# Algolzw/image-restoration-sde

Hardware: AMD Instinct MI355X
Metric: restored images/sec at 256x256, 100-step IR-SDE reverse sampler (higher is better)
Workload: dtype f32; 1 GPU; IR-SDE deraining ConditionalUNet nf=64 depth=4, reverse_sde, batch=16/GPU 256x256, T=100 (BASELINE.json configs[1]); compute_dtype=fp32, global_batch=16

## Files before the change

image_restoration_sde_amd/_lib.py:

```python
import ctypes
import os
import subprocess
import threading

_HERE = os.path.dirname(os.path.abspath(__file__))
LIB_PATH = os.environ.get("IRSDE_LIB_PATH") or os.path.join(_HERE, "libirsde_hip.so")
CSRC = os.path.join(_HERE, "csrc")

MODE = {"sde": 0, "ode": 1, "posterior": 2, "dsde_sde": 3, "dsde_ode": 4}
COEF_STRIDE = 12
FLAG_KEEP_ACTIVATIONS = 1
FLAG_NAIVE_CONV = 2
FLAG_NO_WINOGRAD = 4
FLAG_NO_WINOGRAD_F43 = 8
FLAG_UNCOND_FULLATTN = 16
FLAG_BF16 = 32
FLAG_NAF_INTRO_SKIP = 64
FLAG_BF16_ACT = 128
FLAG_NO_FUSED_LN = 256
FLAG_NAF_LENS = 512
FLAG_FP16 = 1024
FLAG_NO_WINOGRAD_FUSED = 2048
FLAG_NO_FUSED_ATTN = 4096
FLAG_NO_NAF_CHAIN = 8192
FLAG_SPLIT_BF16X2 = 16384
FLAG_SPLIT_F16X2 = 32768
FLAG_NAF_STEREO = 65536
FLAG_NAF_UNCOND = 131072
FLAG_UNET_STEREO = 262144
FLAG_F16_ACT = 524288
FLAG_NO_WINO_POLY = 1048576
FLAG_SCAM_STREAM = 2097152
FLAG_NO_SPLIT3 = 4194304
SAMPLE_GRAPH = 1
SAMPLE_PROFILE = 2

SYMBOLS = [
    "irsde_last_error", "irsde_version", "irsde_create", "irsde_create_nafnet", "irsde_destroy", "irsde_num_weights",
    "irsde_weight_name", "irsde_weight_shape", "irsde_load_weight", "irsde_finalize_weights",
    "irsde_set_schedule", "irsde_unet_forward", "irsde_sample", "irsde_sde_step", "irsde_philox_normal",
    "irsde_get_profile", "irsde_debug_tap", "irsde_work_model", "irsde_debug_conv", "irsde_debug_conv_choice", "irsde_debug_conv_halo_choice", "irsde_debug_conv_features", "irsde_plan_describe", "irsde_bench_conv", "irsde_op_profile", "irsde_debug_split_gemm", "irsde_bench_naf_chain", "irsde_debug_force_subbatches", "irsde_debug_force_chain_groups", "irsde_debug_force_wino_poly", "irsde_debug_force_split3", "irsde_debug_force_split3_attn", "irsde_debug_force_split3_blocks", "irsde_debug_force_split3_1x1", "irsde_debug_split3_1x1", "irsde_debug_split3_1x1_choice", "irsde_debug_scam", "irsde_debug_scam_full",
    "irsde_debug_scam_stream", "irsde_debug_scam_full_stream", "irsde_debug_force_scam_stream",
    "irsde_debug_naf_gate_sca", "irsde_debug_tlsc", "irsde_debug_ln_film", "irsde_debug_naf_lnconv", "irsde_debug_naf_chain", "irsde_debug_naf_chain_split_order",
    "irsde_debug_full_attention16",
    "irsde_eval_metrics", "irsde_tensor2img", "irsde_upscale_bicubic", "irsde_mask_to", "irsde_imresize",
    "irsde_create_lpips", "irsde_lpips", "irsde_debug_lpips_tap",
    "irsde_set_lens_info", "irsde_nafnet_set_local_pool", "irsde_create_latent_unet", "irsde_latent_shapes", "irsde_latent_encode", "irsde_latent_decode", "irsde_latent_hidden",
]


class IrsdeLibraryError(RuntimeError):
    pass


class IrsdeError(RuntimeError):
    pass


class Config(ctypes.Structure):
    _fields_ = [("in_nc", ctypes.c_int32), ("out_nc", ctypes.c_int32), ("nf", ctypes.c_int32),
                ("depth", ctypes.c_int32), ("device", ctypes.c_int32), ("flags", ctypes.c_int32)]


class NafConfig(ctypes.Structure):
    _fields_ = [("img_channel", ctypes.c_int32), ("width", ctypes.c_int32), ("middle_blk_num", ctypes.c_int32),
                ("n_enc", ctypes.c_int32), ("enc_blk_nums", ctypes.c_int32 * 8), ("n_dec", ctypes.c_int32),
                ("dec_blk_nums", ctypes.c_int32 * 8), ("device", ctypes.c_int32), ("flags", ctypes.c_int32)]


class LatentConfig(ctypes.Structure):
    _fields_ = [("in_ch", ctypes.c_int32), ("out_ch", ctypes.c_int32), ("ch", ctypes.c_int32), ("n_mult", ctypes.c_int32),
                ("ch_mult", ctypes.c_int32 * 8), ("embed_dim", ctypes.c_int32), ("device", ctypes.c_int32),
                ("flags", ctypes.c_int32)]


_lib = None
_lock = threading.Lock()


PROBES_LIB_PATH = os.path.join(_HERE, "libirsde_hip_probes.so")


def build_library(force=False, verbose=False, probes=True):
    if force:
        subprocess.run(["make", "-C", CSRC, "clean"], check=True, capture_output=not verbose)
    for extra in ([], ["PROBES=1"]) if probes else ([],):
        r = subprocess.run(["make", "-j8", "-C", CSRC] + extra, capture_output=True, text=True)
        if r.returncode != 0:
            raise IrsdeLibraryError("building libirsde_hip%s.so failed:\n" % ("_probes" if extra else "") + r.stdout + r.stderr)
        if verbose:
            print(r.stdout)
    return LIB_PATH


def _declare(lib):
    c = ctypes
    P = c.c_void_p
    lib.irsde_last_error.restype = c.c_char_p
    lib.irsde_last_error.argtypes = []
    lib.irsde_version.restype = c.c_int
    lib.irsde_create.argtypes = [c.POINTER(Config), c.POINTER(P)]
    lib.irsde_create_nafnet.argtypes = [c.POINTER(NafConfig), c.POINTER(P)]
    lib.irsde_destroy.argtypes = [P]
    lib.irsde_destroy.restype = None
    lib.irsde_num_weights.argtypes = [P]
    lib.irsde_weight_name.argtypes = [P, c.c_int]
    lib.irsde_weight_name.restype = c.c_char_p
    lib.irsde_weight_shape.argtypes = [P, c.c_int, c.POINTER(c.c_int64), c.POINTER(c.c_int)]
    lib.irsde_load_weight.argtypes = [P, c.c_char_p, P, c.POINTER(c.c_int64), c.c_int]
    lib.irsde_finalize_weights.argtypes = [P]
    lib.irsde_set_schedule.argtypes = [P, c.c_int, P]
    lib.irsde_unet_forward.argtypes = [P, P, P, c.POINTER(c.c_int64), c.c_int, c.c_int, c.c_int, c.c_int, P, P]
    lib.irsde_sample.argtypes = [P, c.c_int, P, P, P, c.c_uint64, c.c_uint64, c.c_int, c.c_int, c.c_int,
                                 c.c_int, c.c_int, P, P, c.c_int]
    lib.irsde_sde_step.argtypes = [c.c_int, c.c_int, P, P, P, P, P, c.c_uint64, c.c_uint64, c.c_int, c.c_int,
                                   c.c_int, c.c_int, P]
    lib.irsde_philox_normal.argtypes = [P, c.c_int, c.c_int, c.c_int, c.c_uint64, c.c_uint64, P]
    lib.irsde_get_profile.argtypes = [P, c.POINTER(c.c_double)]
    lib.irsde_debug_tap.argtypes = [P, c.c_char_p, P, c.POINTER(c.c_int64)]
    lib.irsde_work_model.argtypes = [P, c.c_int, c.c_int, c.c_int, c.POINTER(c.c_double)]
    lib.irsde_debug_conv.argtypes = [P, c.c_int, P, c.c_int, c.c_int, c.c_int, c.c_int, c.c_int, P, c.c_int, c.c_int,
                                     c.c_int, c.c_int, c.c_int, P, P, c.c_int, c.c_int, P, P, c.c_int, c.c_int, P]
    lib.irsde_debug_conv_choice.argtypes = [c.c_int] * 13 + [c.c_uint] + [c.c_int] * 4 + [c.POINTER(c.c_int), c.c_char_p, c.c_int]
    lib.irsde_debug_conv_halo_choice.argtypes = [c.c_int] * 13 + [c.c_uint] + [c.c_int] * 5 + [c.c_char_p, c.c_int]
    lib.irsde_debug_conv_features.argtypes = ([P, c.c_int, P, c.c_int] + [c.c_int] * 4 + [P] + [c.c_int] * 7 + [P] * 3 + [P, c.c_int, P, P, P, c.c_int] + [c.c_int] * 6 +
                                              [c.POINTER(c.c_int), P, c.c_char_p, c.c_int, P])
    lib.irsde_plan_describe.argtypes = [P, c.c_int, c.c_int, c.c_int, c.c_char_p, c.c_int]
    lib.irsde_op_profile.argtypes = [P, c.c_char_p, c.c_int]
    lib.irsde_bench_conv.argtypes = [c.c_int] * 11 + [c.POINTER(c.c_double)]
    lib.irsde_bench_naf_chain.argtypes = [c.c_int] * 4 + [c.POINTER(c.c_double)]
    lib.irsde_debug_force_subbatches.argtypes = [c.c_int]
    lib.irsde_debug_force_chain_groups.argtypes = [c.c_int]
    lib.irsde_debug_force_wino_poly.argtypes = [c.c_int]
    lib.irsde_debug_force_split3.argtypes = [c.c_int]
    lib.irsde_debug_force_split3_attn.argtypes = [c.c_int]
    lib.irsde_debug_force_split3_1x1.argtypes = [c.c_int]
    lib.irsde_debug_split3_1x1.argtypes = [P, c.c_int, c.c_int, P, c.c_int, c.c_int, P, P, P, c.c_int, c.c_int, c.c_int, c.c_int, P]
    lib.irsde_debug_split3_1x1_choice.argtypes = [c.c_int] * 13 + [c.c_uint] + [c.c_int] * 6 + [c.c_char_p, c.c_int]
    lib.irsde_debug_force_split3_blocks.argtypes = [c.c_int]
    lib.irsde_debug_scam.argtypes = [P, c.c_int, c.c_int, c.c_int, c.c_int] + [P] * 12 + [P, P]
    lib.irsde_debug_scam_full.argtypes = [P, c.c_int, c.c_int, c.c_int, c.c_int] + [P] * 12 + [P, P]
    lib.irsde_debug_scam_stream.argtypes = [P, c.c_int, c.c_int, c.c_int, c.c_int] + [P] * 12 + [c.c_int, P, P]
    lib.irsde_debug_scam_full_stream.argtypes = [P, c.c_int, c.c_int, c.c_int, c.c_int] + [P] * 12 + [c.c_int, P, P]
    lib.irsde_debug_force_scam_stream.argtypes = [c.c_int]
    lib.irsde_debug_naf_gate_sca.argtypes = [P, c.c_int, c.c_int, c.c_int, c.c_int] + [P] * 8
    lib.irsde_debug_tlsc.argtypes = [P] + [c.c_int] * 6 + [P] * 4
    lib.irsde_debug_ln_film.argtypes = [P, c.c_int64, c.c_int, c.c_int64, P, P, P, c.c_int, P, P]
    lib.irsde_debug_naf_lnconv.argtypes = [c.c_int, P, c.c_int64, c.c_int, c.c_int, c.c_int64, P, P, P, c.c_int, P, P, P, c.c_int, P, P, P, P, P]
    lib.irsde_debug_naf_chain.argtypes = [P, P, c.c_int, c.c_int] + [P] * 16 + [P, c.c_int, c.c_int, P, c.c_int, c.c_int, c.c_int, P]
    lib.irsde_debug_naf_chain_split_order.argtypes = [c.c_int, c.c_int, c.POINTER(c.c_int), c.c_int64]
    lib.irsde_debug_full_attention16.argtypes = [P, c.c_int, c.c_int, P, P]
    lib.irsde_debug_split_gemm.argtypes = [P, P, P, c.c_int, c.c_int, c.c_int, c.c_int, c.c_int, P]
    lib.irsde_eval_metrics.argtypes = [P, P, c.c_int, c.c_int, c.c_int, c.c_int, c.c_int, c.POINTER(c.c_double), P]
    lib.irsde_tensor2img.argtypes = [P, P, c.c_int, c.c_int, c.c_int, c.c_int, P]
    lib.irsde_upscale_bicubic.argtypes = [P, P, c.c_int, c.c_int, c.c_int, c.c_int, c.c_int, P]
    lib.irsde_mask_to.argtypes = [P, P, c.c_int, c.c_int, c.c_int, c.c_int, P, c.c_int, c.c_int, c.c_int, c.c_int, P]
    lib.irsde_imresize.argtypes = [P, P] + [c.c_int] * 6 + [P, P, c.c_int, P, P, c.c_int, P]
    lib.irsde_create_lpips.argtypes = [c.POINTER(P)]
    lib.irsde_lpips.argtypes = [P, P, P, c.c_int, c.c_int, c.c_int, c.c_int, c.POINTER(c.c_double), c.POINTER(c.c_double), P]
    lib.irsde_debug_lpips_tap.argtypes = [P, P, c.c_int, c.c_int, c.c_int, c.c_int, c.c_int, P, c.POINTER(c.c_int64), P]
    lib.irsde_set_lens_info.argtypes =[P, c.POINTER(c.c_float), c.c_int]
    lib.irsde_nafnet_set_local_pool.argtypes = [P, c.c_int, c.c_int, c.c_int, c.c_int]
    lib.irsde_create_latent_unet.argtypes = [c.POINTER(LatentConfig), c.POINTER(P)]
    lib.irsde_latent_shapes.argtypes = [P, c.c_int, c.c_int, c.POINTER(c.c_int64), c.POINTER(c.c_int64), c.POINTER(c.c_int)]
    lib.irsde_latent_encode.argtypes = [P, P, c.c_int, c.c_int, c.c_int, P, c.POINTER(P), P]
    lib.irsde_latent_decode.argtypes = [P, P, c.POINTER(P), c.c_int, c.c_int, c.c_int, P, P]
    lib.irsde_latent_hidden.argtypes = [P, c.c_int, c.c_int, c.c_int, c.c_int, P, P]
    for name in SYMBOLS:
        getattr(lib, name)
    return lib


def lib():
    global _lib
    with _lock:
        if _lib is None:
            if not os.path.exists(LIB_PATH):
                raise IrsdeLibraryError(
                    "libirsde_hip.so not found at %s — build it with `python -c 'import __graft_entry__ as g; "
                    "g.build()'` or `make -C %s`. There is no CPU/PyTorch fallback for this path." % (LIB_PATH, CSRC))
            try:
                _lib = _declare(ctypes.CDLL(LIB_PATH))
            except OSError as ex:
                raise IrsdeLibraryError("failed to load %s: %s" % (LIB_PATH, ex)) from ex
        return _lib


_probes = None


def probes_lib():
    global _probes
    with _lock:
        if _probes is None:
            if not os.path.exists(PROBES_LIB_PATH):
                raise IrsdeLibraryError("libirsde_hip_probes.so not found at %s — build it with `make -C %s PROBES=1`" % (PROBES_LIB_PATH, CSRC))
            try:
                _probes = _declare(ctypes.CDLL(PROBES_LIB_PATH))
            except OSError as ex:
                raise IrsdeLibraryError("failed to load %s: %s" % (PROBES_LIB_PATH, ex)) from ex
        return _probes


def check(rc, L=None):
    if rc != 0:
        msg = (L or lib()).irsde_last_error()
        raise IrsdeError("libirsde_hip error %d: %s" % (rc, msg.decode() if msg else "?"))


def stream_ptr(torch_stream=None):
    import torch
    s = torch_stream if torch_stream is not None else torch.cuda.current_stream()
    return ctypes.c_void_p(s.cuda_stream)
```

image_restoration_sde_amd/csrc/common.h:

```cpp
#pragma once
#include <hip/hip_runtime.h>
#include <cstdint>
#include <cstdio>
#include <cstdlib>
#include <functional>
#include <stdexcept>
#include <string>
#include <vector>
#include "split3_layout.h"

namespace irsde {

struct HipError : std::runtime_error {
    using std::runtime_error::runtime_error;
};
struct HipOutOfMemory : HipError {
    using HipError::HipError;
};

inline int tuning_env_int(const char* name, int dflt) {
    static const bool on = [] { const char* t = getenv("IRSDE_TUNING"); return t && atoi(t) == 1; }();
    if (!on) return dflt;
    const char* v = getenv(name);
    return v ? atoi(v) : dflt;
}

#define IRSDE_HIP_CHECK(expr)                                                                  \
    do {                                                                                       \
        hipError_t _e = (expr);                                                                \
        if (_e != hipSuccess) {                                                                \
            throw ::irsde::HipError(std::string(#expr) + " failed: " + hipGetErrorString(_e) + \
                                    " (" __FILE__ ":" + std::to_string(__LINE__) + ")");       \
        }                                                                                      \
    } while (0)

struct ConvParams {
    const float* in0 = nullptr;
    const float* in1 = nullptr;
    int C0 = 0, C1 = 0;
    int pix0 = 0, pix1 = 0;
    int Hin = 0, Win = 0;
    int in_shift = 0;
    const float* w = nullptr;
    const unsigned short* w_bf = nullptr;
    int f16 = 0;
    const unsigned short* w_pair = nullptr;
    float pair_scale = 1.f;
    int Cout = 0;
    int KH = 1, KW = 1, stride = 1, pad_y = 0, pad_x = 0;
    int B = 0, Ho = 0, Wo = 0;
    float* out = nullptr;
    int out_stride = 0;
    const float* bias = nullptr;
    const float* film = nullptr;
    int film_bstride = 0;
    int silu = 0;
    const float* res = nullptr;
    int res_stride = 0;
    int splits = 1;
    float* partial = nullptr;
    const float* zeros = nullptr;
    const float* ch_scale = nullptr;
    const float* in_scale = nullptr;
    int gate = 0;
    const float* gate_film = nullptr;
    int gate_film_bstride = 0;
    int shuffle = 0;
    int nz = 1;
    long long z_in = 0, z_w = 0, z_out = 0;
    int no_direct_epi = 0;
    int in_bf16 = 0, out_bf16 = 0;
    int in_f16 = 0, out_f16 = 0;
    const float* ln_g = nullptr;
    float ln_eps = 1e-5f;
};

struct WinoParams {
    const float* in0 = nullptr;
    const float* in1 = nullptr;
    int C0 = 0, C1 = 0, Hin = 0, Win = 0, in_shift = 0;
    int B = 0, TH = 0, TW = 0, T = 0;
    int tile = 2;
    float* V = nullptr;
    unsigned short* Vs = nullptr;
    int nplanes = 0;
    int v_f16 = 0;
    float v_scale = 1.f;
    int v_pairs = 0;
    int v_triples = 0;
    const float* M = nullptr;
    int Cout = 0;
    float* out = nullptr;
    int out_stride = 0;
    const float* bias = nullptr;
    const float* film = nullptr;
    int film_bstride = 0;
    int silu = 0;
    const float* res = nullptr;
    int res_stride = 0;
};
void launch_wino_input(const WinoParams& p, hipStream_t s);
struct WinoPolyParams {
    int up = 0;
    const float* in = nullptr;
    int C = 0, Hin = 0, Win = 0;
    int B = 0, TH = 0, TW = 0, T = 0;
    float* V = nullptr;
    unsigned short* Vs = nullptr;
    int thread_writer = 0;
    const float* M = nullptr;
    int Cout = 0, Ho = 0, Wo = 0;
    float* out = nullptr;
    int out_stride = 0;
    const float* bias = nullptr;
};
void launch_wino_poly_input(const WinoPolyParams& p, hipStream_t s);
void launch_wino_poly_output(const WinoPolyParams& p, hipStream_t s);
void wino_poly_transform_weights(const float* w_packed, int Cout, int Cin, float* U, int up);
struct SplitGemmArgs {
    const unsigned short* a = nullptr;
    const unsigned short* b = nullptr;
    float* out = nullptr;
    long long plA = 0, plB = 0, pA = 0, pB = 0, pO = 0;
    int M = 0, N = 0, K = 0, lda = 0, ldc = 0;
    float out_scale = 1.f;
    int n_inner = 1;
    int nblk_n = 0;
};
void gemm_split_global_init();
void launch_gemm_split_pairs(const SplitGemmArgs& a, int ncomp, hipStream_t s, int abl = 0, bool f16 = false);
void launch_split_pairs(const float* in, unsigned short* out, size_t rows, int K, hipStream_t s, bool f16 = false,
                        float scale = 1.0f);
struct Split3Launch {
    enum Abl { FULL = 0, NO_LOADS = 1, NO_MFMA = 3, NO_STORES = 4 };
    enum Tri { RULE, ON, OFF };
    Abl abl = FULL;
    Tri walk = RULE;
    Tri drain = RULE;
};
void launch_gemm_split_triples(const SplitGemmArgs& a, int ncomp, hipStream_t s, const Split3Launch& o = {});
void set_force_split3_blocks(int n);
bool gemm_split_triples_fits(long long M, long long N, long long K, long long ldc);
void launch_split_triples(const float* in, unsigned short* out, int ncomp, size_t rows, int K, hipStream_t s);
struct Split3aArgs {
    const float* in0 = nullptr;
    const float* in1 = nullptr;
    int C0 = 0, C1 = 0;
    int pix0 = 0, pix1 = 0;
    const unsigned short* w3 = nullptr;
    const float* bias = nullptr;
    float* out = nullptr;
    int M = 0, N = 0, out_stride = 0;
    int nblk_n = 0;
};
bool gemm_split3a_fits(const Split3aArgs& a, const char** why_not = nullptr);
int gemm_split3a_blocks(long long M, int N, int cus, bool walk = true);
constexpr size_t kSplit3aLds = (size_t)2 * (256 * 128 + 128 * 192);
void launch_gemm_split3a(const Split3aArgs& a, hipStream_t s, const Split3Launch& o = {});
struct Split3x1Choice {
    bool adopt = false;
    const char* why_not = "";
    int grid = 0, lds = 0;
};
Split3x1Choice split3_1x1_choose(const ConvParams& p, bool exact_f32, int master, int knob, int cus);
Split3aArgs split3_1x1_args(const ConvParams& p, const unsigned short* w3);
void launch_split_planes(const float* in, unsigned short* out, size_t n, size_t plane, int nplanes, hipStream_t s, bool f16 = false,
                         float scale = 1.0f);
void launch_wino_output(const WinoParams& p, hipStream_t s);
void wino_transform_weights(const float* w_packed, int Cout, int Cin, float* U, int tile);
bool wino_fused_eligible(const ConvParams& p);
void wino_fused_pack_weights(const float* U, int Cout, int Cin, float* Uf);
void launch_wino_fused(const ConvParams& p, const float* Uf, hipStream_t s, unsigned long long* dbg = nullptr, int dflags = 0);
int wino_fused_num_blocks(const ConvParams& p);
bool wino_fused64_eligible(const ConvParams& p);
void wino_fused64_pack_weights(const float* U, int Cout, int Cin, float* Uf);
void launch_wino_fused64(const ConvParams& p, const float* Uf, hipStream_t s, int variant = 0);
void wino_fused64_set_debug(unsigned long long* buf);
constexpr float kWinoFused64PairVScale = 0.0625f;
void launch_wino_fused64_split_weights(const float* Uf, unsigned short* out, size_t nfloats, float scale, hipStream_t s);
int wino_fused64_num_blocks(const ConvParams& p);
bool wino_fused64_xcd_nb(const ConvParams& p);
void wino_fused_global_init();
int device_cu_count();
bool wino_fused64t_eligible(const ConvParams& p);
long long wino_fused64t_num_items(const ConvParams& p);
void launch_wino_fused64t(const ConvParams& p, const float* Uf, hipStream_t s, int variant = 0);
void wino_fused64t_set_debug(unsigned long long* buf);
void wino_fused_t_global_init();
void naf_chain_global_init();
void naf_chain_set_debug(unsigned long long* buf);
bool naf_chain_shape_ok(int H, int W, int c);
size_t naf_chain_weight_halves(int nblocks);
size_t naf_chain_vec_floats(int nblocks);
void launch_naf_chain(const float* x, float* out, const unsigned short* w, const float* vecs, int nblocks, int B, const float* film, int film_bstride,
                      int film_off, const float* cam, int cam_bstride, int cam_off, hipStream_t s, int variant = 0);
std::vector<int> naf_chain_split_order(int nblocks, int G);
void naf_chain_build_split_weights(const unsigned short* w1, unsigned short* dst, int nblocks, int G, hipStream_t s);
size_t naf_chain_split_scratch_bytes(int B);
int naf_chain_split_groups(int B, int G);
void launch_naf_chain_split(const float* x, float* out, const unsigned short* wG, const float* vecs, int nblocks, int B, const float* film, int film_bstride,
                            int film_off, const float* cam, int cam_bstride, int cam_off, int G, void* scratch, hipStream_t s);
const unsigned* naf_chain_split_error_flag(const void* scratch, int B);
void naf_chain_split_reset(void* scratch, int B);
void naf_chain_set_sabotage(int on);
void attention_global_init();

double conv_flops(const ConvParams& p);
struct ConvTune {
    enum Tile { TILE_AUTO, TILE_128, TILE_256x128, TILE_256, TILE_128_ONE_PER_CU };
    enum Halo { HALO_AUTO, HALO_OFF, HALO_FORCE_512, HALO_FORCE_256 };
    enum ZLoop { ZLOOP_AUTO, ZLOOP_OFF, ZLOOP_ALL, ZLOOP_PAIRS, ZLOOP_FORCE_1X1 };
    enum Order { ORDER_AUTO, ORDER_N_FAST, ORDER_N_SLOW };
    bool rules_off = false;
    Tile tile = TILE_AUTO;
    bool no_buffer_desc = false;
    bool no_direct_epi = false;
    Halo halo = HALO_AUTO;
    ZLoop zloop = ZLOOP_AUTO;
    Order halo_order = ORDER_AUTO;
};
struct ConvKnobs {
    int small_bn = 2, small_bn_f32 = 0;
    int pair_tile256 = 1, pair_inscale256 = 0;
    int no_bufa = 0;
    int zloop = -1, zloop_1x1 = -1;
    int zloop_maxnk = 32, zloop_minblk = 1024, zloop_deep = 1, zloop_ragged64 = 2048;
};
const ConvKnobs& conv_knobs_from_env();
struct HaloChoice {
    int pixels = 0;
    int BN = 0;
    int op = 0, act = 0;
    int tiles_x = 0, tiles_y = 0, nblk_n = 0;
    int n_slow = 0;
    unsigned grid = 0;
    int lds = 0;
    int instance = -1;
};
constexpr int kHaloInstances = 9;
struct ConvChoice {
    enum Family { PAIR, NARROW3, ZLOOP_BATCH, ZLOOP_1X1, HALO, IGEMM };
    enum Operand { OP_F32, OP_F32_BUF, OP_BF16, OP_F16 };
    enum Storage { ACT_F32, ACT_BF16, ACT_F16 };
    Family family = IGEMM;
    int BM = 0, BN = 0;
    Operand op = OP_F32;
    Storage act = ACT_F32;
    bool inscale = false;
    int zbatch = 0, zrows = 0;
    unsigned gx = 0, gy = 1, gz = 1;
    HaloChoice halo;
    int threads = 0, lds = 0;
    int row = -1;
    std::string name() const;
    long long blocks() const { return (long long)gx * gy * gz; }
};
int conv_base_bn(int Cout);
void conv_validate(const ConvParams& p);
ConvChoice conv_choose(const ConvParams& p, const ConvTune& t, const ConvKnobs& k, int cu_count);
int conv_instance_count();
void launch_conv(const ConvParams& p, hipStream_t s, const ConvTune& t = {}, const ConvKnobs* knobs = nullptr, ConvChoice* chosen = nullptr);
void conv_global_init();
void conv_halo_global_init();
bool conv_halo_eligible(const ConvParams& p);
HaloChoice conv_halo_choose(const ConvParams& p, const ConvTune& t, int halo2, int nslow);
bool conv_halo2_wanted(const ConvParams& p);
HaloChoice launch_conv_halo(const ConvParams& p, hipStream_t s, const ConvTune& t = {});
void launch_fill_random(float* p, size_t n, unsigned seed, float scale, hipStream_t s);
__device__ __forceinline__ float silu_hw(const float v) {
    return v * __builtin_amdgcn_rcpf(1.0f + __builtin_amdgcn_exp2f(v * -1.44269504088896341f));
}

void launch_f32_to_bf16(const float* in, unsigned short* out, size_t n, hipStream_t s);
void launch_f32_to_f16(const float* in, unsigned short* out, size_t n, hipStream_t s);
void launch_bf16_to_f32(const unsigned short* in, float* out, size_t n, hipStream_t s);
void launch_f16_to_f32(const unsigned short* in, float* out, size_t n, hipStream_t s);
void launch_conv_naive(const ConvParams& p, hipStream_t s);

void launch_layernorm(const float* x, const float* g, const float* res, float* out, int64_t M, int C,
                      float eps, hipStream_t s, bool bf16 = false);
void launch_layernorm_film(const float* x, const float* g, const float* scale, const float* shift, int film_bstride,
                           int64_t pixels_per_image, float* out, int64_t M, int C, float eps, hipStream_t s,
                           bool f16 = false);
int dwgate_tiles(int H, int W, int c);
bool naf_lnconv_ok(int c, int Cout, long long M);
void launch_naf_pwconv(const float* x, const float* in_scale, int64_t pixels_per_image, const unsigned short* w16, const float* bias, const float* ch_scale,
                       const float* res, float* out, int64_t M, int c, int Cout, hipStream_t s, bool f16 = false);
void naf_lnconv_global_init();
void launch_naf_lnconv(const float* x, const float* g, const float* fscale, const float* fshift, int film_bstride, int64_t pixels_per_image,
                       const unsigned short* w16, const float* bias, float* out, int64_t M, int c, int Cout, int gate, const float* gate_film,
                       int gate_film_bstride, hipStream_t s, bool f16 = false);
void launch_dwconv_gate(const float* u, const float* w, const float* bias, float* out, float* partial, int B, int H, int W,
                        int c, hipStream_t s, bool f16 = false);
void launch_sca(const float* partial, int ntiles, const float* W, const float* bias, float* mean, float* s_out, int B,
                int c, int HW, hipStream_t s);
void launch_sca_mean(const float* partial, int ntiles, float* mean, int B, int c, int HW, hipStream_t s);
void tlsc_check_shape(int B, int h, int w, int c, int k1, int k2);
void launch_tlsc_pool(const float* gated, float* rowsum, float* pooled, int B, int h, int w, int c, int k1, int k2, hipStream_t s);
void launch_tlsc_scale(float* gated, const float* scale, int B, int h, int w, int c, int k1, int k2, hipStream_t s);
void launch_row_gate(const float* in, float* out, int rows, int h, hipStream_t s);

struct AttnWorkspace {
    float* pmax = nullptr;
    float* pctx = nullptr;
    float* psum = nullptr;
    float* ctx = nullptr;
    int nch = 0;
};
int attn_num_chunks(int N, int B);
void launch_linear_attention(const float* qkv, float* out, int B, int N, const AttnWorkspace& ws, hipStream_t s,
                             bool bf16 = false);

enum class AttnMode : int {
    F32 = 0,
    PairF16 = 1,
    Bf16 = 2,
    Fp16 = 3,
    Bf16x3 = 4,
};
struct AttnProj {
    AttnMode mode = AttnMode::F32;
    bool act_bf16 = false;
    const unsigned short *kv = nullptr, *q = nullptr, *out = nullptr;
    float kv_inv = 1.f, q_inv = 1.f, out_inv = 1.f;
};
bool attn_fused_has_instance(int C, AttnMode mode, bool act_bf16);
void launch_attention_kv_context(const float* xn, const float* wkv, int B, int N, int C, const AttnWorkspace& ws, hipStream_t s,
                                 const float* ln_g = nullptr, float ln_eps = 1e-5f, const AttnProj& proj = {});
__host__ __device__ inline size_t attn_frag3_index(size_t row, int k, int K) {
    return ((((row >> 5) * (size_t)(K >> 4) + (size_t)(k >> 4)) * 2 + (size_t)((k >> 3) & 1)) * 32 + (row & 31)) * 8 + (size_t)(k & 7);
}
void launch_split_frag3(const float* in, unsigned short* out, size_t rows, int K, hipStream_t s);
void launch_attention_q_out(const float* q, float* out, int B, int N, const AttnWorkspace& ws, hipStream_t s);
void launch_attention_q_out_fused(const float* xn, const float* x, const float* wq, const float* wout, const float* bias,
                                  const float* g2, float* y, int B, int N, int C, float eps, const AttnWorkspace& ws, hipStream_t s,
                                  const float* ln_g = nullptr, const AttnProj& proj = {});

void scam_check_shape(int H, int W, int c, bool any_width = false);
void launch_scam_prologue(const float* x, const float* g_l, const float* g_r, float* xs2, int B, int H, int W, int c, hipStream_t s);
void launch_scam_core(const float* qv, float* F, int B, int H, int W, int c, hipStream_t s);
void launch_scam_epilogue(const float* x, const float* F, const float* beta, const float* gamma, float* out, int B, int H, int W, int c, hipStream_t s);
void scam_pack_proj(const float* w1, const float* b1, const float* w2, const float* b2, int c, std::vector<float>& w, std::vector<float>& bias);
constexpr int kScamFullMaxW = 1024;
constexpr int kScamFullMaxC = 2048;
void scam_full_check_shape(int H, int W, int c, bool any_width = false);
void launch_scam_full_prologue(const float* x, const float* g_l, const float* g_r, float* x2, int B, int H, int W, int c, hipStream_t s);
void launch_scam_full_core(const float* qv, float* F, int B, int H, int W, int c, hipStream_t s);
void launch_scam_full_epilogue(float* x, const float* F, const float* beta, const float* gamma, int B, int H, int W, int c, hipStream_t s);
constexpr int kScamMaxWs = 512;
constexpr int kScamStreamMaxBlockW = 512;
bool scam_stream_block_ok(int block_w);
void launch_scam_stream_core(const float* qv, float* F, int B, int Hs, int Ws, int c, int block_w, hipStream_t s);
void launch_stereo_prep(const float* xt, const float* cond, float* x0, int B, int ic, int P, int H, int W, int Hp, int Wp, hipStream_t s);
void launch_stereo_pack_pred(const float* in, float* out, int B, int ic, int Hp, int Wp, int in_stride, int out_stride, hipStream_t s);
void launch_stereo_unet_prep(const float* xt, const float* cond, float* x0, int B, int ic, int P, int H, int W, int Hp, int Wp, hipStream_t s);
void launch_stereo_unet_pack_pred(const float* in, const float* xt, float* out, int B, int ic, int H, int W, int Hp, int Wp, int in_stride, int out_stride,
                                  hipStream_t s);

void launch_full_attention(const float* qkv, float* out, int B, int N, hipStream_t s);
void launch_full_attention16(const unsigned short* qkv, unsigned short* out, int B, int N, hipStream_t s);

void launch_prep_input(const float* xt, const float* cond, float* x0, int B, int in_nc, int H, int W, int Hp, int Wp,
                       hipStream_t s, int reflect = 1);

enum Act { ACT_NONE = 0, ACT_SILU = 1, ACT_GELU = 2 };
void launch_sinusoid(const float* tvals, const float* freqs, float* out, int rows, int half, hipStream_t s);
void launch_row_linear(const float* in, int in_stride, const float* W, const float* b, float* out, int out_stride,
                       int rows, int in_dim, int out_dim, int act_in, int act_out, hipStream_t s);

struct StepState {
    int t;
    int t_next;
    int pad0, pad1;
    float coef[12];
};
void launch_step_begin(StepState* st, const float* film_table, int film_row, float* film_cur,
                       const float* coef_table, hipStream_t s);
void launch_set_step(StepState* st, int t_next, hipStream_t s);

struct SampleCtl {
    int mode;
    int pad;
    const float* noise;
    long long noise_tstride;
    unsigned long long seed;
    unsigned long long image_offset;
};
void launch_set_ctl(SampleCtl* ctl, int mode, const float* noise, long long noise_tstride, unsigned long long seed,
                    unsigned long long image_offset, hipStream_t s);

void launch_unpack_pred(const float* pred, float* out, int B, int C, int H, int W, int Hp, int Wp, int stride, hipStream_t s);
void launch_add(const float* a, const float* b, float* out, size_t n, hipStream_t s);
void launch_nchw_to_nhwc_pad(const float* in, float* out, int B, int C, int H, int W, int Hp, int Wp, int Cp, int reflect,
                             hipStream_t s);
void launch_nhwc_to_nchw(const float* in, float* out, int B, int C, int H, int W, hipStream_t s, bool bf16 = false, bool f16 = false);

struct UpdateParams {
    float* x;
    const float* mu;
    const float* pred;
    int64_t sb, sc, sy, sx;
    const float* noise;
    int64_t noise_tstride;
    const StepState* st;
    const SampleCtl* ctl;
    int t_imm;
    float coef_imm[12];
    int mode;
    int B, C, H, W;
    uint64_t seed;
    uint64_t image_offset;
    int batch0;
};
void launch_sde_update(const UpdateParams& p, hipStream_t s);
void launch_philox_normal(float* out, int B, int CHW, int t, uint64_t seed, uint64_t image_offset, hipStream_t s);

void eval_metrics(const float* out, const float* gt, int B, int C, int H, int W, int crop, double* sums_host, hipStream_t s);
void tensor2img_u8(const float* in, unsigned char* out, int B, int C, int H, int W, hipStream_t s);

struct LpipsLayer { int k, stride, pad, cin, cout; };
constexpr LpipsLayer kLpipsLayers[5] = {{11, 4, 2, 3, 64}, {5, 1, 2, 64, 192}, {3, 1, 1, 192, 384}, {3, 1, 1, 384, 256}, {3, 1, 1, 256, 256}};
inline int lpips_cin_padded(int l) { return (kLpipsLayers[l].cin + 3) & ~3; }
struct LpipsWeights {
    const float* w[5];
    const float* bias[5];
    const float* lin[5];
};
struct LpipsGeom {
    int h[5], w[5];
    int ph[2], pw[2];
};
LpipsGeom lpips_geometry(int H, int W);
int lpips_dist_blocks(int hw);
size_t lpips_workspace_floats(int N, int H, int W);
void lpips_features(const LpipsWeights& wt, const float* in0, const float* in1, int B, int H, int W, int normalize, float* ws, float* taps[5], hipStream_t s,
                    const std::function<void(const char*)>& mark);
void lpips_distances(const LpipsWeights& wt, float* const taps[5], int B, int H, int W, double* partial, hipStream_t s,
                     const std::function<void(const char*)>& mark);

void upscale_bicubic(const float* in, float* out, int B, int C, int H, int W, int scale, hipStream_t s);
void mask_to(const float* x, const unsigned char* masks, int Bm, int Hm, int Wm, int Cm, float* out, int B, int C, int H, int W, hipStream_t s);
void imresize(const float* in, float* out, int B, int C, int H, int W, int Ho, int Wo, const float* wH, const int* sH, int KH, const float* wW,
              const int* sW, int KW, hipStream_t s);

}
```

image_restoration_sde_amd/csrc/engine_debug.hip:

```cpp
#include "engine.h"
#include "../../include/irsde_hip_debug.h"

using namespace irsde;

namespace irsde {
namespace {

struct Scratch {
    hipStream_t s;
    std::vector<void*> bufs;
    explicit Scratch(hipStream_t s_) : s(s_) {}
    ~Scratch() {
        (void)hipStreamSynchronize(s);
        for (void* p : bufs) (void)hipFree(p);
    }
    Scratch(const Scratch&) = delete;
    Scratch& operator=(const Scratch&) = delete;
    template <class T> T* alloc(size_t n) {
        void* p = nullptr;
        IRSDE_HIP_CHECK(hipMalloc(&p, n * sizeof(T)));
        bufs.push_back(p);
        return static_cast<T*>(p);
    }
    float* upload(const float* host, size_t n) {
        float* d = alloc<float>(n);
        IRSDE_HIP_CHECK(hipMemcpy(d, host, n * sizeof(float), hipMemcpyHostToDevice));
        return d;
    }
    float* upload(const std::vector<float>& v) { return upload(v.data(), v.size()); }
};
struct OwnedStream {
    hipStream_t s = nullptr;
    explicit OwnedStream(unsigned flags) { IRSDE_HIP_CHECK(hipStreamCreateWithFlags(&s, flags)); }
    ~OwnedStream() { (void)hipStreamDestroy(s); }
    OwnedStream(const OwnedStream&) = delete;
    OwnedStream& operator=(const OwnedStream&) = delete;
};
struct EventPair {
    hipEvent_t e0 = nullptr, e1 = nullptr;
    EventPair() {
        IRSDE_HIP_CHECK(hipEventCreate(&e0));
        IRSDE_HIP_CHECK(hipEventCreate(&e1));
    }
    ~EventPair() {
        if (e0) (void)hipEventDestroy(e0);
        if (e1) (void)hipEventDestroy(e1);
    }
    EventPair(const EventPair&) = delete;
    EventPair& operator=(const EventPair&) = delete;
};
template <class Run>
double time_launches(hipStream_t s, int iters, Run&& run) {
    EventPair ev;
    IRSDE_HIP_CHECK(hipEventRecord(ev.e0, s));
    for (int i = 0; i < iters; ++i) run();
    IRSDE_HIP_CHECK(hipEventRecord(ev.e1, s));
    IRSDE_HIP_CHECK(hipStreamSynchronize(s));
    float ms = 0.f;
    IRSDE_HIP_CHECK(hipEventElapsedTime(&ms, ev.e0, ev.e1));
    return ms / iters;
}


ConvTune conv_tune_from_code(int code) {
    ConvTune t;
    t.rules_off = code != 0;
    switch (code) {
        case 3: t.tile = ConvTune::TILE_256x128; break;
        case 50: t.tile = ConvTune::TILE_256; break;
        case 5: t.tile = ConvTune::TILE_128_ONE_PER_CU; break;
        case 6: t.no_buffer_desc = true; break;
        case 7: t.no_direct_epi = true; break;
        case 60: t.tile = ConvTune::TILE_256; t.halo = ConvTune::HALO_OFF; break;
        case 61: t.tile = ConvTune::TILE_128; t.halo = ConvTune::HALO_OFF; break;
        case 64: t.halo = ConvTune::HALO_FORCE_512; break;
        case 65: t.halo = ConvTune::HALO_FORCE_256; break;
        case 68: t.halo = ConvTune::HALO_FORCE_512; t.halo_order = ConvTune::ORDER_N_SLOW; break;
        case 69: t.halo = ConvTune::HALO_FORCE_256; t.halo_order = ConvTune::ORDER_N_SLOW; break;
        case 70: t.zloop = ConvTune::ZLOOP_OFF; break;
        case 71: t.zloop = ConvTune::ZLOOP_ALL; break;
        case 72: t.zloop = ConvTune::ZLOOP_PAIRS; break;
        case 73: t.zloop = ConvTune::ZLOOP_FORCE_1X1; break;
        default: break;
    }
    return t;
}

Split3Launch split3_launch_twin(int twin, int abl = 0) {
    Split3Launch o;
    o.abl = static_cast<Split3Launch::Abl>(abl);
    o.walk = twin == 0 ? Split3Launch::RULE : twin == 1 ? Split3Launch::OFF : Split3Launch::ON;
    o.drain = twin == 0 ? Split3Launch::RULE : twin == 1 ? Split3Launch::OFF : Split3Launch::ON;
    return o;
}

enum class Operand { F32, BF16, F16 };

enum class ConvPath {
    Direct,
    Valu,
    WinoF2,
    WinoF4,
    Poly,
    PolyTriples,
    F4Triples,
    F4Pairs,
    DirectPair,
    Fused32,
    Fused64,
    Fused64Pair,
    Fused64T,
    Split3a,
};
struct DebugConvRow {
    int code;
    ConvPath path;
    Operand op;
    bool act_bf16;
    int tune;
    int variant;
    bool up;
    bool thread_writer;
};
constexpr DebugConvRow direct(int code, Operand op, bool act_bf16, int tune) { return {code, ConvPath::Direct, op, act_bf16, tune, 0, false, false}; }
constexpr DebugConvRow on_path(int code, ConvPath path, Operand op = Operand::F32) { return {code, path, op, false, 0, 0, false, false}; }
constexpr DebugConvRow wino(int code, ConvPath path, int tune) { return {code, path, Operand::F32, false, tune, 0, false, false}; }
constexpr DebugConvRow poly(int code, ConvPath path, bool up, bool thread_writer = false) { return {code, path, Operand::F32, false, 0, 0, up, thread_writer}; }
constexpr DebugConvRow fused(int code, ConvPath path, int variant) { return {code, path, Operand::F32, false, 0, variant, false, false}; }
constexpr DebugConvRow kDebugConv[] = {
    direct(0, Operand::F32, false, 0),
    on_path(1, ConvPath::Valu),
    wino(2, ConvPath::WinoF2, 0), wino(12, ConvPath::WinoF2, 71), wino(22, ConvPath::WinoF2, 72),
    wino(3, ConvPath::WinoF4, 0), wino(13, ConvPath::WinoF4, 71), wino(23, ConvPath::WinoF4, 72),
    poly(24, ConvPath::Poly, false), poly(25, ConvPath::Poly, true),
    poly(26, ConvPath::PolyTriples, false), poly(27, ConvPath::PolyTriples, true), poly(28, ConvPath::PolyTriples, true, true),
    on_path(48, ConvPath::F4Triples), on_path(49, ConvPath::Split3a),
    on_path(44, ConvPath::F4Pairs, Operand::F16), on_path(45, ConvPath::F4Pairs, Operand::BF16),
    on_path(46, ConvPath::DirectPair, Operand::F16), on_path(47, ConvPath::DirectPair, Operand::BF16),
    on_path(33, ConvPath::Fused32),
    fused(34, ConvPath::Fused64, 0), fused(36, ConvPath::Fused64, 64), fused(55, ConvPath::Fused64, 20),
    fused(35, ConvPath::Fused64Pair, 4), fused(37, ConvPath::Fused64Pair, 4 + 64), fused(56, ConvPath::Fused64Pair, 24),
    fused(62, ConvPath::Fused64T, 0), fused(63, ConvPath::Fused64T, 64),
    direct(4, Operand::BF16, false, 0), direct(160, Operand::BF16, false, 60), direct(161, Operand::BF16, false, 61), direct(162, Operand::BF16, false, 64),
    direct(163, Operand::BF16, false, 65),
    direct(5, Operand::F16, false, 0), direct(165, Operand::F16, false, 61), direct(166, Operand::F16, false, 64), direct(167, Operand::F16, false, 65),
    direct(204, Operand::BF16, true, 0), direct(260, Operand::BF16, true, 60), direct(261, Operand::BF16, true, 61), direct(262, Operand::BF16, true, 64),
    direct(263, Operand::BF16, true, 65),
    direct(100, Operand::F32, false, 0), direct(103, Operand::F32, false, 3), direct(105, Operand::F32, false, 5), direct(106, Operand::F32, false, 6),
    direct(107, Operand::F32, false, 7), direct(150, Operand::F32, false, 50), direct(170, Operand::F32, false, 70), direct(171, Operand::F32, false, 71),
    direct(172, Operand::F32, false, 72), direct(173, Operand::F32, false, 73),
};

enum class BenchKind {
    Conv,
    Fused32,
    Fused32Stamps,
    Wino3,
    Wino3Gemm,
    Fused64,
    Fused64Stamps,
    Fused64T,
    Fused64TStamps,
    PairGemm,
    TripleGemm,
    Split3aGemm,
};
struct BenchRow {
    int lo, hi;
    BenchKind kind;
    int arg;
    Operand op;
    bool pair;
    bool act_bf16;
};
constexpr BenchRow bench(int lo, int hi, BenchKind kind, int arg, Operand op = Operand::F32, bool pair = false, bool act_bf16 = false) {
    return {lo, hi, kind, arg, op, pair, act_bf16};
}
constexpr BenchRow kBenchConv[] = {
    bench(0, 0, BenchKind::Conv, 0), bench(3, 3, BenchKind::Conv, 3), bench(5, 7, BenchKind::Conv, 5), bench(50, 50, BenchKind::Conv, 50),
    bench(70, 73, BenchKind::Conv, 70),
    bench(60, 61, BenchKind::Conv, 60, Operand::BF16),
    bench(62, 62, BenchKind::Conv, 0, Operand::BF16),
    bench(63, 63, BenchKind::Conv, 0, Operand::BF16, false, true),
    bench(64, 65, BenchKind::Conv, 64, Operand::BF16),
    bench(66, 67, BenchKind::Conv, 64, Operand::BF16, false, true),
    bench(480, 480, BenchKind::Conv, 0, Operand::F16, true), bench(481, 481, BenchKind::Conv, 0, Operand::BF16, true),
    bench(482, 482, BenchKind::Conv, 61, Operand::F16, true),
    bench(80, 80, BenchKind::Fused32, 0),
    bench(83, 82 + 255, BenchKind::Fused32, 1),
    bench(82, 82, BenchKind::Fused32Stamps, 0),
    bench(81, 81, BenchKind::Wino3, 0), bench(421, 421, BenchKind::Wino3Gemm, 0),
    bench(430, 432, BenchKind::Fused64, 20),
    bench(434, 434, BenchKind::Fused64, 24, Operand::F16),
    bench(435, 435, BenchKind::Fused64Stamps, 25), bench(2004, 2004, BenchKind::Fused64Stamps, 25),
    bench(2001, 2002, BenchKind::Fused64Stamps, 28),
    bench(460, 462, BenchKind::Fused64T, 0),
    bench(467, 469, BenchKind::Fused64T, 6),
    bench(465, 465, BenchKind::Fused64TStamps, 5),
    bench(4650, 4653, BenchKind::Fused64TStamps, 12),
    bench(472, 476, BenchKind::PairGemm, 0),
    bench(490, 504, BenchKind::TripleGemm, 0),
    bench(510, 524, BenchKind::Split3aGemm, 0),
};

template <class Row, size_t N, class Lo, class Hi>
constexpr bool codes_disjoint(const Row (&rows)[N], Lo lo, Hi hi) {
    for (size_t i = 0; i < N; ++i)
        for (size_t j = 0; j < N; ++j)
            if (i != j && lo(rows[i]) <= hi(rows[j]) && lo(rows[j]) <= hi(rows[i])) return false;
    return true;
}
constexpr int row_code(const DebugConvRow& r) { return r.code; }
constexpr int row_lo(const BenchRow& r) { return r.lo; }
constexpr int row_hi(const BenchRow& r) { return r.hi; }
static_assert(codes_disjoint(kDebugConv, row_code, row_code), "irsde_debug_conv: a selector code has two rows");
static_assert(codes_disjoint(kBenchConv, row_lo, row_hi), "irsde_bench_conv: a variant has two rows");

const DebugConvRow& debug_conv_lookup(int code) {
    for (const DebugConvRow& r : kDebugConv)
        if (r.code == code) return r;
    throw HipError("debug_conv: unknown selector code " + std::to_string(code));
}
struct BenchSel {
    const BenchRow& row;
    int arg;
};
BenchSel bench_conv_lookup(int code) {
    for (const BenchRow& r : kBenchConv)
        if (code >= r.lo && code <= r.hi) return {r, r.arg + (code - r.lo)};
    throw HipError("bench_conv: unknown variant " + std::to_string(code));
}

SplitGemmArgs split_gemm_args(const unsigned short* a, const unsigned short* b, float* C, int M, int N, int K, size_t pA, size_t pB) {
    SplitGemmArgs g;
    g.a = a; g.b = b; g.out = C;
    g.pA = (long long)pA; g.pB = (long long)pB; g.pO = (long long)M * N;
    g.M = M; g.N = N; g.K = K; g.lda = K; g.ldc = N;
    return g;
}
SplitGemmArgs split_triples(Scratch& mem, const float* A, const float* Bm, float* C, int M, int N, int K, int ncomp, hipStream_t s) {
    const size_t ea = split3_comp_elems((size_t)M, (size_t)K), eb = split3_comp_elems((size_t)N, (size_t)K);
    unsigned short *ta = mem.alloc<unsigned short>(ea * ncomp), *tb = mem.alloc<unsigned short>(eb * ncomp);
    launch_split_triples(A, ta, ncomp, (size_t)M, K, s);
    launch_split_triples(Bm, tb, ncomp, (size_t)N, K, s);
    return split_gemm_args(ta, tb, C, M, N, K, ea, eb);
}
SplitGemmArgs split_pairs(Scratch& mem, const float* A, const float* Bm, float* C, int M, int N, int K, int ncomp, hipStream_t s, bool f16 = false, float sa = 1.f,
                          float sb = 1.f) {
    unsigned short *pa = mem.alloc<unsigned short>((size_t)2 * ncomp * M * K), *pb = mem.alloc<unsigned short>((size_t)2 * ncomp * N * K);
    launch_split_pairs(A, pa, (size_t)ncomp * M, K, s, f16, sa);
    launch_split_pairs(Bm, pb, (size_t)ncomp * N, K, s, f16, sb);
    SplitGemmArgs g = split_gemm_args(pa, pb, C, M, N, K, (size_t)M * K, (size_t)N * K);
    g.out_scale = 1.0f / (sa * sb);
    return g;
}

void write_choice_line(const ConvChoice& c, char* out, int out_len) {
    snprintf(out, (size_t)out_len, "name=%s family=%d tile=%dx%d op=%d act=%d inscale=%d zbatch=%d zrows=%d grid=%ux%ux%u threads=%d lds=%d row=%d of %d",
             c.name().c_str(), (int)c.family, c.BM, c.BN, (int)c.op, (int)c.act, (int)c.inscale, c.zbatch, c.zrows, c.gx, c.gy, c.gz, c.threads, c.lds, c.row,
             conv_instance_count());
}

void write_halo_line(const HaloChoice& h, char* out, int out_len) {
    snprintf(out, (size_t)out_len, "kernel=halo%d bn=%d op=%d act=%d tiles=%dx%d nblk_n=%d nslow=%d grid=%u lds=%d instance=%d of %d", h.pixels, h.BN, h.op, h.act,
             h.tiles_x, h.tiles_y, h.nblk_n, h.n_slow, h.grid, h.lds, h.instance, kHaloInstances);
}

ConvParams choice_hook_params(int B, int Hin, int Win, int C0, int C1, int Cout, int K, int stride, int pad, int in_shift, int operand, int storage, int pair,
                              unsigned features, int splits, int nz) {
    static const float dummy[4] = {};
    float* const some = const_cast<float*>(dummy);
    auto bit = [&](int i) { return (features >> i & 1u) ? some : nullptr; };
    ConvParams p;
    p.in0 = some; p.C0 = C0; p.pix0 = C0; p.in1 = C1 ? some : nullptr; p.C1 = C1; p.pix1 = C1;
    p.Hin = Hin; p.Win = Win; p.in_shift = in_shift;
    p.w = some; p.Cout = Cout; p.KH = K; p.KW = K; p.stride = stride; p.pad_y = pad; p.pad_x = pad;
    p.B = B;
    p.Ho = ((Hin << in_shift) + 2 * pad - K) / stride + 1;
    p.Wo = ((Win << in_shift) + 2 * pad - K) / stride + 1;
    p.out = some; p.out_stride = Cout; p.res_stride = Cout; p.zeros = some;
    p.bias = bit(0); p.film = bit(1); p.silu = bit(2) != nullptr; p.res = bit(3); p.in_scale = bit(4); p.ch_scale = bit(5);
    p.gate = bit(6) != nullptr; p.shuffle = bit(7) != nullptr; p.ln_g = bit(8);
    if (pair) p.w_pair = reinterpret_cast<const unsigned short*>(some);
    else if (operand) p.w_bf = reinterpret_cast<const unsigned short*>(some);
    p.f16 = operand == 2;
    p.in_bf16 = p.out_bf16 = storage == 1;
    p.in_f16 = p.out_f16 = storage == 2;
    p.nz = nz;
    if (splits > 1) { p.splits = splits; p.partial = some; }
    return p;
}

struct ScamHookArgs {
    const float* x;
    float* out;
    const float *norm_l_g, *norm_r_g, *l_proj1_w, *l_proj1_b, *r_proj1_w, *r_proj1_b, *l_proj2_w, *l_proj2_b, *r_proj2_w, *r_proj2_b, *beta, *gamma;
};
struct ScamHookDev {
    float *gl, *gr, *beta, *gamma;
    float *in2, *qv, *F;
    size_t vsz;
};
template <class ShapeCheck, class Prologue, class Tail>
void scam_hook(const ScamHookArgs& a, int B, int Hs, int Ws, int C, void* stream, ShapeCheck check_shape, Prologue prologue, Tail tail) {
    if (!a.x || !a.out || !a.norm_l_g || !a.norm_r_g || !a.l_proj1_w || !a.l_proj1_b || !a.r_proj1_w || !a.r_proj1_b || !a.l_proj2_w || !a.l_proj2_b ||
        !a.r_proj2_w || !a.r_proj2_b || !a.beta || !a.gamma)
        throw HipError("null argument");
    check_shape();
    hipStream_t s = reinterpret_cast<hipStream_t>(stream);
    conv_global_init();
    std::vector<float> wl, bl, wr, br;
    scam_pack_proj(a.l_proj1_w, a.l_proj1_b, a.l_proj2_w, a.l_proj2_b, C, wl, bl);
    scam_pack_proj(a.r_proj1_w, a.r_proj1_b, a.r_proj2_w, a.r_proj2_b, C, wr, br);
    Scratch mem(s);
    auto up = [&](const float* h, size_t n) {
        float* d = mem.alloc<float>(std::max<size_t>(n, 16));
        if (h) IRSDE_HIP_CHECK(hipMemcpy(d, h, n * 4, hipMemcpyHostToDevice));
        return d;
    };
    ScamHookDev d;
    d.gl = up(a.norm_l_g, C); d.gr = up(a.norm_r_g, C); d.beta = up(a.beta, C); d.gamma = up(a.gamma, C);
    float *dwl = up(wl.data(), wl.size()), *dbl = up(bl.data(), bl.size()), *dwr = up(wr.data(), wr.size()), *dbr = up(br.data(), br.size());
    d.vsz = (size_t)B * Hs * Ws * 2 * C;
    d.in2 = up(nullptr, 2 * d.vsz); d.qv = up(nullptr, 2 * d.vsz); d.F = up(nullptr, d.vsz);
    float* dz = up(nullptr, 256);
    IRSDE_HIP_CHECK(hipMemset(dz, 0, 1024));
    prologue(d, s);
    for (int v = 0; v < 2; ++v) {
        ConvParams p;
        p.in0 = d.in2 + v * d.vsz; p.C0 = 2 * C; p.pix0 = 2 * C;
        p.Hin = Hs; p.Win = Ws;
        p.w = v ? dwr : dwl; p.Cout = 2 * C; p.KH = p.KW = 1; p.stride = 1;
        p.B = B; p.Ho = Hs; p.Wo = Ws;
        p.out = d.qv + v * d.vsz; p.out_stride = 2 * C;
        p.bias = v ? dbr : dbl;
        p.zeros = dz;
        launch_conv(p, s);
    }
    tail(d, s);
    IRSDE_HIP_CHECK(hipStreamSynchronize(s));
}

}
}

extern "C" {

int irsde_debug_scam(const float* x, int B, int H, int W, int C, const float* norm_l_g, const float* norm_r_g, const float* l_proj1_w,
                     const float* l_proj1_b, const float* r_proj1_w, const float* r_proj1_b, const float* l_proj2_w, const float* l_proj2_b,
                     const float* r_proj2_w, const float* r_proj2_b, const float* beta, const float* gamma, float* out, void* stream) {
    return guard([&] {
        scam_hook(
            {x, out, norm_l_g, norm_r_g, l_proj1_w, l_proj1_b, r_proj1_w, r_proj1_b, l_proj2_w, l_proj2_b, r_proj2_w, r_proj2_b, beta, gamma}, B, H / 4, W / 4, C, stream,
            [&] {
                if (B < 1) throw HipError("debug_scam: bad shape");
                scam_check_shape(H, W, C);
            },
            [&](const ScamHookDev& d, hipStream_t s) { launch_scam_prologue(x, d.gl, d.gr, d.in2, B, H, W, C, s); },
            [&](const ScamHookDev& d, hipStream_t s) {
                launch_scam_core(d.qv, d.F, B, H, W, C, s);
                launch_scam_epilogue(x, d.F, d.beta, d.gamma, out, B, H, W, C, s);
            });
    });
}

int irsde_debug_scam_full(const float* x, int B, int H, int W, int C, const float* norm_l_g, const float* norm_r_g, const float* l_proj1_w,
                          const float* l_proj1_b, const float* r_proj1_w, const float* r_proj1_b, const float* l_proj2_w, const float* l_proj2_b,
                          const float* r_proj2_w, const float* r_proj2_b, const float* beta, const float* gamma, float* out, void* stream) {
    return guard([&] {
        scam_hook(
            {x, out, norm_l_g, norm_r_g, l_proj1_w, l_proj1_b, r_proj1_w, r_proj1_b, l_proj2_w, l_proj2_b, r_proj2_w, r_proj2_b, beta, gamma}, B, H, W, C, stream,
            [&] {
                if (B < 1 || (long long)B * H > 65535) throw HipError("debug_scam_full: bad shape");
                scam_full_check_shape(H, W, C);
            },
            [&](const ScamHookDev& d, hipStream_t s) { launch_scam_full_prologue(x, d.gl, d.gr, d.in2, B, H, W, C, s); },
            [&](const ScamHookDev& d, hipStream_t s) {
                launch_scam_full_core(d.qv, d.F, B, H, W, C, s);
                if (out != x) IRSDE_HIP_CHECK(hipMemcpyAsync(out, x, d.vsz * sizeof(float), hipMemcpyDeviceToDevice, s));
                launch_scam_full_epilogue(out, d.F, d.beta, d.gamma, B, H, W, C, s);
            });
    });
}

int irsde_debug_scam_stream(const float* x, int B, int H, int W, int C, const float* norm_l_g, const float* norm_r_g, const float* l_proj1_w,
                            const float* l_proj1_b, const float* r_proj1_w, const float* r_proj1_b, const float* l_proj2_w, const float* l_proj2_b,
                            const float* r_proj2_w, const float* r_proj2_b, const float* beta, const float* gamma, int block_w, float* out, void* stream) {
    return guard([&] {
        scam_hook(
            {x, out, norm_l_g, norm_r_g, l_proj1_w, l_proj1_b, r_proj1_w, r_proj1_b, l_proj2_w, l_proj2_b, r_proj2_w, r_proj2_b, beta, gamma}, B, H / 4, W / 4, C, stream,
            [&] {
                if (B < 1 || (long long)B * (H / 4) > 65535) throw HipError("debug_scam_stream: bad shape");
                if (block_w != 0 && !scam_stream_block_ok(block_w)) throw HipError("debug_scam_stream: block_w must be 0 or a multiple of 16 in [16, 512]");
                scam_check_shape(H, W, C, true);
            },
            [&](const ScamHookDev& d, hipStream_t s) { launch_scam_prologue(x, d.gl, d.gr, d.in2, B, H, W, C, s); },
            [&](const ScamHookDev& d, hipStream_t s) {
                launch_scam_stream_core(d.qv, d.F, B, H / 4, W / 4, C, block_w, s);
                launch_scam_epilogue(x, d.F, d.beta, d.gamma, out, B, H, W, C, s);
            });
    });
}

int irsde_debug_scam_full_stream(const float* x, int B, int H, int W, int C, const float* norm_l_g, const float* norm_r_g, const float* l_proj1_w,
                                 const float* l_proj1_b, const float* r_proj1_w, const float* r_proj1_b, const float* l_proj2_w, const float* l_proj2_b,
                                 const float* r_proj2_w, const float* r_proj2_b, const float* beta, const float* gamma, int block_w, float* out,
                                 void* stream) {
    return guard([&] {
        scam_hook(
            {x, out, norm_l_g, norm_r_g, l_proj1_w, l_proj1_b, r_proj1_w, r_proj1_b, l_proj2_w, l_proj2_b, r_proj2_w, r_proj2_b, beta, gamma}, B, H, W, C, stream,
            [&] {
                if (B < 1 || (long long)B * H > 65535) throw HipError("debug_scam_full_stream: bad shape");
                if (block_w != 0 && !scam_stream_block_ok(block_w)) throw HipError("debug_scam_full_stream: block_w must be 0 or a multiple of 16 in [16, 512]");
                scam_full_check_shape(H, W, C, true);
            },
            [&](const ScamHookDev& d, hipStream_t s) { launch_scam_full_prologue(x, d.gl, d.gr, d.in2, B, H, W, C, s); },
            [&](const ScamHookDev& d, hipStream_t s) {
                launch_scam_stream_core(d.qv, d.F, B, H, W, C, block_w, s);
                if (out != x) IRSDE_HIP_CHECK(hipMemcpyAsync(out, x, d.vsz * sizeof(float), hipMemcpyDeviceToDevice, s));
                launch_scam_full_epilogue(out, d.F, d.beta, d.gamma, B, H, W, C, s);
            });
    });
}

int irsde_debug_force_scam_stream(int block_w) {
    if (block_w != 0 && !scam_stream_block_ok(block_w)) return guard([&] { throw HipError("debug_force_scam_stream: block_w must be 0 or a multiple of 16 in [16, 512]"); });
    set_force_scam_stream(block_w);
    return IRSDE_OK;
}

int irsde_debug_naf_gate_sca(const float* u, int B, int H, int W, int c, const float* conv2_w, const float* conv2_b, const float* sca_w, const float* sca_b,
                             float* gated_out, float* mean_out, float* s_out, void* stream) {
    return guard([&] {
        if (!u || !conv2_w || !conv2_b || !sca_w || !sca_b || !gated_out || !s_out) throw HipError("null argument");
        if (B < 1 || B > 65535 || H < 1 || W < 1 || c < 4 || c % 4 || (long long)H * W >= (1ll << 31)) throw HipError("debug_naf_gate_sca: bad shape");
        hipStream_t s = reinterpret_cast<hipStream_t>(stream);
        conv_global_init();
        Scratch mem(s);
        float *dw = mem.upload(pack_dwconv_taps(conv2_w, 2 * c)), *db = mem.upload(conv2_b, (size_t)2 * c);
        float *dsw = mem.upload(sca_w, (size_t)c * c), *dsb = mem.upload(sca_b, c);
        const int nt = dwgate_tiles(H, W, c);
        float *partial = mem.alloc<float>((size_t)B * nt * c), *mean = mem.alloc<float>((size_t)B * c);
        launch_dwconv_gate(u, dw, db, gated_out, partial, B, H, W, c, s);
        launch_sca(partial, nt, dsw, dsb, mean, s_out, B, c, H * W, s);
        if (mean_out) launch_sca_mean(partial, nt, mean_out, B, c, H * W, s);
        IRSDE_HIP_CHECK(hipStreamSynchronize(s));
    });
}

int irsde_debug_tlsc(const float* g, int B, int h, int w, int c, int k1, int k2, float* pooled_out, const float* scale_map, float* scaled_out, void* stream) {
    return guard([&] {
        if (!g || !pooled_out || !scale_map || !scaled_out) throw HipError("null argument");
        tlsc_check_shape(B, h, w, c, k1, k2);
        hipStream_t s = reinterpret_cast<hipStream_t>(stream);
        conv_global_init();
        Scratch mem(s);
        float* rowsum = mem.alloc<float>((size_t)B * h * (w - k2 + 1) * c);
        launch_tlsc_pool(g, rowsum, pooled_out, B, h, w, c, k1, k2, s);
        IRSDE_HIP_CHECK(hipMemcpyAsync(scaled_out, g, (size_t)B * h * w * c * sizeof(float), hipMemcpyDeviceToDevice, s));
        launch_tlsc_scale(scaled_out, scale_map, B, h, w, c, k1, k2, s);
        IRSDE_HIP_CHECK(hipStreamSynchronize(s));
    });
}

int irsde_debug_ln_film(const float* x, long long M, int C, long long ppi, const float* g, const float* fscale, const float* fshift, int film_bstride,
                        float* out, void* stream) {
    return guard([&] {
        if (!x || !g || !fscale || !fshift || !out) throw HipError("null argument");
        if (M < 1 || ppi < 1 || C < 4 || C % 4 || C > 2048 || film_bstride < 0 || film_bstride % 4) throw HipError("debug_ln_film: bad shape");
        hipStream_t s = reinterpret_cast<hipStream_t>(stream);
        conv_global_init();
        Scratch mem(s);
        float* dg = mem.upload(g, C);
        launch_layernorm_film(x, dg, fscale, fshift, film_bstride, ppi, out, M, C, 1e-5f, s);
        IRSDE_HIP_CHECK(hipStreamSynchronize(s));
    });
}

int irsde_debug_full_attention16(const void* qkv_bf16, int B, int N, void* out_bf16, void* stream) {
    return guard([&] {
        if (!qkv_bf16 || !out_bf16) throw HipError("null argument");
        hipStream_t s = reinterpret_cast<hipStream_t>(stream);
        launch_full_attention16(static_cast<const unsigned short*>(qkv_bf16), static_cast<unsigned short*>(out_bf16), B, N, s);
        IRSDE_HIP_CHECK(hipStreamSynchronize(s));
    });
}

int irsde_debug_naf_lnconv(int mode, const float* x, long long M, int c, int Cout, long long ppi, const float* g, const float* fscale, const float* fshift,
                           int film_bstride, const float* w, const float* bias, const float* gate_film, int gate_film_bstride, const float* in_scale,
                           const float* ch_scale, const float* res, float* out, void* stream) {
    return guard([&] {
        if (mode < 0 || mode > 3) throw HipError("debug_naf_lnconv: mode must be 0 .. 3");
        if (!x || !w || !bias || !out) throw HipError("null argument");
        if (!naf_lnconv_ok(c, Cout, M) || ppi < 1) throw HipError("debug_naf_lnconv: bad shape");
        const bool ln = mode <= 1;
        if (ln && (!g || !fscale || !fshift || film_bstride < 0 || film_bstride % 4)) throw HipError("debug_naf_lnconv: modes 0 / 1 need g and the FiLM rows");
        if (mode == 1 && gate_film && gate_film_bstride < 0) throw HipError("debug_naf_lnconv: bad lens FiLM stride");
        if (!ln && (!ch_scale || !res || (mode == 2 && !in_scale))) throw HipError("debug_naf_lnconv: modes 2 / 3 need ch_scale and res, mode 2 in_scale");
        hipStream_t s = reinterpret_cast<hipStream_t>(stream);
        conv_global_init();
        std::vector<float> pw, pb;
        pack_conv_rows(w, bias, Cout, c, 1, 1, mode == 1 ? naf_gate_perm(Cout / 2) : std::vector<int>(), pw, pb);
        Scratch mem(s);
        float *dwf = mem.upload(pw), *dbias = mem.upload(pb);
        unsigned short* w16 = mem.alloc<unsigned short>(pw.size());
        launch_f32_to_f16(dwf, w16, pw.size(), s);
        if (ln) {
            float* dg = mem.upload(g, c);
            launch_naf_lnconv(x, dg, fscale, fshift, film_bstride, ppi, w16, dbias, out, M, c, Cout, mode, mode == 1 ? gate_film : nullptr,
                              mode == 1 && gate_film ? gate_film_bstride : 0, s);
        } else {
            float* dcs = mem.upload(ch_scale, Cout);
            launch_naf_pwconv(x, mode == 2 ? in_scale : nullptr, ppi, w16, dbias, dcs, res, out, M, c, Cout, s);
        }
        IRSDE_HIP_CHECK(hipStreamSynchronize(s));
    });
}

int irsde_debug_naf_chain(const float* x, float* out, int B, int nblocks, const float* norm1_g, const float* conv1_w, const float* conv1_b, const float* conv2_w,
                          const float* conv2_b, const float* sca_w, const float* sca_b, const float* conv3_w, const float* conv3_b, const float* beta,
                          const float* norm2_g, const float* conv4_w, const float* conv4_b, const float* conv5_w, const float* conv5_b, const float* gamma,
                          const float* film, int film_bstride, int film_off, const float* cam, int cam_bstride, int cam_off, int groups, void* stream) {
    return guard([&] {
        if (!x || !out || !norm1_g || !conv1_w || !conv1_b || !conv2_w || !conv2_b || !sca_w || !sca_b || !conv3_w || !conv3_b || !beta || !norm2_g || !conv4_w ||
            !conv4_b || !conv5_w || !conv5_b || !gamma || !film)
            throw HipError("null argument");
        if (B < 1 || B > 65535 || nblocks < 1 || nblocks > 64) throw HipError("debug_naf_chain: bad B or nblocks");
        if (groups != 1 && groups != 2 && groups != 4) throw HipError("debug_naf_chain: groups must be 1, 2 or 4");
        if (film_bstride < 0 || film_bstride % 4 || film_off < 0 || film_off % 4) throw HipError("debug_naf_chain: bad FiLM stride / offset");
        if (cam && (cam_bstride < 0 || cam_bstride % 4 || cam_off < 0 || cam_off % 4)) throw HipError("debug_naf_chain: bad lens FiLM stride / offset");
        hipStream_t s = reinterpret_cast<hipStream_t>(stream);
        conv_global_init();
        if (groups > 1 && naf_chain_split_groups(B, groups) > device_cu_count())
            throw HipError("debug_naf_chain: more work-groups than compute units (they must be co-resident)");
        constexpr size_t C = 512;
        std::vector<NafChainHostW> blocks(nblocks);
        for (int i = 0; i < nblocks; ++i) {
            NafChainHostW& b = blocks[i];
            const size_t k = (size_t)i;
            b.norm1_g = norm1_g + k * C; b.conv1_w = conv1_w + k * 2 * C * C; b.conv1_b = conv1_b + k * 2 * C;
            b.conv2_w = conv2_w + k * 18 * C; b.conv2_b = conv2_b + k * 2 * C;
            b.sca_w = sca_w + k * C * C; b.sca_b = sca_b + k * C;
            b.conv3_w = conv3_w + k * C * C; b.conv3_b = conv3_b + k * C; b.beta = beta + k * C;
            b.norm2_g = norm2_g + k * C; b.conv4_w = conv4_w + k * 2 * C * C; b.conv4_b = conv4_b + k * 2 * C;
            b.conv5_w = conv5_w + k * C * C; b.conv5_b = conv5_b + k * C; b.gamma = gamma + k * C;
        }
        std::vector<unsigned short> w;
        std::vector<float> vecs;
        pack_naf_chain_host(blocks, w, vecs);
        Scratch mem(s);
        unsigned short* dw = mem.alloc<unsigned short>(w.size());
        IRSDE_HIP_CHECK(hipMemcpy(dw, w.data(), w.size() * 2, hipMemcpyHostToDevice));
        float* dvec = mem.upload(vecs);
        if (groups == 1) {
            launch_naf_chain(x, out, dw, dvec, nblocks, B, film, film_bstride, film_off, cam, cam ? cam_bstride : 0, cam ? cam_off : 0, s, 0);
            IRSDE_HIP_CHECK(hipStreamSynchronize(s));
            return;
        }
        unsigned short* dwg = mem.alloc<unsigned short>(w.size());
        naf_chain_build_split_weights(dw, dwg, nblocks, groups, s);
        const size_t sb = naf_chain_split_scratch_bytes(B);
        char* dscratch = mem.alloc<char>(sb);
        IRSDE_HIP_CHECK(hipMemset(dscratch, 0, sb));
        launch_naf_chain_split(x, out, dwg, dvec, nblocks, B, film, film_bstride, film_off, cam, cam ? cam_bstride : 0, cam ? cam_off : 0, groups, dscratch, s);
        IRSDE_HIP_CHECK(hipStreamSynchronize(s));
        std::vector<unsigned> state((size_t)4 * B + 1);
        IRSDE_HIP_CHECK(hipMemcpy(state.data(), naf_chain_split_error_flag(dscratch, B) - 4 * B, state.size() * 4, hipMemcpyDeviceToHost));
        if (state[(size_t)4 * B]) throw HipError("debug_naf_chain: the split kernel's groups were not co-resident (spin timeout)");
        for (size_t i = 0; i < (size_t)4 * B; ++i)
            if (state[i]) throw HipError("debug_naf_chain: the split kernel left a barrier counter non-zero");
    });
}

int irsde_debug_naf_chain_split_order(int nblocks, int groups, int* order_out, long long n) {
    return guard([&] {
        if (!order_out || nblocks < 1 || nblocks > 64) throw HipError("debug_naf_chain_split_order: bad argument");
        const std::vector<int> order = naf_chain_split_order(nblocks, groups);
        if ((long long)order.size() != n) throw HipError("debug_naf_chain_split_order: the order has " + std::to_string(order.size()) + " entries");
        std::copy(order.begin(), order.end(), order_out);
    });
}

int irsde_debug_conv(const float* in0, int C0, const float* in1, int C1, int B, int Hin, int Win, int in_shift,
                     const float* w_oihw, int Cout, int KH, int KW, int stride, int pad, const float* bias,
                     const float* film, int film_bstride, int silu, const float* res, float* out, int naive,
                     int splits, void* stream) {
    return guard([&] {
        if (!in0 || !w_oihw || !out) throw HipError("null argument");
        const DebugConvRow& r = debug_conv_lookup(naive);
        hipStream_t s = reinterpret_cast<hipStream_t>(stream);
        conv_global_init();
        const int Cin = C0 + C1;
        std::vector<float> pk((size_t)Cout * KH * KW * Cin);
        for (int o = 0; o < Cout; ++o)
            for (int i = 0; i < Cin; ++i)
                for (int ky = 0; ky < KH; ++ky)
                    for (int kx = 0; kx < KW; ++kx)
                        pk[(((size_t)o * KH + ky) * KW + kx) * Cin + i] = w_oihw[(((size_t)o * Cin + i) * KH + ky) * KW + kx];
        Scratch mem(s);
        float* dw = mem.upload(pk);
        float* db = bias ? mem.upload(bias, Cout) : nullptr;
        ConvParams p;
        p.in0 = in0; p.C0 = C0; p.pix0 = C0; p.in1 = in1; p.C1 = C1; p.pix1 = C1;
        p.Hin = Hin; p.Win = Win; p.in_shift = in_shift;
        p.w = dw; p.Cout = Cout; p.KH = KH; p.KW = KW; p.stride = stride; p.pad_y = pad; p.pad_x = pad;
        p.B = B;
        p.Ho = ((Hin << in_shift) + 2 * pad - KH) / stride + 1;
        p.Wo = ((Win << in_shift) + 2 * pad - KW) / stride + 1;
        p.out = out; p.out_stride = Cout; p.bias = db; p.film = film; p.film_bstride = film_bstride; p.silu = silu;
        p.res = res; p.res_stride = Cout;
        float* dz = mem.alloc<float>(256);
        IRSDE_HIP_CHECK(hipMemset(dz, 0, 1024));
        p.zeros = dz;
        if (splits > 1 && r.path != ConvPath::Valu && r.path != ConvPath::WinoF2 && r.path != ConvPath::WinoF4) {
            p.splits = splits;
            p.partial = mem.alloc<float>((size_t)splits * B * p.Ho * p.Wo * Cout);
        }
        auto wino_weights = [&](int tile) {
            std::vector<float> U((size_t)(tile + 2) * (tile + 2) * Cout * Cin);
            wino_transform_weights(pk.data(), Cout, Cin, U.data(), tile);
            return U;
        };
        auto wino_tiles = [&](int tile) { return (long long)B * (p.Ho / tile) * (p.Wo / tile); };
        auto alloc_M = [&](int ncomp, long long T) { return mem.alloc<float>((size_t)ncomp * T * Cout); };
        auto poly_plan = [&](const char* refusal, float*& dU) {
            if (!(r.up ? wino_poly_up_shape(p) : wino_poly_down_shape(p)) || !wino_poly_eligible(p) || splits > 1) throw HipError(refusal);
            std::vector<float> U((size_t)100 * Cout * Cin);
            wino_poly_transform_weights(pk.data(), Cout, Cin, U.data(), r.up);
            dU = mem.upload(U);
            return make_wino_poly(p, dU, nullptr, nullptr);
        };
        switch (r.path) {
        case ConvPath::PolyTriples: {
            float* dU = nullptr;
            WinoPolyPlan wp = poly_plan("debug_conv: selectors 26 / 27 / 28 run what 24 / 25 run (single source, channels a multiple of 32, bias only)", dU);
            if (!gemm_split_triples_fits(wp.T, Cout, wp.K, Cout)) throw HipError("debug_conv: shape not eligible for the three-piece GEMM");
            unsigned short* dUt = mem.alloc<unsigned short>((size_t)wp.ncomp * split3_comp_elems((size_t)Cout, (size_t)wp.K));
            unsigned short* dVt = mem.alloc<unsigned short>((size_t)wp.ncomp * split3_comp_elems((size_t)wp.T, (size_t)wp.K));
            float* dM = alloc_M(wp.ncomp, wp.T);
            launch_split_triples(dU, dUt, wp.ncomp, (size_t)Cout, wp.K, s);
            wp = make_wino_poly(p, dU, nullptr, dM);
            const SplitGemmArgs sg = make_wino_poly_triples(wp, Cout, dUt, dVt, dM);
            wp.in.thread_writer = r.thread_writer;
            launch_wino_poly_input(wp.in, s);
            launch_gemm_split_triples(sg, wp.ncomp, s);
            launch_wino_poly_output(wp.out, s);
            break;
        }
        case ConvPath::Poly: {
            float* dU = nullptr;
            WinoPolyPlan wp = poly_plan(r.up ? "debug_conv: selector 25 runs a 3x3 stride-1 pad-1 convolution with in_shift = 1 (single source, channels a multiple of 32, bias only)"
                                             : "debug_conv: selector 24 runs a 4x4 stride-2 pad-1 convolution (single source, channels a multiple of 32, bias only)", dU);
            float* dV = mem.alloc<float>((size_t)wp.ncomp * wp.T * wp.K);
            wp = make_wino_poly(p, dU, dV, alloc_M(wp.ncomp, wp.T));
            launch_wino_poly_input(wp.in, s);
            launch_conv(wp.gemm, s);
            launch_wino_poly_output(wp.out, s);
            break;
        }
        case ConvPath::F4Triples: {
            if (!wino_shape_ok(p, 4) || Cin % 32) throw HipError("debug_conv: shape not eligible for the three-piece GEMM");
            const std::vector<float> U = wino_weights(4);
            const long long T = wino_tiles(4);
            if (!gemm_split_triples_fits(T, Cout, Cin, Cout)) throw HipError("debug_conv: shape not eligible for the three-piece GEMM");
            float* dU = mem.upload(U);
            unsigned short* dUt = mem.alloc<unsigned short>((size_t)36 * split3_comp_elems((size_t)Cout, (size_t)Cin));
            unsigned short* dVt = mem.alloc<unsigned short>((size_t)36 * split3_comp_elems((size_t)T, (size_t)Cin));
            launch_split_triples(dU, dUt, 36, (size_t)Cout, Cin, s);
            const WinoSplitPlan sp = make_wino_triples(p, dUt, dVt, alloc_M(36, T));
            launch_wino_input(sp.in, s);
            launch_gemm_split_triples(sp.gemm, 36, s);
            launch_wino_output(sp.out, s);
            break;
        }
        case ConvPath::Split3a: {
            if (splits > 1) p.splits = splits;
            const Split3x1Choice c = split3_1x1_choose(p, true, 2, 2, device_cu_count());
            if (!c.adopt) throw HipError(std::string("debug_conv: selector 49 runs a plain 1x1 layer (bias only): ") + c.why_not);
            unsigned short* dwt = mem.alloc<unsigned short>(split3_comp_elems((size_t)Cout, (size_t)Cin));
            launch_split_triples(dw, dwt, 1, (size_t)Cout, Cin, s);
            launch_gemm_split3a(split3_1x1_args(p, dwt), s);
            break;
        }
        case ConvPath::F4Pairs: {
            const bool f16 = r.op == Operand::F16;
            if (!wino_shape_ok(p, 4) || Cin % 32) throw HipError("debug_conv: shape not eligible for the pair GEMM");
            std::vector<float> U = wino_weights(4);
            const float us = f16 ? pow2_scale_into_512(U.data(), U.size()) : 1.f;
            const long long T = wino_tiles(4);
            float* dU = mem.upload(U);
            unsigned short* dUp = mem.alloc<unsigned short>(2 * U.size());
            unsigned short* dVp = mem.alloc<unsigned short>((size_t)36 * T * Cin * 2);
            launch_split_pairs(dU, dUp, (size_t)36 * Cout, Cin, s, f16, us);
            const WinoSplitPlan sp = make_wino_pairs(p, dUp, dVp, alloc_M(36, T), f16, us);
            launch_wino_input(sp.in, s);
            launch_gemm_split_pairs(sp.gemm, 36, s, 0, f16);
            launch_wino_output(sp.out, s);
            break;
        }
        case ConvPath::Fused64Pair: {
            if (!wino_fused64_eligible(p)) throw HipError("debug_conv: shape not eligible for the fused Winograd kernel");
            std::vector<float> U = wino_weights(4), Uf(U.size());
            wino_fused64_pack_weights(U.data(), Cout, Cin, Uf.data());
            const float usc = pow2_scale_into_512(U.data(), U.size());
            float* dUf = mem.upload(Uf);
            unsigned short* dUp = mem.alloc<unsigned short>(2 * Uf.size());
            launch_wino_fused64_split_weights(dUf, dUp, Uf.size(), usc, s);
            p.pair_scale = 1.0f / (kWinoFused64PairVScale * usc);
            launch_wino_fused64(p, reinterpret_cast<const float*>(dUp), s, r.variant);
            break;
        }
        case ConvPath::Fused32:
        case ConvPath::Fused64:
        case ConvPath::Fused64T: {
            const bool f32k = r.path == ConvPath::Fused32;
            if (f32k ? !wino_fused_eligible(p) : !wino_fused64_eligible(p)) throw HipError("debug_conv: shape not eligible for the fused Winograd kernel");
            const std::vector<float> U = wino_weights(4);
            std::vector<float> Uf(U.size());
            if (f32k) wino_fused_pack_weights(U.data(), Cout, Cin, Uf.data());
            else wino_fused64_pack_weights(U.data(), Cout, Cin, Uf.data());
            float* dUf = mem.upload(Uf);
            if (r.path == ConvPath::Fused64T) {
                if (!wino_fused64t_eligible(p)) throw HipError("debug_conv: shape not eligible for the two-tile-group fused Winograd kernel");
                launch_wino_fused64t(p, dUf, s, r.variant);
            } else if (f32k) {
                launch_wino_fused(p, dUf, s);
            } else {
                launch_wino_fused64(p, dUf, s, r.variant);
            }
            break;
        }
        case ConvPath::WinoF2:
        case ConvPath::WinoF4: {
            const int tile = r.path == ConvPath::WinoF2 ? 2 : 4, ncomp = (tile + 2) * (tile + 2);
            if (!wino_shape_ok(p, tile)) throw HipError("debug_conv: shape not eligible for Winograd");
            const std::vector<float> U = wino_weights(tile);
            const long long T = wino_tiles(tile);
            float* dU = mem.upload(U);
            float* dV = mem.alloc<float>((size_t)ncomp * T * Cin);
            const WinoPlan wp = make_wino(p, dU, dV, alloc_M(ncomp, T), tile);
            launch_wino_input(wp.in, s);
            launch_conv(wp.gemm, s, conv_tune_from_code(r.tune));
            launch_wino_output(wp.out, s);
            break;
        }
        case ConvPath::DirectPair: {
            const bool f16 = r.op == Operand::F16;
            const float sc = f16 ? pow2_scale_into_512(pk.data(), pk.size()) : 1.f;
            unsigned short* dwp = mem.alloc<unsigned short>(2 * pk.size());
            launch_split_pairs(dw, dwp, (size_t)Cout, KH * KW * (C0 + C1), s, f16, sc);
            p.w_pair = dwp; p.pair_scale = 1.0f / sc; p.f16 = f16 ? 1 : 0;
            launch_conv(p, s);
            break;
        }
        case ConvPath::Valu:
            launch_conv_naive(p, s);
            break;
        case ConvPath::Direct: {
            unsigned short* ao = nullptr;
            if (r.op != Operand::F32) {
                unsigned short* d16 = mem.alloc<unsigned short>(pk.size());
                if (r.op == Operand::F16) launch_f32_to_f16(dw, d16, pk.size(), s);
                else launch_f32_to_bf16(dw, d16, pk.size(), s);
                p.w_bf = d16;
                p.f16 = r.op == Operand::F16 ? 1 : 0;
            }
            const size_t npix_in = (size_t)B * Hin * Win, nout = (size_t)B * p.Ho * p.Wo * Cout;
            if (r.act_bf16) {
                auto to_bf = [&](const float* src, size_t n) {
                    unsigned short* d = mem.alloc<unsigned short>(n + 32);
                    launch_f32_to_bf16(src, d, n, s);
                    return reinterpret_cast<const float*>(d);
                };
                p.in0 = to_bf(in0, npix_in * C0);
                if (in1) p.in1 = to_bf(in1, npix_in * C1);
                if (res) p.res = to_bf(res, nout);
                ao = mem.alloc<unsigned short>(nout + 32);
                p.out = reinterpret_cast<float*>(ao);
                p.in_bf16 = p.out_bf16 = 1;
            }
            launch_conv(p, s, conv_tune_from_code(r.tune));
            if (r.act_bf16) launch_bf16_to_f32(ao, out, nout, s);
            break;
        }
        }
        IRSDE_HIP_CHECK(hipStreamSynchronize(s));
    });
}

int irsde_debug_conv_choice(int B, int Hin, int Win, int C0, int C1, int Cout, int K, int stride, int pad, int in_shift, int operand, int storage, int pair,
                            unsigned features, int splits, int nz, int tune, int cu_count, const int* knobs, char* out, int out_len) {
    return guard([&] {
        if (!out || out_len < 1 || K < 1 || stride < 1 || cu_count < 1 || operand < 0 || operand > 2 || storage < 0 || storage > 2 || (pair && operand == 0))
            throw HipError("debug_conv_choice: bad argument");
        const ConvParams p = choice_hook_params(B, Hin, Win, C0, C1, Cout, K, stride, pad, in_shift, operand, storage, pair, features, splits, nz);
        ConvKnobs k;
        static_assert(sizeof(ConvKnobs) == 11 * sizeof(int), "the hook's knob array is ConvKnobs, field by field");
        if (knobs) memcpy(&k, knobs, sizeof k);
        conv_validate(p);
        const ConvChoice c = conv_choose(p, conv_tune_from_code(tune), k, cu_count);
        const bool tabled = c.family != ConvChoice::NARROW3 && c.family != ConvChoice::HALO;
        if (tabled && c.row < 0) throw HipError("launch_conv: no kernel instance " + c.name());
        write_choice_line(c, out, out_len);
    });
}

int irsde_debug_conv_halo_choice(int B, int Hin, int Win, int C0, int C1, int Cout, int K, int stride, int pad, int in_shift, int operand, int storage, int pair,
                                 unsigned features, int splits, int nz, int tune, int halo2, int nslow, char* out, int out_len) {
    return guard([&] {
        if (!out || out_len < 1 || K < 1 || stride < 1 || operand < 0 || operand > 2 || storage < 0 || storage > 2 || (pair && operand == 0))
            throw HipError("debug_conv_halo_choice: bad argument");
        const ConvParams p = choice_hook_params(B, Hin, Win, C0, C1, Cout, K, stride, pad, in_shift, operand, storage, pair, features, splits, nz);
        conv_validate(p);
        const ConvTune t = conv_tune_from_code(tune);
        const ConvChoice c = conv_choose(p, t, ConvKnobs{}, 256);
        if (c.family != ConvChoice::HALO) throw HipError("debug_conv_halo_choice: conv_choose does not send this layer to the halo family, but to " + c.name());
        write_halo_line(conv_halo_choose(p, t, halo2, nslow), out, out_len);
    });
}

int irsde_debug_conv_features(const float* in0, int C0, const float* in1, int C1, int B, int Hin, int Win, int in_shift, const float* w_oihw, int Cout, int K,
                              int stride, int pad, int operand, int storage, int pair, const float* bias, const float* ch_scale, const float* ln_g,
                              const float* film, int film_bstride, const float* res, const float* in_scale, const float* gate_film, int gate_film_bstride,
                              int silu, int gate, int shuffle, int nz, int splits, int tune, const int* knobs, float* out, char* choice, int choice_len,
                              void* stream) {
    return guard([&] {
        if (!in0 || !w_oihw || !out || !choice || choice_len < 1) throw HipError("null argument");
        if (B < 1 || Hin < 1 || Win < 1 || C0 < 1 || C1 < 0 || (C1 > 0) != (in1 != nullptr) || Cout < 1 || K < 1 || stride < 1 || pad < 0 || in_shift < 0 || in_shift > 1 ||
            operand < 0 || operand > 2 || storage < 0 || storage > 2 || (pair && operand == 0) || nz < 1 || splits < 1 || film_bstride < 0 || gate_film_bstride < 0)
            throw HipError("debug_conv_features: bad argument");
        if ((gate && shuffle) || (gate && (Cout % 4 || res)) || (shuffle && Cout % 4) || (gate_film && !gate) || ((gate || shuffle) && film))
            throw HipError("debug_conv_features: gate needs Cout % 4 == 0 and takes no residual, shuffle needs Cout % 4 == 0, gate_film goes with gate, film with neither");
        if (nz > 1 && (B != 1 || Hin != 1 || K != 1 || stride != 1 || pad || in_shift || C1 || storage))
            throw HipError("debug_conv_features: nz > 1 is a stack of 1x1 GEMMs: B = 1, Hin = 1, K = 1, one fp32 source");
        const int Ho = ((Hin << in_shift) + 2 * pad - K) / stride + 1, Wo = ((Win << in_shift) + 2 * pad - K) / stride + 1;
        if (Ho < 1 || Wo < 1) throw HipError("debug_conv_features: empty output");
        hipStream_t s = reinterpret_cast<hipStream_t>(stream);
        conv_global_init();
        const int Cin = C0 + C1;
        const std::vector<int> perm = gate ? naf_gate_perm(Cout / 2) : shuffle ? naf_shuffle_perm(Cout) : std::vector<int>();
        const size_t wz = (size_t)Cout * K * K * Cin;
        std::vector<float> pk(wz * nz), pb, one, oneb;
        for (int z = 0; z < nz; ++z) {
            pack_conv_rows(w_oihw + z * wz, z == 0 ? bias : nullptr, Cout, Cin, K, K, perm, one, z == 0 ? pb : oneb);
            std::copy(one.begin(), one.end(), pk.begin() + z * wz);
        }
        Scratch mem(s);
        float* dw = mem.upload(pk);
        ConvParams p;
        p.in0 = in0; p.C0 = C0; p.pix0 = C0; p.in1 = in1; p.C1 = C1; p.pix1 = C1;
        p.Hin = Hin; p.Win = Win; p.in_shift = in_shift;
        p.w = dw; p.Cout = Cout; p.KH = K; p.KW = K; p.stride = stride; p.pad_y = pad; p.pad_x = pad;
        p.B = B; p.Ho = Ho; p.Wo = Wo;
        const int ostride = gate ? Cout / 2 : shuffle ? Cout / 4 : Cout;
        const size_t npix_in = (size_t)B * Hin * Win * nz, M = (size_t)B * Ho * Wo, nout = M * nz * (gate ? Cout / 2 : Cout);
        p.out = out; p.out_stride = ostride; p.res = res; p.res_stride = ostride;
        if (bias) p.bias = mem.upload(pb);
        if (ch_scale) {
            std::vector<float> cs(Cout);
            for (int o = 0; o < Cout; ++o) cs[o] = ch_scale[perm.empty() ? o : perm[o]];
            p.ch_scale = mem.upload(cs);
        }
        if (ln_g) p.ln_g = mem.upload(ln_g, Cout);
        p.film = film; p.film_bstride = film_bstride; p.silu = silu; p.in_scale = in_scale;
        p.gate = gate ? 1 : 0; p.gate_film = gate_film; p.gate_film_bstride = gate_film ? gate_film_bstride : 0; p.shuffle = shuffle ? 1 : 0;
        p.nz = nz;
        if (nz > 1) { p.z_in = (long long)Win * C0; p.z_w = (long long)Cout * C0; p.z_out = (long long)Win * Cout; }
        float* dz = mem.alloc<float>(256);
        IRSDE_HIP_CHECK(hipMemset(dz, 0, 1024));
        p.zeros = dz;
        if (splits > 1) {
            p.splits = splits;
            p.partial = mem.alloc<float>((size_t)splits * M * Cout);
        }
        const bool f16 = operand == 2;
        unsigned short *w16 = nullptr, *a0 = nullptr, *a1 = nullptr, *ar = nullptr, *ao = nullptr;
        float wsc = 1.f;
        if (pair) {
            wsc = f16 ? pow2_scale_into_512(pk.data(), pk.size()) : 1.f;
            w16 = mem.alloc<unsigned short>(2 * pk.size());
            p.w_pair = w16; p.pair_scale = 1.0f / wsc;
        } else if (operand) {
            w16 = mem.alloc<unsigned short>(pk.size());
            p.w_bf = w16;
        }
        p.f16 = f16 ? 1 : 0;
        if (storage) {
            a0 = mem.alloc<unsigned short>(npix_in * C0);
            p.in0 = reinterpret_cast<const float*>(a0);
            if (in1) { a1 = mem.alloc<unsigned short>(npix_in * C1); p.in1 = reinterpret_cast<const float*>(a1); }
            if (res) { ar = mem.alloc<unsigned short>(nout); p.res = reinterpret_cast<const float*>(ar); }
            ao = mem.alloc<unsigned short>(nout);
            p.out = reinterpret_cast<float*>(ao);
            p.in_bf16 = p.out_bf16 = storage == 1;
            p.in_f16 = p.out_f16 = storage == 2;
        }
        ConvKnobs k;
        static_assert(sizeof(ConvKnobs) == 11 * sizeof(int), "the hook's knob array is ConvKnobs, field by field");
        if (knobs) memcpy(&k, knobs, sizeof k);
        conv_validate(p);
        auto narrow = [&](const float* src, unsigned short* dst, size_t n) {
            if (storage == 2) launch_f32_to_f16(src, dst, n, s);
            else launch_f32_to_bf16(src, dst, n, s);
        };
        if (pair) launch_split_pairs(dw, w16, (size_t)Cout * nz, K * K * Cin, s, f16, wsc);
        else if (operand == 2) launch_f32_to_f16(dw, w16, pk.size(), s);
        else if (operand == 1) launch_f32_to_bf16(dw, w16, pk.size(), s);
        if (storage) {
            narrow(in0, a0, npix_in * C0);
            if (in1) narrow(in1, a1, npix_in * C1);
            if (res) narrow(res, ar, nout);
            IRSDE_HIP_CHECK(hipMemsetAsync(ao, 0xFF, nout * 2, s));
        }
        ConvChoice c;
        launch_conv(p, s, conv_tune_from_code(tune), knobs ? &k : nullptr, &c);
        if (storage == 2) launch_f16_to_f32(ao, out, nout, s);
        else if (storage == 1) launch_bf16_to_f32(ao, out, nout, s);
        IRSDE_HIP_CHECK(hipStreamSynchronize(s));
        write_choice_line(c, choice, choice_len);
        if (c.family == ConvChoice::HALO) {
            const size_t n = strlen(choice);
            if (n + 2 < (size_t)choice_len) {
                choice[n] = ' ';
                write_halo_line(c.halo, choice + n + 1, choice_len - (int)n - 1);
            }
        }
    });
}

int irsde_debug_split_gemm(const float* A, const float* Bm, float* C, int M, int N, int K, int ncomp, int nplanes, void* stream) {
    return guard([&] {
        const int twin3 = nplanes == 43 ? 0 : nplanes == 45 ? 1 : nplanes == 47 ? 2 : -1;
        if (twin3 < 0 && nplanes != 42 && nplanes != 44) throw HipError("debug_split_gemm: nplanes must be 42, 43, 44, 45 or 47");
        hipStream_t s = reinterpret_cast<hipStream_t>(stream);
        conv_global_init();
        Scratch mem(s);
        if (twin3 >= 0) {
            if (!gemm_split_triples_fits(M, N, K, N)) throw HipError("debug_split_gemm: shape not eligible for the three-piece GEMM");
            launch_gemm_split_triples(split_triples(mem, A, Bm, C, M, N, K, ncomp, s), ncomp, s, split3_launch_twin(twin3));
        } else {
            const bool f16 = nplanes == 44;
            launch_gemm_split_pairs(split_pairs(mem, A, Bm, C, M, N, K, ncomp, s, f16, f16 ? 1.0f / 16.0f : 1.f, f16 ? 64.0f : 1.f), ncomp, s, 0, f16);
        }
        IRSDE_HIP_CHECK(hipStreamSynchronize(s));
    });
}

int irsde_debug_force_chain_groups(int g) {
    set_force_chain_groups(g == 1 || g == 2 || g == 4 ? g : 0);
    return IRSDE_OK;
}

int irsde_debug_force_split3(int mode) {
    set_force_split3(mode >= 0 && mode <= 2 ? mode : -1);
    return IRSDE_OK;
}

int irsde_debug_force_split3_attn(int mode) {
    set_force_split3_attn(mode >= 0 && mode <= 2 ? mode : -1);
    return IRSDE_OK;
}
int irsde_debug_force_split3_1x1(int mode) {
    set_force_split3_1x1(mode >= 0 && mode <= 2 ? mode : -1);
    return IRSDE_OK;
}

int irsde_debug_split3_1x1(const float* in0, int C0, int pix0, const float* in1, int C1, int pix1, const float* w, const float* bias, float* out, int M, int N,
                           int out_stride, int mode, void* stream) {
    return guard([&] {
        if (!in0 || !w || !out || (C1 && !in1) || mode < 0 || mode > 2) throw HipError("debug_split3_1x1: bad argument");
        hipStream_t s = reinterpret_cast<hipStream_t>(stream);
        conv_global_init();
        Split3aArgs a;
        a.in0 = in0; a.C0 = C0; a.pix0 = pix0; a.in1 = C1 ? in1 : nullptr; a.C1 = C1; a.pix1 = C1 ? pix1 : 0;
        a.bias = bias; a.out = out; a.M = M; a.N = N; a.out_stride = out_stride;
        const char* why = nullptr;
        if (!gemm_split3a_fits(a, &why)) throw HipError(std::string("debug_split3_1x1: ") + why);
        Scratch mem(s);
        unsigned short* wt = mem.alloc<unsigned short>(split3_comp_elems((size_t)N, (size_t)(C0 + C1)));
        launch_split_triples(w, wt, 1, (size_t)N, C0 + C1, s);
        a.w3 = wt;
        launch_gemm_split3a(a, s, split3_launch_twin(mode));
        IRSDE_HIP_CHECK(hipStreamSynchronize(s));
    });
}

int irsde_debug_split3_1x1_choice(int B, int Hin, int Win, int C0, int C1, int Cout, int K, int stride, int pad, int in_shift, int operand, int storage, int pair,
                                  unsigned features, int splits, int nz, int engine_flags, int master, int knob, int cu_count, char* out, int out_len) {
    return guard([&] {
        if (!out || out_len < 1 || K < 1 || stride < 1 || cu_count < 1 || operand < 0 || operand > 2 || storage < 0 || storage > 2 || (pair && operand == 0))
            throw HipError("debug_split3_1x1_choice: bad argument");
        const ConvParams p = choice_hook_params(B, Hin, Win, C0, C1, Cout, K, stride, pad, in_shift, operand, storage, pair, features, splits, nz);
        const Split3x1Choice c = split3_1x1_choose(p, !(engine_flags & kSplit3NotExactF32), master, knob, cu_count);
        snprintf(out, (size_t)out_len, "adopt=%d grid=%d lds=%d why_not=%s", c.adopt ? 1 : 0, c.grid, c.lds, c.why_not);
    });
}

int irsde_debug_force_split3_blocks(int n) {
    if (n >= 0 && n < 8) return guard([&] { throw HipError("debug_force_split3_blocks: n must be at least 8 (one block per XCD), or negative for the default"); });
    set_force_split3_blocks(n);
    return IRSDE_OK;
}

int irsde_debug_force_wino_poly(int mode) {
    set_force_wino_poly(mode >= 0 && mode <= 2 ? mode : -1);
    return IRSDE_OK;
}

int irsde_debug_force_subbatches(int n) {
    set_force_subbatches(n < 0 ? 0 : n);
    return IRSDE_OK;
}

int irsde_bench_naf_chain(int variant, int nblocks, int B, int iters, double* ms_out) {
    return guard([&] {
        if (!ms_out || nblocks < 1 || nblocks > 64 || B < 1 || iters < 1) throw HipError("bench_naf_chain: bad argument");
        const int G = variant == 22 ? 2 : (variant == 24 || variant == 25 || variant == 26) ? 4 : 1;
#ifdef IRSDE_PROBES
        if (variant != 0 && variant != 1 && variant != 11 && G == 1) throw HipError("bench_naf_chain: bad variant");
#else
        if (variant != 0 && variant != 1 && G == 1) throw HipError("bench_naf_chain: variant 11 is a measurement twin (make PROBES=1)");
#endif
        conv_global_init();
        OwnedStream stream(hipStreamDefault);
        hipStream_t s = stream.s;
        Scratch mem(s);
        const size_t nx = (size_t)B * 64 * 512, nw = naf_chain_weight_halves(nblocks), nv = naf_chain_vec_floats(nblocks);
        float *dx = mem.alloc<float>(nx), *dout = mem.alloc<float>(nx), *dvec = mem.alloc<float>(nv), *dfilm = mem.alloc<float>((size_t)nblocks * 2048);
        unsigned short* dw = mem.alloc<unsigned short>(nw);
        const size_t chunk = (size_t)64 << 20;
        float* dwf = mem.alloc<float>(chunk);
        launch_fill_random(dx, nx, 1, 1.0f, s);
        launch_fill_random(dvec, nv, 2, 0.1f, s);
        launch_fill_random(dfilm, (size_t)nblocks * 2048, 3, 0.1f, s);
        for (size_t o = 0; o < nw; o += chunk) {
            const size_t n = std::min(chunk, nw - o);
            launch_fill_random(dwf, n, 4 + (unsigned)(o / chunk), 0.04f, s);
            launch_f32_to_f16(dwf, dw + o, n, s);
        }
        unsigned short* dwg = nullptr;
        void* dscratch = nullptr;
        if (G > 1) {
            IRSDE_HIP_CHECK(hipStreamSynchronize(s));
            dwg = mem.alloc<unsigned short>(nw);
            naf_chain_build_split_weights(dw, dwg, nblocks, G, s);
            dscratch = mem.alloc<char>(naf_chain_split_scratch_bytes(B));
            IRSDE_HIP_CHECK(hipMemset(dscratch, 0, naf_chain_split_scratch_bytes(B)));
        }
        auto run = [&]() {
            if (G > 1) launch_naf_chain_split(dx, dout, dwg, dvec, nblocks, B, dfilm, 0, 0, nullptr, 0, 0, G, dscratch, s);
            else launch_naf_chain(dx, dout, dw, dvec, nblocks, B, dfilm, 0, 0, nullptr, 0, 0, s, variant == 11 ? 1 : variant);
        };
        if (variant == 26) {
#ifdef IRSDE_PROBES
            naf_chain_set_sabotage(1);
#else
            throw HipError("bench_naf_chain: variant 26 is a PROBES-build test");
#endif
        }
        struct SabotageOff { ~SabotageOff() { naf_chain_set_sabotage(0); } } sabotage_off;
        run();
        if (variant == 25) {
#ifdef IRSDE_PROBES
            const int ng = naf_chain_split_groups(B, 4);
            unsigned long long* dd = mem.alloc<unsigned long long>((size_t)ng * 8 * 16);
            IRSDE_HIP_CHECK(hipMemsetAsync(dd, 0, (size_t)ng * 8 * 16 * 8, s));
            naf_chain_set_debug(dd);
            run();
            IRSDE_HIP_CHECK(hipStreamSynchronize(s));
            naf_chain_set_debug(nullptr);
            std::vector<unsigned long long> hd((size_t)ng * 8 * 16);
            IRSDE_HIP_CHECK(hipMemcpy(hd.data(), dd, hd.size() * 8, hipMemcpyDeviceToHost));
            double acc[16] = {0};
            double nwv = 0;
            for (size_t w = 0; w < (size_t)ng * 8; ++w) {
                if (!hd[w * 16 + 15]) continue;
                for (int k = 0; k < 16; ++k) acc[k] += (double)hd[w * 16 + k];
                nwv += 1;
            }
            static const char* names[12] = {"norm1 (incl. residual-stream fetch)", "conv1 GEMM passes", "depthwise 3x3 + gate + pool", "gated fetch behind barrier (pool)", "sca.1 GEMM", "conv3 GEMM + residual", "norm2 (incl. residual-stream fetch)", "conv4 GEMM + gate", "conv5 GEMM + residual", "scale-vector / gated fetch (sca, conv4)", "group barriers (6 per block)", "publishing (gated slice, residual slice)"};
            printf("naf_chain stamps, 4 groups per image: %d blocks, B=%d; shader cycles per wave and block (mean over %.0f waves)\n", nblocks, B, nwv);
            for (int k = 0; k < 12; ++k) printf("  %-42s %9.0f\n", names[k], acc[k] / nwv / nblocks);
            printf("  %-42s %9.0f\n", "whole kernel / blocks", acc[15] / nwv / nblocks);
            fflush(stdout);
#else
            throw HipError("bench_naf_chain: variant 25 is a measurement twin (make PROBES=1)");
#endif
        }
        if (variant == 11) {
            unsigned long long* dd = mem.alloc<unsigned long long>((size_t)B * 8 * 16);
            IRSDE_HIP_CHECK(hipMemsetAsync(dd, 0, (size_t)B * 8 * 16 * 8, s));
            naf_chain_set_debug(dd);
            launch_naf_chain(dx, dout, dw, dvec, nblocks, B, dfilm, 0, 0, nullptr, 0, 0, s, 11);
            IRSDE_HIP_CHECK(hipStreamSynchronize(s));
            naf_chain_set_debug(nullptr);
            std::vector<unsigned long long> hd((size_t)B * 8 * 16);
            IRSDE_HIP_CHECK(hipMemcpy(hd.data(), dd, hd.size() * 8, hipMemcpyDeviceToHost));
            double acc[16] = {0};
            for (size_t i = 0; i < hd.size(); ++i) acc[i % 16] += (double)hd[i];
            const double nwv = (double)B * 8, nb = nblocks;
            static const char* names[10] = {"norm1", "conv1 GEMM passes", "depthwise 3x3 + gate + pool", "barrier (pool)", "sca.1 GEMM", "conv3 GEMM + residual", "norm2", "conv4 GEMM + gate", "conv5 GEMM + residual", "barriers (sca, conv4)"};
            printf("naf_chain stamps: %d blocks, B=%d; shader cycles per wave and block (mean over %d waves); MFMA floor per wave: conv1 / conv4 512 x 16, conv3 / conv5 256 x 16, sca 64 x 16\n", nblocks, B, B * 8);
            for (int k = 0; k < 10; ++k) printf("  %-30s %9.0f\n", names[k], acc[k] / nwv / nb);
            printf("  %-30s %9.0f\n", "whole kernel / blocks", acc[15] / nwv / nb);
            fflush(stdout);
        }
        *ms_out = time_launches(s, iters, run);
        if (G > 1) {
            unsigned flag = 0;
            IRSDE_HIP_CHECK(hipMemcpy(&flag, naf_chain_split_error_flag(dscratch, B), 4, hipMemcpyDeviceToHost));
            if (flag) throw HipError("bench_naf_chain: the split kernel's groups were not co-resident (spin timeout)");
        }
    });
}

int irsde_bench_conv(int variant, int B, int H, int W, int Cin, int Cout, int K, int stride, int up, int epi, int iters,
                     double* ms_out) {
    return guard([&] {
        if (!ms_out || iters < 1) throw HipError("bad argument");
        const BenchSel sel = bench_conv_lookup(variant);
        const BenchRow& r = sel.row;
        const BenchKind kind = r.kind;
        const int arg = sel.arg;
        conv_global_init();
        OwnedStream stream(hipStreamNonBlocking);
        hipStream_t s = stream.s;
        Scratch mem(s);
        ConvParams p;
        p.B = B; p.Hin = H; p.Win = W; p.in_shift = up; p.C0 = Cin; p.pix0 = Cin;
        p.Cout = Cout; p.KH = K; p.KW = K; p.stride = stride; p.pad_y = p.pad_x = (K == 4 ? 1 : K / 2);
        p.Ho = ((H << up) + 2 * p.pad_y - K) / stride + 1;
        p.Wo = ((W << up) + 2 * p.pad_x - K) / stride + 1;
        const size_t nin = (size_t)B * H * W * Cin, nw = (size_t)Cout * K * K * Cin, nout = (size_t)B * p.Ho * p.Wo * Cout;
        float *din = mem.alloc<float>(nin), *dw = mem.alloc<float>(nw), *dout = mem.alloc<float>(nout), *dres = mem.alloc<float>(nout);
        float* dfilm = mem.alloc<float>((size_t)2 * Cout + 256);
        float* dz = dfilm + 2 * Cout;
        IRSDE_HIP_CHECK(hipMemset(dz, 0, 1024));
        p.zeros = dz;
        launch_fill_random(din, nin, 1, 1.0f, s);
        launch_fill_random(dw, nw, 2, 1.0f / sqrtf((float)(K * K * Cin)), s);
        launch_fill_random(dres, nout, 3, 1.0f, s);
        launch_fill_random(dfilm, (size_t)2 * Cout, 4, 0.3f, s);
        p.in0 = din; p.w = dw; p.out = dout; p.out_stride = Cout;
        if (kind == BenchKind::Conv && r.op == Operand::BF16 && !r.pair) {
            unsigned short* dbf = mem.alloc<unsigned short>(nw);
            launch_f32_to_bf16(dw, dbf, nw, s);
            p.w_bf = dbf;
        }
        if (epi == 1) { p.film = dfilm; p.silu = 1; }
        if (epi == 2) { p.silu = 1; p.res = dres; p.res_stride = Cout; }
        if (r.act_bf16) {
            unsigned short* dabf = mem.alloc<unsigned short>(nin);
            launch_f32_to_bf16(din, dabf, nin, s);
            launch_f32_to_bf16(dout, reinterpret_cast<unsigned short*>(dres), nout / 2, s);
            p.in0 = reinterpret_cast<const float*>(dabf);
            p.in_bf16 = 1; p.out_bf16 = 1;
        }
        if (r.pair) {
            const bool f16 = r.op == Operand::F16;
            unsigned short* dwp = mem.alloc<unsigned short>(2 * nw);
            launch_split_pairs(dw, dwp, (size_t)Cout, K * K * Cin, s, f16, 64.0f);
            p.w_pair = dwp; p.pair_scale = 1.0f / 64.0f; p.f16 = f16 ? 1 : 0;
        }
        if (kind == BenchKind::Split3aGemm) {
            const Split3x1Choice c = split3_1x1_choose(p, true, 2, 2, device_cu_count());
            if (!c.adopt || up || epi) throw HipError(std::string("bench_conv: variants 510 - 524 run a plain 1x1 layer: ") + (c.adopt ? "no epilogue" : c.why_not));
            unsigned short* dwt = mem.alloc<unsigned short>(split3_comp_elems((size_t)Cout, (size_t)Cin));
            launch_split_triples(dw, dwt, 1, (size_t)Cout, Cin, s);
            const Split3aArgs a = split3_1x1_args(p, dwt);
            const Split3Launch twin = split3_launch_twin(arg / 5, arg % 5);
            for (int i = 0; i < 2; ++i) launch_gemm_split3a(a, s, twin);
            *ms_out = time_launches(s, iters, [&] { launch_gemm_split3a(a, s, twin); });
            return;
        }
        if (kind == BenchKind::TripleGemm || kind == BenchKind::PairGemm) {
            if (K != 3 || stride != 1 || !wino_shape_ok(p, 4)) throw HipError("bench_conv: Winograd variants need an eligible 3x3 stride-1 layer");
            const long long T = (long long)B * (p.Ho / 4) * (p.Wo / 4);
            const bool triples = kind == BenchKind::TripleGemm;
            if (triples && !gemm_split_triples_fits(T, Cout, Cin, Cout)) throw HipError("bench_conv: shape not eligible for the three-piece GEMM");
            float *vf = mem.alloc<float>((size_t)36 * T * Cin), *uf = mem.alloc<float>((size_t)36 * Cout * Cin), *mo = mem.alloc<float>((size_t)36 * T * Cout);
            launch_fill_random(vf, (size_t)36 * T * Cin, 7, 1.0f, s);
            launch_fill_random(uf, (size_t)36 * Cout * Cin, 8, 0.05f, s);
            const SplitGemmArgs g = triples ? split_triples(mem, vf, uf, mo, (int)T, Cout, Cin, 36, s) : split_pairs(mem, vf, uf, mo, (int)T, Cout, Cin, 36, s);
            const Split3Launch twin = split3_launch_twin(arg / 5, arg % 5);
            auto gemms = [&] {
                if (triples) launch_gemm_split_triples(g, 36, s, twin);
                else launch_gemm_split_pairs(g, 36, s, arg);
            };
            for (int i = 0; i < 2; ++i) gemms();
            *ms_out = time_launches(s, iters, gemms);
            return;
        }
        float* dU = nullptr;
        WinoPlan wp{};
        if (kind == BenchKind::Fused32Stamps) {
            dU = mem.alloc<float>((size_t)36 * nw / 9);
            launch_fill_random(dU, (size_t)36 * nw / 9, 5, 1.0f / sqrtf((float)(9 * Cin)), s);
            const int nb = wino_fused_num_blocks(p);
            unsigned long long* dd = mem.alloc<unsigned long long>((size_t)nb * 128);
            launch_wino_fused(p, dU, s);
            IRSDE_HIP_CHECK(hipMemsetAsync(dd, 0, (size_t)nb * 128 * 8, s));
            launch_wino_fused(p, dU, s, dd);
            IRSDE_HIP_CHECK(hipStreamSynchronize(s));
            std::vector<unsigned long long> hd((size_t)nb * 128);
            IRSDE_HIP_CHECK(hipMemcpy(hd.data(), dd, hd.size() * 8, hipMemcpyDeviceToHost));
            double ph[2][4] = {{0, 0, 0, 0}, {0, 0, 0, 0}};
            unsigned long long rt_min = ~0ull, rt_max = 0;
            for (int bi = 0; bi < nb; ++bi)
                for (int w = 0; w < 8; ++w) {
                    const unsigned long long* t = &hd[((size_t)bi * 8 + w) * 16];
                    for (int k = 0; k < 4; ++k) ph[w >= 4][k] += (double)(t[k + 1] - t[k]) / ((double)nb * 4);
                    rt_min = std::min(rt_min, t[7]);
                    rt_max = std::max(rt_max, t[7]);
                }
            printf("wino_fused timeline B=%d %dx%d Cin=%d Cout=%d: %d blocks, block starts span %.1f us\n", B, p.Ho, p.Wo, Cin, Cout, nb,
                   (double)(rt_max - rt_min) / 100.0);
            printf("  MFMA waves     (shader cycles): start->V[0] ready %.0f | K loop %.0f | acc->LDS+barrier %.0f | epilogue %.0f\n", ph[0][0],
                   ph[0][1], ph[0][2], ph[0][3]);
            printf("  producer waves (shader cycles): start->chunk 0 done %.0f | K loop rest %.0f | wait MFMA+acc %.0f | epilogue %.0f\n",
                   ph[1][0], ph[1][1], ph[1][2], ph[1][3]);
            fflush(stdout);
            *ms_out = 0.0;
            return;
        }
        if (kind != BenchKind::Conv) {
            const bool three_launch = kind == BenchKind::Wino3 || kind == BenchKind::Wino3Gemm;
            if (K != 3 || stride != 1) throw HipError("bench_conv: Winograd variants need a 3x3 stride-1 layer");
            dU = mem.alloc<float>((size_t)36 * nw / 9);
            launch_fill_random(dU, (size_t)36 * nw / 9, 5, 1.0f / sqrtf((float)(9 * Cin)), s);
            if (!three_launch && !wino_fused_eligible(p)) throw HipError("bench_conv: shape not eligible for the fused Winograd kernel");
            if (kind != BenchKind::Fused32 && kind != BenchKind::Wino3 && !wino_fused64_eligible(p))
                throw HipError("bench_conv: shape not eligible for the 64-cout fused Winograd kernel");
            if (kind == BenchKind::Fused64 && r.op == Operand::F16) {
                float* dUp = mem.alloc<float>((size_t)36 * nw / 9);
                launch_wino_fused64_split_weights(dU, reinterpret_cast<unsigned short*>(dUp), (size_t)36 * nw / 9, 256.0f, s);
                dU = dUp;
                p.pair_scale = 1.0f / (kWinoFused64PairVScale * 256.0f);
            }
            if (three_launch) {
                if (!wino_shape_ok(p, 4)) throw HipError("bench_conv: shape not eligible for Winograd F(4x4,3x3)");
                const long long T = (long long)B * (p.Ho / 4) * (p.Wo / 4);
                float* dV = mem.alloc<float>((size_t)36 * T * Cin);
                float* dM = mem.alloc<float>((size_t)36 * T * Cout);
                wp = make_wino(p, dU, dV, dM, 4);
                if (kind == BenchKind::Wino3Gemm) launch_wino_input(wp.in, s);
            }
        }
        if (kind == BenchKind::Fused64TStamps) {
            if (!wino_fused64t_eligible(p)) throw HipError("bench_conv: shape not eligible for the two-tile-group fused Winograd kernel");
            const int nbp = 256;
            unsigned long long* dd = mem.alloc<unsigned long long>((size_t)nbp * 64);
            launch_wino_fused64t(p, dU, s, 0);
            IRSDE_HIP_CHECK(hipMemsetAsync(dd, 0, (size_t)nbp * 64 * 8, s));
            wino_fused64t_set_debug(dd);
            launch_wino_fused64t(p, dU, s, arg);
            IRSDE_HIP_CHECK(hipStreamSynchronize(s));
            wino_fused64t_set_debug(nullptr);
            std::vector<unsigned long long> hd((size_t)nbp * 64);
            IRSDE_HIP_CHECK(hipMemcpy(hd.data(), dd, hd.size() * 8, hipMemcpyDeviceToHost));
            double a5[8] = {0, 0, 0, 0, 0, 0, 0, 0};
            int nwv = 0;
            for (int bi = 0; bi < nbp; ++bi)
                for (int w = 0; w < 8; ++w) {
                    const unsigned long long* t = &hd[((size_t)bi * 8 + w) * 8];
                    if (!t[3]) continue;
                    for (int k = 0; k < 8; ++k) a5[k] += (double)t[k];
                    nwv++;
                }
            const int nst = Cin / 16;
            const double items = a5[4] / std::max(nwv, 1), chunks = items * nst;
            printf("wino4_fused64t stamps B=%d %dx%d Cin=%d Cout=%d: %.1f items x %d chunks of 16 channels per block; shader cycles per wave (mean over %d waves)\n", B, p.Ho, p.Wo, Cin,
                   Cout, items, nst, nwv);
            printf("  kernel %.0f = K loops incl. transform slices %.0f (%.0f per chunk; MFMA floor per SIMD 9216) + chunk barrier waits %.0f (%.0f per chunk) + epilogue, exchange, first-chunk transform %.0f (%.0f per item)\n",
                   a5[3] / nwv, a5[0] / nwv, a5[0] / nwv / chunks, a5[1] / nwv, a5[1] / nwv / chunks, (a5[2] + a5[5] + a5[6] + a5[7]) / nwv, (a5[2] + a5[5] + a5[6] + a5[7]) / nwv / items);
            printf("  per item: first stage + exchange writes + ring %.0f | exchange barriers + reads %.0f | second stage, stores, gathers %.0f | zero, first-chunk transform, barrier %.0f\n",
                   a5[5] / nwv / items, a5[6] / nwv / items, a5[7] / nwv / items, a5[2] / nwv / items);
            fflush(stdout);
            *ms_out = 0.0;
            return;
        }
        if (kind == BenchKind::Fused64Stamps) {
            const int nbp = 256;
            unsigned long long* dd = mem.alloc<unsigned long long>((size_t)nbp * 64);
            launch_wino_fused64(p, dU, s, 20);
            IRSDE_HIP_CHECK(hipMemsetAsync(dd, 0, (size_t)nbp * 64 * 8, s));
            wino_fused64_set_debug(dd);
            launch_wino_fused64(p, dU, s, arg);
            IRSDE_HIP_CHECK(hipStreamSynchronize(s));
            wino_fused64_set_debug(nullptr);
            std::vector<unsigned long long> hd((size_t)nbp * 64);
            IRSDE_HIP_CHECK(hipMemcpy(hd.data(), dd, hd.size() * 8, hipMemcpyDeviceToHost));
            double acc[2][5] = {{0, 0, 0, 0, 0}, {0, 0, 0, 0, 0}};
            int nw[2] = {0, 0};
            for (int bi = 0; bi < nbp; ++bi)
                for (int w = 0; w < 8; ++w) {
                    const unsigned long long* t = &hd[((size_t)bi * 8 + w) * 8];
                    if (!t[3]) continue;
                    for (int k = 0; k < 5; ++k) acc[w >= 4][k] += (double)t[k];
                    nw[w >= 4]++;
                }
            const int nchk = Cin / 32;
            const double items = acc[0][4] / std::max(nw[0], 1), chunks = acc[1][4] / std::max(nw[1], 1);
            printf("wino4_fused64p stamps B=%d %dx%d Cin=%d Cout=%d: %.1f items x %d chunks per block; shader cycles per wave (mean over %d + %d waves)\n", B, p.Ho, p.Wo,
                   Cin, Cout, items, nchk, nw[0], nw[1]);
            printf("  MFMA waves    : kernel %.0f = K-loop compute %.0f (%.0f per chunk; MFMA floor 9216) + barrier wait %.0f (%.0f per chunk) + epilogue %.0f (%.0f per item)\n",
                   acc[0][3] / nw[0], acc[0][0] / nw[0], acc[0][0] / nw[0] / (items * nchk), acc[0][1] / nw[0], acc[0][1] / nw[0] / (items * nchk), acc[0][2] / nw[0],
                   acc[0][2] / nw[0] / items);
            printf("  producer waves: kernel %.0f = load issue %.0f (%.0f per chunk) + data wait, transform, LDS writes %.0f (%.0f per chunk) + barrier wait %.0f (%.0f per chunk)\n",
                   acc[1][3] / nw[1], acc[1][0] / nw[1], acc[1][0] / nw[1] / chunks, acc[1][1] / nw[1], acc[1][1] / nw[1] / chunks, acc[1][2] / nw[1], acc[1][2] / nw[1] / chunks);
            fflush(stdout);
            *ms_out = 0.0;
            return;
        }
        const ConvTune tune = kind == BenchKind::Conv ? conv_tune_from_code(arg) : ConvTune{};
        auto run = [&] {
            switch (kind) {
            case BenchKind::Fused32: launch_wino_fused(p, dU, s, nullptr, arg); break;
            case BenchKind::Fused64T: launch_wino_fused64t(p, dU, s, arg); break;
            case BenchKind::Fused64: launch_wino_fused64(p, dU, s, arg); break;
            case BenchKind::Wino3:
                launch_wino_input(wp.in, s);
                launch_conv(wp.gemm, s);
                launch_wino_output(wp.out, s);
                break;
            case BenchKind::Wino3Gemm: launch_conv(wp.gemm, s); break;
            default: launch_conv(p, s, tune); break;
            }
        };
        for (int i = 0; i < 2; ++i) run();
        *ms_out = time_launches(s, iters, run);
    });
}

int irsde_debug_lpips_tap(irsde_engine* e, const float* in, int B, int H, int W, int normalize, int tap, float* dst, int64_t dims[4], void* stream) {
    return guard([&] {
        if (!e || !in || !dims) throw HipError("debug_lpips_tap: null argument");
        if (!lpips_engine(e)) throw HipError("debug_lpips_tap: not an LPIPS engine (irsde_create_lpips)");
        if (!e->finalized) throw HipError("debug_lpips_tap: weights not finalized");
        if (B < 1 || tap < 1 || tap > 5) throw HipError("debug_lpips_tap: B must be positive and tap in 1..5");
        const LpipsGeom g = lpips_geometry(H, W);
        dims[0] = B; dims[1] = g.h[tap - 1]; dims[2] = g.w[tap - 1]; dims[3] = kLpipsLayers[tap - 1].cout;
        if (!dst) return;
        std::lock_guard<std::mutex> lk(e->mu);
        DeviceScope dev_scope(e->cfg.device);
        hipStream_t s = reinterpret_cast<hipStream_t>(stream);
        float* ws = lpips_workspace(e, B, H, W);
        float* taps[5];
        lpips_features(e->lpips, in, nullptr, B, H, W, normalize, ws, taps, s, nullptr);
        IRSDE_HIP_CHECK(hipMemcpyAsync(dst, taps[tap - 1], (size_t)dims[0] * dims[1] * dims[2] * dims[3] * sizeof(float), hipMemcpyDeviceToDevice, s));
        IRSDE_HIP_CHECK(hipStreamSynchronize(s));
    });
}

}
```

image_restoration_sde_amd/csrc/gemm_split.hip:

```cpp
#include "common.h"
#include <algorithm>
#include <atomic>
#include <type_traits>

namespace irsde {

typedef float floatx16 __attribute__((ext_vector_type(16)));
typedef __bf16 bf16x8 __attribute__((ext_vector_type(8)));
typedef _Float16 f16x8 __attribute__((ext_vector_type(8)));
typedef unsigned uintx4 __attribute__((ext_vector_type(4)));
typedef float floatx4 __attribute__((ext_vector_type(4)));

namespace {

constexpr int SG_BK = 32;

#define IRSDE_GLDS16(GPTR, LPTR) \
    __builtin_amdgcn_global_load_lds((const __attribute__((address_space(1))) void*)(GPTR), (__attribute__((address_space(3))) void*)(LPTR), 16, 0, 0)

template <int ABL = 0, bool F16 = false>
__global__ __launch_bounds__(512, 2) void gemm_split2i_kernel(const SplitGemmArgs g) {
    using frag_t = typename std::conditional<F16, f16x8, bf16x8>::type;
    constexpr int TM = 4, TN = 2, WN = 4, BM = 256, BN = 256;
    constexpr int A_STAGE = BM * 128, STAGE = (BM + BN) * 128;
    extern __shared__ __attribute__((aligned(16))) char lds[];
    const int tid = threadIdx.x, lane = tid & 63;
    const int wave = __builtin_amdgcn_readfirstlane(tid >> 6);
    const int wm = wave / WN, wn = wave % WN;
    const int l31 = lane & 31, h = lane >> 5;
    const int mtiles = (g.M + BM - 1) / BM;
    const int units = mtiles * g.n_inner;
    const int xcd = blockIdx.x & 7, jx = blockIdx.x >> 3;
    const int ulo = (int)((long long)xcd * units / 8), uhi = (int)((long long)(xcd + 1) * units / 8);
    const int unit = ulo + jx / g.nblk_n;
    if (unit >= uhi) return;
    const int nblk = jx % g.nblk_n;
    const int plane0 = unit / mtiles, mblk = unit - plane0 * mtiles;
    const int m0 = mblk * BM, n0 = nblk * BN;
    const int nk = g.K / SG_BK;
    const int steps = nk;
    const unsigned rowb = (unsigned)nk * 128u;

    unsigned a_voff[4], b_voff[4];
#pragma unroll
    for (int ps = 0; ps < 4; ++ps) {
        const int row = (ps * 8 + wave) * 8 + (lane >> 3);
        const unsigned pc = (unsigned)((lane & 7) ^ ((row >> 1) & 7)) * 16u;
        int m = m0 + row;
        m = m < g.M ? m : g.M - 1;
        a_voff[ps] = (unsigned)m * rowb + pc;
        int n = n0 + row;
        n = n < g.N ? n : g.N - 1;
        b_voff[ps] = (unsigned)n * rowb + pc;
    }
    const char* abase = reinterpret_cast<const char*>(g.a);
    const char* bbase = reinterpret_cast<const char*>(g.b);
    const long long pA2 = g.pA * 4, pB2 = g.pB * 4;
    int kb = 0;
    const char* acomp = abase + (long long)plane0 * pA2;
    const char* bcomp = bbase + (long long)plane0 * pB2;
    auto issue_loads = [&](int buf) {
        char* la = lds + buf * STAGE + wave * 1024;
        const char* ga = acomp + kb * 128;
        const char* gb = bcomp + kb * 128;
#pragma unroll
        for (int ps = 0; ps < 4; ++ps) IRSDE_GLDS16(ga + a_voff[ps], la + ps * 8192);
#pragma unroll
        for (int ps = 0; ps < 4; ++ps) IRSDE_GLDS16(gb + b_voff[ps], la + A_STAGE + ps * 8192);
    };

    auto issue_loads_part = [&](int buf, int part) {
        char* la = lds + buf * STAGE + wave * 1024;
        const char* ga = acomp + kb * 128;
        const char* gb = bcomp + kb * 128;
        if (part == 0) {
            IRSDE_GLDS16(ga + a_voff[0], la);
            IRSDE_GLDS16(ga + a_voff[1], la + 8192);
            IRSDE_GLDS16(ga + a_voff[2], la + 2 * 8192);
        } else if (part == 1) {
            IRSDE_GLDS16(ga + a_voff[3], la + 3 * 8192);
            IRSDE_GLDS16(gb + b_voff[0], la + A_STAGE);
            IRSDE_GLDS16(gb + b_voff[1], la + A_STAGE + 8192);
        } else {
            IRSDE_GLDS16(gb + b_voff[2], la + A_STAGE + 2 * 8192);
            IRSDE_GLDS16(gb + b_voff[3], la + A_STAGE + 3 * 8192);
        }
    };

    floatx16 acc[TM][TN];
#pragma unroll
    for (int i = 0; i < TM; ++i)
#pragma unroll
        for (int j = 0; j < TN; ++j)
#pragma unroll
            for (int r = 0; r < 16; ++r) acc[i][j][r] = 0.f;

    issue_loads(0);
    __syncthreads();

    const int wm_s = wm, wn_s = wn;
    unsigned o_voff[16];
#pragma unroll
    for (int r = 0; r < 16; ++r) o_voff[r] = (unsigned)(((r & 3) + 8 * (r >> 2) + 4 * h) * g.ldc + l31) * 4u;
    auto flush = [&](int fi) {
        const int rowb_ = m0 + wm_s * TM * 32, colb = n0 + wn_s * TN * 32;
        float* ob = g.out + (long long)(plane0 + fi) * g.pO + (long long)rowb_ * g.ldc;
        const int rows = g.M - rowb_;
        const unsigned nrec = rows <= 0 ? 0u : (unsigned)(rows < TM * 32 ? rows : TM * 32) * (unsigned)g.ldc * 4u;
        const __amdgpu_buffer_rsrc_t ro = __builtin_amdgcn_make_buffer_rsrc(ob, 0, nrec, 0x00020000);
#pragma unroll
        for (int i = 0; i < TM; ++i)
#pragma unroll
            for (int j = 0; j < TN; ++j) {
                const int colu = colb + j * 32;
                if (colu + l31 < g.N && (ABL != 4 || acc[i][j][0] == 1.2345e30f)) {
                    const int soff = (i * 32 * g.ldc + colu) * 4;
#pragma unroll
                    for (int r = 0; r < 16; ++r) {
                        const float v = F16 ? acc[i][j][r] * g.out_scale : acc[i][j][r];
                        __builtin_amdgcn_raw_buffer_store_b32(__builtin_bit_cast(unsigned, v), ro, (int)o_voff[r], soff, ABL == 5 ? 2 : 0);
                    }
                }
#pragma unroll
                for (int r = 0; r < 16; ++r) acc[i][j][r] = 0.f;
            }
    };
    const int swz = (l31 >> 1) & 7;
    int fr_off[2][2];
#pragma unroll
    for (int p = 0; p < 2; ++p)
#pragma unroll
        for (int sb = 0; sb < 2; ++sb) fr_off[p][sb] = l31 * 128 + (((p * 4 + sb * 2 + h) ^ swz) * 16);
    for (int st = 0; st < steps; ++st) {
        const int buf = st & 1;
        const bool more = st + 1 < steps;
        if (more) ++kb;
        const char* a = lds + buf * STAGE + wm * TM * 32 * 128;
        const char* b = lds + buf * STAGE + A_STAGE + wn * TN * 32 * 128;
        frag_t fa[2][2][TM], fb[2][2][TN];
#pragma unroll
        for (int sb = 0; sb < 2; ++sb)
#pragma unroll
            for (int p = 0; p < 2; ++p) {
#pragma unroll
                for (int i = 0; i < TM; ++i) fa[sb][p][i] = *reinterpret_cast<const frag_t*>(a + i * 32 * 128 + fr_off[p][sb]);
#pragma unroll
                for (int j = 0; j < TN; ++j) fb[sb][p][j] = *reinterpret_cast<const frag_t*>(b + j * 32 * 128 + fr_off[p][sb]);
            }
        __builtin_amdgcn_sched_barrier(0);
#pragma unroll
        for (int sb = 0; sb < 2; ++sb)
#pragma unroll
            for (int pr = 0; pr < 3; ++pr) {
#pragma unroll
                for (int i = 0; i < TM; ++i)
#pragma unroll
                    for (int j = 0; j < TN; ++j)
                        if (ABL != 3) {
                            if constexpr (F16) acc[i][j] = __builtin_amdgcn_mfma_f32_32x32x16_f16(fa[sb][pr == 1 ? 1 : 0][i], fb[sb][pr == 0 ? 1 : 0][j], acc[i][j], 0, 0, 0);
                            else acc[i][j] = __builtin_amdgcn_mfma_f32_32x32x16_bf16(fa[sb][pr == 1 ? 1 : 0][i], fb[sb][pr == 0 ? 1 : 0][j], acc[i][j], 0, 0, 0);
                        }
                        else acc[i][j][0] += (float)fa[sb][pr == 1 ? 1 : 0][i][0] * (float)fb[sb][pr == 0 ? 1 : 0][j][0];
                if (sb == 0 && ABL != 1 && more) issue_loads_part(buf ^ 1, pr);
                __builtin_amdgcn_sched_barrier(0);
            }
        __syncthreads();
    }
    flush(0);
}
#define IRSDE_WAIT_VM(N) asm volatile("s_waitcnt vmcnt(" #N ")" ::: "memory")
#define IRSDE_PHASE_BARRIER()                              \
    do {                                                   \
        asm volatile("s_waitcnt lgkmcnt(0)" ::: "memory"); \
        __builtin_amdgcn_s_barrier();                      \
    } while (0)
template <int ABL = 0, bool WALK = true, bool DRAIN = false>
__global__ __launch_bounds__(512, 1) void gemm_split3i_kernel(const SplitGemmArgs g) {
    constexpr int TM = 2, TN = 2, WN = 2, BM = 256, BN = 128;
    constexpr int ROWB = 192, GROUP = 16 * ROWB;
    constexpr int A_STAGE = BM * ROWB, STAGE = (BM + BN) * ROWB;
    constexpr int PA[6] = {0, 1, 2, 0, 1, 0};
    constexpr int PB[6] = {2, 1, 0, 1, 0, 0};
    extern __shared__ __attribute__((aligned(16))) char lds[];
    const int tid = threadIdx.x, lane = tid & 63;
    const int wave = __builtin_amdgcn_readfirstlane(tid >> 6);
    const int wm = wave / WN, wn = wave % WN;
    const int l31 = lane & 31, h = lane >> 5;
    const int mtiles = (g.M + BM - 1) / BM;
    const int units = mtiles * g.n_inner;
    const int xcd = blockIdx.x & 7, jx = blockIdx.x >> 3;
    const int ulo = (int)((long long)xcd * units / 8), uhi = (int)((long long)(xcd + 1) * units / 8);
    const int nitems = (uhi - ulo) * g.nblk_n;
    const int it_step = WALK ? ((int)gridDim.x - xcd + 7) >> 3 : nitems;
    int it = jx;
    if (it >= nitems) return;
    const int nk = g.K / SG_BK;
    const unsigned pairb = (unsigned)nk * 384u;

    const int ga0 = 4 * (wave >> 1) + (wave & 1);
    int plane0, m0, n0;
    unsigned a_voff[6], b_voff[3];
    const char *acomp, *bcomp;
    auto set_item = [&](int i) {
        const int unit = ulo + i / g.nblk_n, nblk = i % g.nblk_n;
        plane0 = unit / mtiles;
        m0 = (unit - plane0 * mtiles) * BM;
        n0 = nblk * BN;
#pragma unroll
        for (int q = 0; q < 9; ++q) {
            const int gi = q / 3, wl = q - gi * 3;
            const int sl = wl * 64 + lane;
            const int r = sl / 12, pos = sl - r * 12;
            int j = pos - ((r >> 2) & 3);
            j = j < 0 ? j + 12 : j;
            if (gi < 2) {
                int m = m0 + (ga0 + 2 * gi) * 16 + r;
                m = m < g.M ? m : g.M - 1;
                a_voff[q] = (unsigned)(m >> 1) * pairb + (unsigned)(m & 1) * 192u + (unsigned)j * 16u;
            } else {
                int n = n0 + wave * 16 + r;
                n = n < g.N ? n : g.N - 1;
                b_voff[wl] = (unsigned)(n >> 1) * pairb + (unsigned)(n & 1) * 192u + (unsigned)j * 16u;
            }
        }
        acomp = reinterpret_cast<const char*>(g.a) + (long long)plane0 * g.pA * 2;
        bcomp = reinterpret_cast<const char*>(g.b) + (long long)plane0 * g.pB * 2;
    };
    auto issue_unit = [&](int kb, int kind) {
        const char* gsrc = (kind < 2 ? acomp : bcomp) + (size_t)kb * 384;
        char* l = lds + (kb & 1) * STAGE + (kind < 2 ? (ga0 + 2 * kind) * GROUP : A_STAGE + wave * GROUP);
#pragma unroll
        for (int wl = 0; wl < 3; ++wl) IRSDE_GLDS16(gsrc + (kind < 2 ? a_voff[kind * 3 + wl] : b_voff[wl]), l + wl * 1024);
    };
    auto issue_one = [&](int kb, int kind, int wl) {
        const char* gsrc = (kind < 2 ? acomp : bcomp) + (size_t)kb * 384;
        char* l = lds + (kb & 1) * STAGE + (kind < 2 ? (ga0 + 2 * kind) * GROUP : A_STAGE + wave * GROUP);
        IRSDE_GLDS16(gsrc + (kind < 2 ? a_voff[kind * 3 + wl] : b_voff[wl]), l + wl * 1024);
    };
    auto issue_first = [&]() {
        issue_unit(0, 0);
        issue_unit(0, 2);
        issue_unit(0, 1);
        if (nk > 1) {
            issue_unit(1, 0);
            issue_unit(1, 2);
        }
    };

    floatx16 acc[TM][TN];
#pragma unroll
    for (int i = 0; i < TM; ++i)
#pragma unroll
        for (int j = 0; j < TN; ++j)
#pragma unroll
            for (int r = 0; r < 16; ++r) acc[i][j][r] = 0.f;

    set_item(it);
    issue_first();

    int fr_off[3][2];
#pragma unroll
    for (int p = 0; p < 3; ++p)
#pragma unroll
        for (int sb = 0; sb < 2; ++sb) fr_off[p][sb] = l31 * ROWB + ((p * 4 + sb * 2 + h + ((l31 >> 2) & 3)) % 12) * 16;
    bf16x8 fa[2][3], fb[2][3][TN];
    auto read_a = [&](int sb, const char* a) {
#pragma unroll
        for (int p = 0; p < 3; ++p) fa[sb][p] = *reinterpret_cast<const bf16x8*>(a + fr_off[p][sb]);
    };
    auto read_b = [&](int sb, const char* b) {
#pragma unroll
        for (int p = 0; p < 3; ++p)
#pragma unroll
            for (int j = 0; j < TN; ++j) fb[sb][p][j] = *reinterpret_cast<const bf16x8*>(b + j * 32 * ROWB + fr_off[p][sb]);
    };
    const bool late = wave >= 4;
    const int a_base = wm * TM * 32 * ROWB, b_base = A_STAGE + wn * TN * 32 * ROWB;
    for (;;) {
        IRSDE_WAIT_VM(0);
        IRSDE_PHASE_BARRIER();
        read_a(0, lds + a_base);
        read_b(0, lds + b_base);
        __builtin_amdgcn_sched_barrier(0);
        for (int st = 0; st < nk; ++st) {
            const bool more1 = st + 1 < nk, more2 = st + 2 < nk;
            const char* a = lds + (st & 1) * STAGE + a_base;
            const char* b = lds + (st & 1) * STAGE + b_base;
            const char* an = lds + ((st + 1) & 1) * STAGE + a_base;
            const char* bn = lds + ((st + 1) & 1) * STAGE + b_base;
#pragma unroll
            for (int i = 0; i < TM; ++i) {
                if (i == 1) {
                    read_a(0, a + 32 * ROWB);
                    __builtin_amdgcn_sched_barrier(0);
                }
#pragma unroll
                for (int sb = 0; sb < 2; ++sb)
#pragma unroll
                    for (int pr = 0; pr < 6; ++pr) {
#pragma unroll
                        for (int j = 0; j < TN; ++j) {
                            if (ABL != 3) acc[i][j] = __builtin_amdgcn_mfma_f32_32x32x16_bf16(fa[sb][PA[pr]], fb[sb][PB[pr]][j], acc[i][j], 0, 0, 0);
                            else acc[i][j][0] += (float)fa[sb][PA[pr]][0] * (float)fb[sb][PB[pr]][j][0];
                        }
                        __builtin_amdgcn_sched_barrier(0);
                        if (sb == 0 && pr == 0) {
                            if (i == 0) {
                                read_a(1, a);
                                read_b(1, b);
                            } else {
                                read_a(1, a + 32 * ROWB);
                            }
                        }
                        if (i == 1 && sb == 1 && pr == 0 && more1) {
                            read_a(0, an);
                            read_b(0, bn);
                        }
                        if (ABL != 1 && (sb == 1) == late) {
                            if (i == 0 && pr >= 1 && pr <= 3 && more1) issue_one(st + 1, 1, pr - 1);
                            if (i == 1 && more2) issue_one(st + 2, pr < 3 ? 0 : 2, pr % 3);
                        }
                        __builtin_amdgcn_sched_barrier(0);
                    }
                if (DRAIN || (i == 0 && !more1)) IRSDE_WAIT_VM(0);
                else if (i == 0) IRSDE_WAIT_VM(3);
                IRSDE_PHASE_BARRIER();
            }
        }

        const int rowb_ = m0 + wm * TM * 32, colb = n0 + wn * TN * 32;
        float* ob = g.out + (long long)plane0 * g.pO + (long long)rowb_ * g.ldc;
        const int rows = g.M - rowb_;
        const unsigned nrec = rows <= 0 ? 0u : (unsigned)(rows < TM * 32 ? rows : TM * 32) * (unsigned)g.ldc * 4u;
        const __amdgpu_buffer_rsrc_t ro = __builtin_amdgcn_make_buffer_rsrc(ob, 0, nrec, 0x00020000);
        it += it_step;
        const bool next = WALK && it < nitems;
        if (next) {
            set_item(it);
            issue_first();
            __builtin_amdgcn_sched_barrier(0);
        }
#pragma unroll
        for (int i = 0; i < TM; ++i)
#pragma unroll
            for (int j = 0; j < TN; ++j) {
                const int colu = colb + j * 32;
                if (colu + l31 < g.N && (ABL != 4 || acc[i][j][0] == 1.2345e30f)) {
#pragma unroll
                    for (int r = 0; r < 16; ++r) {
                        const float v = acc[i][j][r];
                        const unsigned voff = (unsigned)((i * 32 + (r & 3) + 8 * (r >> 2) + 4 * h) * g.ldc + colu + l31) * 4u;
                        __builtin_amdgcn_raw_buffer_store_b32(__builtin_bit_cast(unsigned, v), ro, (int)voff, 0, 0);
                    }
                }
            }
        if (!next) break;
#pragma unroll
        for (int i = 0; i < TM; ++i)
#pragma unroll
            for (int j = 0; j < TN; ++j)
#pragma unroll
                for (int r = 0; r < 16; ++r) acc[i][j][r] = 0.f;
    }
}
template <int ABL = 0, bool WALK = true, bool DRAIN = false>
__global__ __launch_bounds__(512, 1) void gemm_split3a_kernel(const Split3aArgs g) {
    constexpr int TN = 4, BM = 256, BN = 128;
    constexpr int AROW = 128, BROW = 192;
    constexpr int A_STAGE = BM * AROW, B_HALF = 64 * BROW, STAGE = A_STAGE + 2 * B_HALF;
    constexpr int PA[6] = {0, 1, 2, 0, 1, 0};
    constexpr int PB[6] = {2, 1, 0, 1, 0, 0};
    extern __shared__ __attribute__((aligned(16))) char lds[];
    const int tid = threadIdx.x, lane = tid & 63;
    const int wave = __builtin_amdgcn_readfirstlane(tid >> 6);
    const int l31 = lane & 31, h = lane >> 5;
    const int units = (g.M + BM - 1) / BM;
    const int xcd = blockIdx.x & 7, jx = blockIdx.x >> 3;
    const int ulo = (int)((long long)xcd * units / 8), uhi = (int)((long long)(xcd + 1) * units / 8);
    const int nitems = (uhi - ulo) * g.nblk_n;
    const int it_step = WALK ? ((int)gridDim.x - xcd + 7) >> 3 : nitems;
    int it = jx;
    if (it >= nitems) return;
    const int nk0 = g.C0 / SG_BK, nk = (g.C0 + g.C1) / SG_BK;
    const unsigned pairb = (unsigned)nk * 384u;

    int m0, n0;
    unsigned a_voff0[4], a_voff1[4], b_voff[2][2];
    float bias_r[TN];
    auto set_item = [&](int i) {
        const int unit = ulo + i / g.nblk_n, nblk = i % g.nblk_n;
        m0 = unit * BM;
        n0 = nblk * BN;
#pragma unroll
        for (int ps = 0; ps < 4; ++ps) {
            const int row = (ps * 8 + wave) * 8 + (lane >> 3);
            const unsigned pc = (unsigned)((lane & 7) ^ ((row >> 1) & 7)) * 16u;
            int m = m0 + row;
            m = m < g.M ? m : g.M - 1;
            a_voff0[ps] = (unsigned)m * (unsigned)g.pix0 * 4u + pc;
            a_voff1[ps] = (unsigned)m * (unsigned)g.pix1 * 4u + pc;
        }
#pragma unroll
        for (int hb = 0; hb < 2; ++hb)
#pragma unroll
            for (int wl = 0; wl < 2; ++wl) {
                const int sl = wl * 32 + lane;
                const int r = sl / 12, pos = sl - r * 12;
                const int rowt = wave * 8 + r;
                int j = pos - ((rowt >> 2) & 3);
                j = j < 0 ? j + 12 : j;
                int n = n0 + hb * 64 + rowt;
                n = n < g.N ? n : g.N - 1;
                b_voff[hb][wl] = (unsigned)(n >> 1) * pairb + (unsigned)(n & 1) * 192u + (unsigned)j * 16u;
            }
        if (g.bias) {
#pragma unroll
            for (int j = 0; j < TN; ++j) {
                int n = n0 + j * 32 + l31;
                n = n < g.N ? n : g.N - 1;
                bias_r[j] = g.bias[n];
            }
        }
    };
    auto issue_a = [&](int kb, int ps) {
        const bool second = kb >= nk0;
        const char* gsrc = second ? reinterpret_cast<const char*>(g.in1) + (size_t)(kb - nk0) * 128 : reinterpret_cast<const char*>(g.in0) + (size_t)kb * 128;
        IRSDE_GLDS16(gsrc + (second ? a_voff1[ps] : a_voff0[ps]), lds + (kb & 1) * STAGE + (ps * 8 + wave) * 1024);
    };
    auto issue_b = [&](int kb, int hb, int wl) {
        const char* gsrc = reinterpret_cast<const char*>(g.w3) + (size_t)kb * 384;
        IRSDE_GLDS16(gsrc + b_voff[hb][wl], lds + (kb & 1) * STAGE + A_STAGE + hb * B_HALF + wave * 8 * BROW + wl * 512);
    };
    auto issue_first = [&]() {
        issue_b(0, 0, 0); issue_b(0, 0, 1);
#pragma unroll
        for (int ps = 0; ps < 4; ++ps) issue_a(0, ps);
        issue_b(0, 1, 0); issue_b(0, 1, 1);
        if (nk > 1) {
#pragma unroll
            for (int ps = 0; ps < 4; ++ps) issue_a(1, ps);
            issue_b(1, 0, 0); issue_b(1, 0, 1);
        }
    };

    floatx16 acc[TN];
#pragma unroll
    for (int j = 0; j < TN; ++j)
#pragma unroll
        for (int r = 0; r < 16; ++r) acc[j][r] = 0.f;

    set_item(it);
    issue_first();

    const int swz = (l31 >> 1) & 7;
    int fa_off[2][2], fr_off[3][2];
#pragma unroll
    for (int sb = 0; sb < 2; ++sb)
#pragma unroll
        for (int e = 0; e < 2; ++e) fa_off[sb][e] = l31 * AROW + (((2 * (2 * sb + h) + e) ^ swz) * 16);
#pragma unroll
    for (int p = 0; p < 3; ++p)
#pragma unroll
        for (int sb = 0; sb < 2; ++sb) fr_off[p][sb] = l31 * BROW + ((p * 4 + sb * 2 + h + ((l31 >> 2) & 3)) % 12) * 16;
    bf16x8 fa[2][3], fb[2][3][2];
    floatx4 ra[2];
    auto read_a = [&](int sb, const char* a) {
#pragma unroll
        for (int e = 0; e < 2; ++e) ra[e] = *reinterpret_cast<const floatx4*>(a + fa_off[sb][e]);
    };
    auto split_a = [&](int sb) {
#pragma unroll
        for (int e = 0; e < 8; ++e) {
            float r = ra[e >> 2][e & 3];
#pragma unroll
            for (int p = 0; p < 3; ++p) {
                const __bf16 hb = (__bf16)r;
                fa[sb][p][e] = hb;
                r -= (float)hb;
            }
        }
    };
    auto read_b = [&](int sb, const char* b) {
#pragma unroll
        for (int p = 0; p < 3; ++p)
#pragma unroll
            for (int j = 0; j < 2; ++j) fb[sb][p][j] = *reinterpret_cast<const bf16x8*>(b + j * 32 * BROW + fr_off[p][sb]);
    };
    const bool late = wave >= 4;
    const int a_base = wave * 32 * AROW;
    for (;;) {
        IRSDE_WAIT_VM(0);
        IRSDE_PHASE_BARRIER();
        read_a(0, lds + a_base);
        read_b(0, lds + A_STAGE);
        split_a(0);
        __builtin_amdgcn_sched_barrier(0);
        for (int st = 0; st < nk; ++st) {
            const bool more1 = st + 1 < nk, more2 = st + 2 < nk;
            const char* a = lds + (st & 1) * STAGE + a_base;
            const char* b = lds + (st & 1) * STAGE + A_STAGE;
            const char* an = lds + ((st + 1) & 1) * STAGE + a_base;
            const char* bn = lds + ((st + 1) & 1) * STAGE + A_STAGE;
#pragma unroll
            for (int i = 0; i < 2; ++i) {
                if (i == 1) {
                    read_b(0, b + B_HALF);
                    __builtin_amdgcn_sched_barrier(0);
                }
#pragma unroll
                for (int sb = 0; sb < 2; ++sb)
#pragma unroll
                    for (int pr = 0; pr < 6; ++pr) {
#pragma unroll
                        for (int j = 0; j < 2; ++j) {
                            if (ABL != 3) acc[2 * i + j] = __builtin_amdgcn_mfma_f32_32x32x16_bf16(fa[sb][PA[pr]], fb[sb][PB[pr]][j], acc[2 * i + j], 0, 0, 0);
                            else acc[2 * i + j][0] += (float)fa[sb][PA[pr]][0] * (float)fb[sb][PB[pr]][j][0];
                        }
                        __builtin_amdgcn_sched_barrier(0);
                        if (sb == 0 && pr == 0) {
                            if (i == 0) {
                                read_a(1, a);
                                read_b(1, b);
                            } else {
                                read_b(1, b + B_HALF);
                            }
                        }
                        if (i == 0 && sb == 0 && pr == 3) split_a(1);
                        if (i == 1 && sb == 1 && more1) {
                            if (pr == 0) {
                                read_a(0, an);
                                read_b(0, bn);
                            }
                            if (pr == 3) split_a(0);
                        }
                        if (ABL != 1 && (sb == 1) == late) {
                            if (i == 0 && pr >= 1 && pr <= 2 && more1) issue_b(st + 1, 1, pr - 1);
                            if (i == 1 && more2) {
                                if (pr < 4) issue_a(st + 2, pr);
                                else issue_b(st + 2, 0, pr - 4);
                            }
                        }
                        __builtin_amdgcn_sched_barrier(0);
                    }
                if (DRAIN || (i == 0 && !more1)) IRSDE_WAIT_VM(0);
                else if (i == 0) IRSDE_WAIT_VM(2);
                IRSDE_PHASE_BARRIER();
            }
        }

        if (g.bias) {
#pragma unroll
            for (int j = 0; j < TN; ++j)
#pragma unroll
                for (int r = 0; r < 16; ++r) acc[j][r] += bias_r[j];
        }
        const int rowb_ = m0 + wave * 32, colb = n0;
        float* ob = g.out + (long long)rowb_ * g.out_stride;
        const int rows = g.M - rowb_;
        const unsigned nrec = rows <= 0 ? 0u : (unsigned)(rows < 32 ? rows : 32) * (unsigned)g.out_stride * 4u;
        const __amdgpu_buffer_rsrc_t ro = __builtin_amdgcn_make_buffer_rsrc(ob, 0, nrec, 0x00020000);
        it += it_step;
        const bool next = WALK && it < nitems;
        if (next) {
            __builtin_amdgcn_sched_barrier(0);
            set_item(it);
            issue_first();
            __builtin_amdgcn_sched_barrier(0);
        }
#pragma unroll
        for (int j = 0; j < TN; ++j) {
            const int colu = colb + j * 32;
            if (colu + l31 < g.N && (ABL != 4 || acc[j][0] == 1.2345e30f)) {
#pragma unroll
                for (int r = 0; r < 16; ++r) {
                    const float v = acc[j][r];
                    const unsigned voff = (unsigned)(((r & 3) + 8 * (r >> 2) + 4 * h) * g.out_stride + colu + l31) * 4u;
                    __builtin_amdgcn_raw_buffer_store_b32(__builtin_bit_cast(unsigned, v), ro, (int)voff, 0, 0);
                }
            }
        }
        if (!next) break;
#pragma unroll
        for (int j = 0; j < TN; ++j)
#pragma unroll
            for (int r = 0; r < 16; ++r) acc[j][r] = 0.f;
    }
}
#undef IRSDE_PHASE_BARRIER
#undef IRSDE_WAIT_VM
#undef IRSDE_GLDS16

__global__ __launch_bounds__(256) void split_triples_kernel(const float* __restrict__ in, unsigned short* __restrict__ out, const size_t n, const size_t rows,
                                                            const int K) {
    const size_t i = (size_t)blockIdx.x * blockDim.x + threadIdx.x;
    if (i >= n) return;
    const size_t rk = rows * (size_t)K;
    const size_t z = i / rk, rem = i - z * rk;
    const size_t row = rem / K;
    const int k = (int)(rem - row * K);
    float r = in[i];
    unsigned short* o = out + z * split3_comp_elems(rows, K);
#pragma unroll
    for (int p = 0; p < 3; ++p) {
        const __bf16 hb = (__bf16)r;
        o[split3_index(row, k, p, K / 32)] = __builtin_bit_cast(unsigned short, hb);
        r -= (float)hb;
    }
}

template <bool F16>
__global__ __launch_bounds__(256) void split_pairs_kernel(const float* __restrict__ in, unsigned short* __restrict__ out, const size_t n, const int K,
                                                          const float scale) {
    const size_t i = (size_t)blockIdx.x * blockDim.x + threadIdx.x;
    if (i >= n) return;
    const size_t row = i / K;
    const int k = (int)(i - row * K);
    float r = in[i];
    const size_t base = (row * (size_t)(K / 32) + k / 32) * 64 + (k & 31);
    if constexpr (F16) {
        r *= scale;
        const _Float16 hb = (_Float16)r;
        out[base] = __builtin_bit_cast(unsigned short, hb);
        r -= (float)hb;
        const _Float16 lb = (_Float16)r;
        out[base + 32] = __builtin_bit_cast(unsigned short, lb);
    } else {
        const __bf16 hb = (__bf16)r;
        out[base] = __builtin_bit_cast(unsigned short, hb);
        r -= (float)hb;
        const __bf16 lb = (__bf16)r;
        out[base + 32] = __builtin_bit_cast(unsigned short, lb);
    }
}

template <int NPL, bool F16 = false>
__global__ __launch_bounds__(256) void split_planes_kernel(const float* __restrict__ in, unsigned short* __restrict__ out, const size_t n,
                                                           const size_t plane, const float scale) {
    const size_t i = (size_t)blockIdx.x * blockDim.x + threadIdx.x;
    if (i >= n) return;
    float r = F16 ? in[i] * scale : in[i];
#pragma unroll
    for (int p = 0; p < NPL; ++p) {
        if constexpr (F16) {
            const _Float16 hb = (_Float16)r;
            out[p * plane + i] = __builtin_bit_cast(unsigned short, hb);
            r -= (float)hb;
        } else {
            const __bf16 hb = (__bf16)r;
            out[p * plane + i] = __builtin_bit_cast(unsigned short, hb);
            r -= (float)hb;
        }
    }
}

__global__ __launch_bounds__(256) void split_frag3_kernel(const float* __restrict__ in, unsigned short* __restrict__ out, const size_t n, const int K) {
    const size_t i = (size_t)blockIdx.x * blockDim.x + threadIdx.x;
    if (i >= n) return;
    const size_t row = i / K;
    const int k = (int)(i - row * K);
    float r = in[i];
    const size_t o = attn_frag3_index(row, k, K);
#pragma unroll
    for (int p = 0; p < 3; ++p) {
        const __bf16 hb = (__bf16)r;
        out[p * n + o] = __builtin_bit_cast(unsigned short, hb);
        r -= (float)hb;
    }
}

}

void launch_split_frag3(const float* in, unsigned short* out, size_t rows, int K, hipStream_t s) {
    if (rows % 32 || K % 16) throw HipError("split_frag3: rows must be a multiple of 32, K of 16");
    const size_t n = rows * (size_t)K;
    hipLaunchKernelGGL(split_frag3_kernel, dim3((unsigned)((n + 255) / 256)), dim3(256), 0, s, in, out, n, K);
    IRSDE_HIP_CHECK(hipGetLastError());
}

void gemm_split_global_init() {
    IRSDE_HIP_CHECK(hipFuncSetAttribute(reinterpret_cast<const void*>(gemm_split2i_kernel<0>), hipFuncAttributeMaxDynamicSharedMemorySize, 160 * 1024));
    IRSDE_HIP_CHECK(hipFuncSetAttribute(reinterpret_cast<const void*>(gemm_split2i_kernel<0, true>), hipFuncAttributeMaxDynamicSharedMemorySize, 160 * 1024));
    IRSDE_HIP_CHECK(hipFuncSetAttribute(reinterpret_cast<const void*>(gemm_split2i_kernel<5, true>), hipFuncAttributeMaxDynamicSharedMemorySize, 160 * 1024));
    IRSDE_HIP_CHECK(hipFuncSetAttribute(reinterpret_cast<const void*>(gemm_split2i_kernel<1>), hipFuncAttributeMaxDynamicSharedMemorySize, 160 * 1024));
    IRSDE_HIP_CHECK(hipFuncSetAttribute(reinterpret_cast<const void*>(gemm_split2i_kernel<3>), hipFuncAttributeMaxDynamicSharedMemorySize, 160 * 1024));
    IRSDE_HIP_CHECK(hipFuncSetAttribute(reinterpret_cast<const void*>(gemm_split2i_kernel<4>), hipFuncAttributeMaxDynamicSharedMemorySize, 160 * 1024));
    IRSDE_HIP_CHECK(hipFuncSetAttribute(reinterpret_cast<const void*>(gemm_split3i_kernel<0, true>), hipFuncAttributeMaxDynamicSharedMemorySize, 160 * 1024));
    IRSDE_HIP_CHECK(hipFuncSetAttribute(reinterpret_cast<const void*>(gemm_split3i_kernel<0, false>), hipFuncAttributeMaxDynamicSharedMemorySize, 160 * 1024));
    IRSDE_HIP_CHECK(hipFuncSetAttribute(reinterpret_cast<const void*>(gemm_split3i_kernel<0, true, true>), hipFuncAttributeMaxDynamicSharedMemorySize, 160 * 1024));
    IRSDE_HIP_CHECK(hipFuncSetAttribute(reinterpret_cast<const void*>(gemm_split3a_kernel<0, true>), hipFuncAttributeMaxDynamicSharedMemorySize, 160 * 1024));
    IRSDE_HIP_CHECK(hipFuncSetAttribute(reinterpret_cast<const void*>(gemm_split3a_kernel<0, false>), hipFuncAttributeMaxDynamicSharedMemorySize, 160 * 1024));
    IRSDE_HIP_CHECK(hipFuncSetAttribute(reinterpret_cast<const void*>(gemm_split3a_kernel<0, true, true>), hipFuncAttributeMaxDynamicSharedMemorySize, 160 * 1024));
#ifdef IRSDE_PROBES
    for (const void* f : {reinterpret_cast<const void*>(gemm_split3a_kernel<1, true>), reinterpret_cast<const void*>(gemm_split3a_kernel<3, true>),
                          reinterpret_cast<const void*>(gemm_split3a_kernel<4, true>), reinterpret_cast<const void*>(gemm_split3a_kernel<1, false>),
                          reinterpret_cast<const void*>(gemm_split3a_kernel<3, false>), reinterpret_cast<const void*>(gemm_split3a_kernel<4, false>),
                          reinterpret_cast<const void*>(gemm_split3a_kernel<1, true, true>), reinterpret_cast<const void*>(gemm_split3a_kernel<3, true, true>),
                          reinterpret_cast<const void*>(gemm_split3a_kernel<4, true, true>)})
        IRSDE_HIP_CHECK(hipFuncSetAttribute(f, hipFuncAttributeMaxDynamicSharedMemorySize, 160 * 1024));
    IRSDE_HIP_CHECK(hipFuncSetAttribute(reinterpret_cast<const void*>(gemm_split3i_kernel<1, true>), hipFuncAttributeMaxDynamicSharedMemorySize, 160 * 1024));
    IRSDE_HIP_CHECK(hipFuncSetAttribute(reinterpret_cast<const void*>(gemm_split3i_kernel<3, true>), hipFuncAttributeMaxDynamicSharedMemorySize, 160 * 1024));
    IRSDE_HIP_CHECK(hipFuncSetAttribute(reinterpret_cast<const void*>(gemm_split3i_kernel<4, true>), hipFuncAttributeMaxDynamicSharedMemorySize, 160 * 1024));
    IRSDE_HIP_CHECK(hipFuncSetAttribute(reinterpret_cast<const void*>(gemm_split3i_kernel<1, false>), hipFuncAttributeMaxDynamicSharedMemorySize, 160 * 1024));
    IRSDE_HIP_CHECK(hipFuncSetAttribute(reinterpret_cast<const void*>(gemm_split3i_kernel<3, false>), hipFuncAttributeMaxDynamicSharedMemorySize, 160 * 1024));
    IRSDE_HIP_CHECK(hipFuncSetAttribute(reinterpret_cast<const void*>(gemm_split3i_kernel<4, false>), hipFuncAttributeMaxDynamicSharedMemorySize, 160 * 1024));
    IRSDE_HIP_CHECK(hipFuncSetAttribute(reinterpret_cast<const void*>(gemm_split3i_kernel<1, true, true>), hipFuncAttributeMaxDynamicSharedMemorySize, 160 * 1024));
    IRSDE_HIP_CHECK(hipFuncSetAttribute(reinterpret_cast<const void*>(gemm_split3i_kernel<3, true, true>), hipFuncAttributeMaxDynamicSharedMemorySize, 160 * 1024));
    IRSDE_HIP_CHECK(hipFuncSetAttribute(reinterpret_cast<const void*>(gemm_split3i_kernel<4, true, true>), hipFuncAttributeMaxDynamicSharedMemorySize, 160 * 1024));
#endif
}

void launch_gemm_split_pairs(const SplitGemmArgs& a, int ncomp, hipStream_t s, int abl, bool f16) {
    if (a.K % SG_BK) throw HipError("gemm_split_pairs: K must be a multiple of 32");
    if ((unsigned long long)a.M * a.K * 4ull >= 0xffffffffull || (unsigned long long)a.N * a.K * 4ull >= 0xffffffffull ||
        (size_t)a.M * a.ldc * 4 >= 0xffffffffull)
        throw HipError("gemm_split_pairs: a component exceeds the 32-bit offset range");
    SplitGemmArgs g = a;
    g.nblk_n = (a.N + 255) / 256;
    g.n_inner = ncomp;
    const int units = ((a.M + 255) / 256) * ncomp;
    int per_xcd = 0;
    for (int x = 0; x < 8; ++x) per_xcd = std::max(per_xcd, (int)((long long)(x + 1) * units / 8) - (int)((long long)x * units / 8));
    const dim3 grid((unsigned)(8 * per_xcd * g.nblk_n));
    const size_t lds = (size_t)2 * 512 * 128;
    if (f16) {
        if (abl != 0) throw HipError("gemm_split_pairs: the ablation twins exist for the bf16 kernel only");
        static const bool nt = tuning_env_int("IRSDE_SPLIT_NT", 0) != 0;
        if (nt) hipLaunchKernelGGL((gemm_split2i_kernel<5, true>), grid, dim3(512), lds, s, g);
        else hipLaunchKernelGGL((gemm_split2i_kernel<0, true>), grid, dim3(512), lds, s, g);
        IRSDE_HIP_CHECK(hipGetLastError());
        return;
    }
    switch (abl) {
        case 0: hipLaunchKernelGGL(gemm_split2i_kernel<0>, grid, dim3(512), lds, s, g); break;
        case 1: hipLaunchKernelGGL(gemm_split2i_kernel<1>, grid, dim3(512), lds, s, g); break;
        case 3: hipLaunchKernelGGL(gemm_split2i_kernel<3>, grid, dim3(512), lds, s, g); break;
        case 4: hipLaunchKernelGGL(gemm_split2i_kernel<4>, grid, dim3(512), lds, s, g); break;
        default: throw HipError("gemm_split_pairs: bad ablation variant");
    }
    IRSDE_HIP_CHECK(hipGetLastError());
}

bool gemm_split_triples_fits(long long M, long long N, long long K, long long ldc) {
    if (M < 1 || N < 1 || K < 32 || K % SG_BK) return false;
    return (unsigned long long)split3_comp_elems((size_t)M, (size_t)K) * 2ull < 0xffffffffull && (unsigned long long)split3_comp_elems((size_t)N, (size_t)K) * 2ull < 0xffffffffull &&
           (unsigned long long)M * ldc * 4ull < 0xffffffffull;
}

static std::atomic<int> g_force_split3_blocks{-1};
void set_force_split3_blocks(int n) { g_force_split3_blocks.store(n >= 8 ? n : -1, std::memory_order_relaxed); }

template <int ABL>
static void launch_split3_abl(bool walk, bool drain, dim3 grid, size_t lds, hipStream_t s, const SplitGemmArgs& g) {
    if (drain) hipLaunchKernelGGL((gemm_split3i_kernel<ABL, true, true>), grid, dim3(512), lds, s, g);
    else if (walk) hipLaunchKernelGGL((gemm_split3i_kernel<ABL, true>), grid, dim3(512), lds, s, g);
    else hipLaunchKernelGGL((gemm_split3i_kernel<ABL, false>), grid, dim3(512), lds, s, g);
}
void launch_gemm_split_triples(const SplitGemmArgs& a, int ncomp, hipStream_t s, const Split3Launch& o) {
    if (a.K % SG_BK) throw HipError("gemm_split_triples: K must be a multiple of 32");
    if (!gemm_split_triples_fits(a.M, a.N, a.K, a.ldc)) throw HipError("gemm_split_triples: a component exceeds the 32-bit offset range");
    if (ncomp < 1 || a.ldc < a.N) throw HipError("gemm_split_triples: bad component count or output stride");
    static const bool walk_knob = tuning_env_int("IRSDE_SPLIT3_WALK", 1) != 0, drain_knob = tuning_env_int("IRSDE_SPLIT3_DRAIN", 0) != 0;
    const bool walk = o.walk == Split3Launch::RULE ? walk_knob : o.walk == Split3Launch::ON;
    const bool drain = o.drain == Split3Launch::RULE ? drain_knob : o.drain == Split3Launch::ON;
    if (drain && !walk) throw HipError("gemm_split_triples: the drain twin exists on the walk only");
    SplitGemmArgs g = a;
    g.nblk_n = (a.N + 127) / 128;
    g.n_inner = ncomp;
    const long long units = (long long)((a.M + 255) / 256) * ncomp;
    long long per_xcd = 0;
    for (int x = 0; x < 8; ++x) per_xcd = std::max(per_xcd, (x + 1) * units / 8 - x * units / 8);
    long long blocks = 8 * per_xcd * g.nblk_n;
    if (blocks >= 0x7fffffffll) throw HipError("gemm_split_triples: grid too large");
    if (walk) {
        const int forced = g_force_split3_blocks.load(std::memory_order_relaxed);
        blocks = std::min<long long>(blocks, std::max(8, forced > 0 ? forced : device_cu_count()));
    }
    const dim3 grid((unsigned)blocks);
    const size_t lds = (size_t)2 * (256 + 128) * 192;
    switch (o.abl) {
        case Split3Launch::FULL: launch_split3_abl<0>(walk, drain, grid, lds, s, g); break;
#ifdef IRSDE_PROBES
        case Split3Launch::NO_LOADS: launch_split3_abl<1>(walk, drain, grid, lds, s, g); break;
        case Split3Launch::NO_MFMA: launch_split3_abl<3>(walk, drain, grid, lds, s, g); break;
        case Split3Launch::NO_STORES: launch_split3_abl<4>(walk, drain, grid, lds, s, g); break;
#endif
        default: throw HipError("gemm_split_triples: the ablation twins are part of the PROBES build");
    }
    IRSDE_HIP_CHECK(hipGetLastError());
}

bool gemm_split3a_fits(const Split3aArgs& a, const char** why_not) {
    const char* why = nullptr;
    const unsigned long long lim = 0xffffffffull;
    const long long K = (long long)a.C0 + a.C1;
    if (a.M < 1 || a.N < 1) why = "empty";
    else if (a.C0 < 32 || a.C0 % SG_BK) why = "C0 not a multiple of 32";
    else if (a.C1 < 0 || a.C1 % SG_BK) why = "C1 not a multiple of 32";
    else if (a.pix0 < a.C0 || a.pix0 % 4 || (a.C1 && (a.pix1 < a.C1 || a.pix1 % 4)) || a.out_stride < a.N) why = "bad stride";
    else if ((unsigned long long)a.M * a.pix0 * 4ull >= lim || (unsigned long long)a.M * a.pix1 * 4ull >= lim ||
             (unsigned long long)split3_comp_elems((size_t)a.N, (size_t)K) * 2ull >= lim || 32ull * a.out_stride * 4ull >= lim)
        why = "beyond the 32-bit offset range";
    if (why_not) *why_not = why;
    return !why;
}

int gemm_split3a_blocks(long long M, int N, int cus, bool walk) {
    const long long units = (M + 255) / 256;
    long long per_xcd = 0;
    for (int x = 0; x < 8; ++x) per_xcd = std::max(per_xcd, (x + 1) * units / 8 - x * units / 8);
    long long blocks = 8 * per_xcd * ((N + 127) / 128);
    if (walk) blocks = std::min<long long>(blocks, std::max(8, cus));
    return blocks >= 0x7fffffffll ? -1 : (int)blocks;
}

Split3aArgs split3_1x1_args(const ConvParams& p, const unsigned short* w3) {
    Split3aArgs a;
    a.in0 = p.in0; a.C0 = p.C0; a.pix0 = p.pix0;
    a.in1 = p.C1 ? p.in1 : nullptr; a.C1 = p.C1; a.pix1 = p.C1 ? p.pix1 : 0;
    a.w3 = w3; a.bias = p.bias; a.out = p.out;
    a.M = p.B * p.Ho * p.Wo; a.N = p.Cout; a.out_stride = p.out_stride;
    return a;
}

static constexpr long long kSplit3x1MinRows = 2048;
static constexpr int kSplit3x1MinK = 128, kSplit3x1MinCout = 128;
static constexpr double kSplit3x1MinFlop = 1e10;
Split3x1Choice split3_1x1_choose(const ConvParams& p, bool exact_f32, int master, int knob, int cus) {
    Split3x1Choice c;
    const long long M = (long long)p.B * p.Ho * p.Wo;
    const char* why = nullptr;
    if (!exact_f32) why = "not the exact-fp32 engine";
    else if (master <= 0) why = "IRSDE_SPLIT3 = 0";
    else if (knob <= 0) why = "IRSDE_SPLIT3_1X1 = 0";
    else if (p.KH != 1 || p.KW != 1) why = "not a 1x1 convolution";
    else if (p.stride != 1) why = "stride";
    else if (p.in_shift) why = "in_shift";
    else if (p.pad_y || p.pad_x) why = "padding";
    else if (p.film) why = "film";
    else if (p.silu) why = "silu";
    else if (p.res) why = "res";
    else if (p.in_scale) why = "in_scale";
    else if (p.ch_scale) why = "ch_scale";
    else if (p.gate || p.gate_film) why = "gate";
    else if (p.shuffle) why = "shuffle";
    else if (p.ln_g) why = "ln_g";
    else if (p.in_bf16 || p.out_bf16 || p.in_f16 || p.out_f16) why = "16-bit storage";
    else if (p.w_bf || p.w_pair) why = "16-bit operands";
    else if (p.splits > 1) why = "split-K";
    else if (p.nz != 1) why = "batched";
    else if (M < 1 || M >= 0x7fffffffll) why = "empty";
    else gemm_split3a_fits(split3_1x1_args(p, nullptr), &why);
    if (!why && knob == 1) {
        const int K = p.C0 + p.C1;
        if (M < kSplit3x1MinRows) why = "rule: rows";
        else if (K < kSplit3x1MinK) why = "rule: K";
        else if (p.Cout < kSplit3x1MinCout) why = "rule: Cout";
        else if (2.0 * (double)M * K * p.Cout < kSplit3x1MinFlop) why = "rule: FLOP";
    }
    if (why) {
        c.why_not = why;
        return c;
    }
    c.adopt = true;
    c.grid = gemm_split3a_blocks(M, p.Cout, cus, true);
    c.lds = (int)kSplit3aLds;
    return c;
}

template <int ABL>
static void launch_split3a_abl(bool walk, bool drain, dim3 grid, hipStream_t s, const Split3aArgs& g) {
    if (drain) hipLaunchKernelGGL((gemm_split3a_kernel<ABL, true, true>), grid, dim3(512), kSplit3aLds, s, g);
    else if (walk) hipLaunchKernelGGL((gemm_split3a_kernel<ABL, true>), grid, dim3(512), kSplit3aLds, s, g);
    else hipLaunchKernelGGL((gemm_split3a_kernel<ABL, false>), grid, dim3(512), kSplit3aLds, s, g);
}
void launch_gemm_split3a(const Split3aArgs& a, hipStream_t s, const Split3Launch& o) {
    const char* why = nullptr;
    if (!gemm_split3a_fits(a, &why)) throw HipError(std::string("gemm_split3a: ") + why);
    if (!a.in0 || (a.C1 && !a.in1) || !a.w3 || !a.out) throw HipError("gemm_split3a: null operand");
    const bool walk = o.walk != Split3Launch::OFF, drain = o.drain == Split3Launch::ON;
    if (drain && !walk) throw HipError("gemm_split3a: the drain twin exists on the walk only");
    Split3aArgs g = a;
    g.nblk_n = (a.N + 127) / 128;
    const int forced = g_force_split3_blocks.load(std::memory_order_relaxed);
    const int blocks = gemm_split3a_blocks(a.M, a.N, forced > 0 ? forced : device_cu_count(), walk);
    if (blocks < 1) throw HipError("gemm_split3a: grid too large");
    const dim3 grid((unsigned)blocks);
    switch (o.abl) {
        case Split3Launch::FULL: launch_split3a_abl<0>(walk, drain, grid, s, g); break;
#ifdef IRSDE_PROBES
        case Split3Launch::NO_LOADS: launch_split3a_abl<1>(walk, drain, grid, s, g); break;
        case Split3Launch::NO_MFMA: launch_split3a_abl<3>(walk, drain, grid, s, g); break;
        case Split3Launch::NO_STORES: launch_split3a_abl<4>(walk, drain, grid, s, g); break;
#endif
        default: throw HipError("gemm_split3a: the ablation twins are part of the PROBES build");
    }
    IRSDE_HIP_CHECK(hipGetLastError());
}

void launch_split_triples(const float* in, unsigned short* out, int ncomp, size_t rows, int K, hipStream_t s) {
    if (K % 32 || ncomp < 1 || rows < 1) throw HipError("split_triples: K must be a multiple of 32");
    const size_t n = (size_t)ncomp * rows * (size_t)K;
    hipLaunchKernelGGL(split_triples_kernel, dim3((unsigned)((n + 255) / 256)), dim3(256), 0, s, in, out, n, rows, K);
    IRSDE_HIP_CHECK(hipGetLastError());
}

void launch_split_pairs(const float* in, unsigned short* out, size_t rows, int K, hipStream_t s, bool f16, float scale) {
    if (K % 32) throw HipError("split_pairs: K must be a multiple of 32");
    const size_t n = rows * (size_t)K;
    if (f16) hipLaunchKernelGGL(split_pairs_kernel<true>, dim3((unsigned)((n + 255) / 256)), dim3(256), 0, s, in, out, n, K, scale);
    else hipLaunchKernelGGL(split_pairs_kernel<false>, dim3((unsigned)((n + 255) / 256)), dim3(256), 0, s, in, out, n, K, 1.0f);
    IRSDE_HIP_CHECK(hipGetLastError());
}

void launch_split_planes(const float* in, unsigned short* out, size_t n, size_t plane, int nplanes, hipStream_t s, bool f16, float scale) {
    const dim3 grid((unsigned)((n + 255) / 256));
    if (f16 && nplanes != 2) throw HipError("split_planes: fp16 pieces come in pairs");
    if (f16) hipLaunchKernelGGL((split_planes_kernel<2, true>), grid, dim3(256), 0, s, in, out, n, plane, scale);
    else if (nplanes == 2) hipLaunchKernelGGL((split_planes_kernel<2, false>), grid, dim3(256), 0, s, in, out, n, plane, 1.0f);
    else throw HipError("split_planes: 2 planes");
    IRSDE_HIP_CHECK(hipGetLastError());
}

}
```

include/irsde_hip_debug.h:

```cpp
#ifndef IRSDE_HIP_DEBUG_H
#define IRSDE_HIP_DEBUG_H

#include "irsde_hip.h"

#ifdef __cplusplus
extern "C" {
#endif

int irsde_debug_conv(const float* in0, int C0, const float* in1, int C1, int B, int Hin, int Win, int in_shift,
                     const float* w_oihw, int Cout, int KH, int KW, int stride, int pad, const float* bias,
                     const float* film, int film_bstride, int silu, const float* res, float* out, int naive,
                     int splits, void* stream);

int irsde_debug_conv_choice(int B, int Hin, int Win, int C0, int C1, int Cout, int K, int stride, int pad, int in_shift, int operand, int storage, int pair,
                            unsigned features, int splits, int nz, int tune, int cu_count, const int* knobs, char* out, int out_len);

int irsde_debug_conv_halo_choice(int B, int Hin, int Win, int C0, int C1, int Cout, int K, int stride, int pad, int in_shift, int operand, int storage, int pair,
                                 unsigned features, int splits, int nz, int tune, int halo2, int nslow, char* out, int out_len);

int irsde_debug_conv_features(const float* in0, int C0, const float* in1, int C1, int B, int Hin, int Win, int in_shift, const float* w_oihw, int Cout, int K,
                              int stride, int pad, int operand, int storage, int pair, const float* bias, const float* ch_scale, const float* ln_g,
                              const float* film, int film_bstride, const float* res, const float* in_scale, const float* gate_film, int gate_film_bstride,
                              int silu, int gate, int shuffle, int nz, int splits, int tune, const int* knobs, float* out, char* choice, int choice_len,
                              void* stream);

int irsde_debug_split_gemm(const float* A, const float* B, float* C, int M, int N, int K, int ncomp, int nplanes, void* stream);

int irsde_bench_conv(int variant, int B, int H, int W, int Cin, int Cout, int K, int stride, int up, int epi, int iters,
                     double* ms_out);
int irsde_bench_naf_chain(int variant, int nblocks, int B, int iters, double* ms_out);
int irsde_debug_force_subbatches(int n);
int irsde_debug_force_chain_groups(int g);
int irsde_debug_force_wino_poly(int mode);
int irsde_debug_force_split3(int mode);
int irsde_debug_force_split3_attn(int mode);
int irsde_debug_force_split3_blocks(int n);
int irsde_debug_force_split3_1x1(int mode);
int irsde_debug_split3_1x1(const float* in0, int C0, int pix0, const float* in1, int C1, int pix1, const float* w, const float* bias, float* out, int M, int N,
                           int out_stride, int mode, void* stream);
int irsde_debug_split3_1x1_choice(int B, int Hin, int Win, int C0, int C1, int Cout, int K, int stride, int pad, int in_shift, int operand, int storage, int pair,
                                  unsigned features, int splits, int nz, int engine_flags, int master, int knob, int cu_count, char* out, int out_len);

int irsde_debug_scam(const float* x, int B_pairs, int H, int W, int C, const float* norm_l_g, const float* norm_r_g, const float* l_proj1_w,
                     const float* l_proj1_b, const float* r_proj1_w, const float* r_proj1_b, const float* l_proj2_w, const float* l_proj2_b,
                     const float* r_proj2_w, const float* r_proj2_b, const float* beta, const float* gamma, float* out, void* stream);

int irsde_debug_naf_gate_sca(const float* u, int B, int H, int W, int c, const float* conv2_w, const float* conv2_b, const float* sca_w, const float* sca_b,
                             float* gated_out, float* mean_out, float* s_out, void* stream);
int irsde_debug_tlsc(const float* g, int B, int h, int w, int c, int k1, int k2, float* pooled_out, const float* scale_map, float* scaled_out, void* stream);
int irsde_debug_ln_film(const float* x, long long M, int C, long long ppi, const float* g, const float* fscale, const float* fshift, int film_bstride,
                        float* out, void* stream);
int irsde_debug_naf_lnconv(int mode, const float* x, long long M, int c, int Cout, long long ppi, const float* g, const float* fscale, const float* fshift,
                           int film_bstride, const float* w, const float* bias, const float* gate_film, int gate_film_bstride, const float* in_scale,
                           const float* ch_scale, const float* res, float* out, void* stream);

int irsde_debug_naf_chain(const float* x, float* out, int B, int nblocks, const float* norm1_g, const float* conv1_w, const float* conv1_b, const float* conv2_w,
                          const float* conv2_b, const float* sca_w, const float* sca_b, const float* conv3_w, const float* conv3_b, const float* beta,
                          const float* norm2_g, const float* conv4_w, const float* conv4_b, const float* conv5_w, const float* conv5_b, const float* gamma,
                          const float* film, int film_bstride, int film_off, const float* cam, int cam_bstride, int cam_off, int groups, void* stream);
int irsde_debug_naf_chain_split_order(int nblocks, int groups, int* order_out, long long n);

int irsde_debug_full_attention16(const void* qkv_bf16, int B, int N, void* out_bf16, void* stream);

int irsde_debug_scam_full(const float* x, int B_pairs, int H, int W, int C, const float* norm_l_g, const float* norm_r_g, const float* l_proj1_w,
                          const float* l_proj1_b, const float* r_proj1_w, const float* r_proj1_b, const float* l_proj2_w, const float* l_proj2_b,
                          const float* r_proj2_w, const float* r_proj2_b, const float* beta, const float* gamma, float* out, void* stream);

int irsde_debug_scam_stream(const float* x, int B_pairs, int H, int W, int C, const float* norm_l_g, const float* norm_r_g, const float* l_proj1_w,
                            const float* l_proj1_b, const float* r_proj1_w, const float* r_proj1_b, const float* l_proj2_w, const float* l_proj2_b,
                            const float* r_proj2_w, const float* r_proj2_b, const float* beta, const float* gamma, int block_w, float* out, void* stream);
int irsde_debug_scam_full_stream(const float* x, int B_pairs, int H, int W, int C, const float* norm_l_g, const float* norm_r_g, const float* l_proj1_w,
                                 const float* l_proj1_b, const float* r_proj1_w, const float* r_proj1_b, const float* l_proj2_w, const float* l_proj2_b,
                                 const float* r_proj2_w, const float* r_proj2_b, const float* beta, const float* gamma, int block_w, float* out,
                                 void* stream);
int irsde_debug_force_scam_stream(int block_w);

int irsde_debug_lpips_tap(irsde_engine* e, const float* in, int B, int H, int W, int normalize, int tap, float* dst, int64_t dims[4], void* stream);

#ifdef __cplusplus
}
#endif
#endif
```

Before: 5.081 images/s.

## Add 16x16x32 MFMA twins of split3 GEMM kernels and enable by default

Adds M16 variants of the bf16-triple split GEMM kernels (split3i and split3a) that use 16x16x32 MFMA instructions instead of 32x32 ones. The LDS rotation and swizzle patterns are changed to match the new fragment layout, and the accumulators and epilogue are reorganized into floatx4 tiles. kSplit3MfmaDefault=1 makes this path the default, which is meant to improve MFMA throughput or latency hiding in the fp32-emulating split GEMMs. The cost is more MFMA instructions and different LDS access patterns that may create bank conflicts, along with extra template instantiations.

```diff
diff --git a/image_restoration_sde_amd/_lib.py b/image_restoration_sde_amd/_lib.py
--- a/image_restoration_sde_amd/_lib.py
+++ b/image_restoration_sde_amd/_lib.py
@@ -39,7 +39,7 @@
     "irsde_last_error", "irsde_version", "irsde_create", "irsde_create_nafnet", "irsde_destroy", "irsde_num_weights",
     "irsde_weight_name", "irsde_weight_shape", "irsde_load_weight", "irsde_finalize_weights",
     "irsde_set_schedule", "irsde_unet_forward", "irsde_sample", "irsde_sde_step", "irsde_philox_normal",
-    "irsde_get_profile", "irsde_debug_tap", "irsde_work_model", "irsde_debug_conv", "irsde_debug_conv_choice", "irsde_debug_conv_halo_choice", "irsde_debug_conv_features", "irsde_plan_describe", "irsde_bench_conv", "irsde_op_profile", "irsde_debug_split_gemm", "irsde_bench_naf_chain", "irsde_debug_force_subbatches", "irsde_debug_force_chain_groups", "irsde_debug_force_wino_poly", "irsde_debug_force_split3", "irsde_debug_force_split3_attn", "irsde_debug_force_split3_blocks", "irsde_debug_force_split3_1x1", "irsde_debug_split3_1x1", "irsde_debug_split3_1x1_choice", "irsde_debug_scam", "irsde_debug_scam_full",
+    "irsde_get_profile", "irsde_debug_tap", "irsde_work_model", "irsde_debug_conv", "irsde_debug_conv_choice", "irsde_debug_conv_halo_choice", "irsde_debug_conv_features", "irsde_plan_describe", "irsde_bench_conv", "irsde_op_profile", "irsde_debug_split_gemm", "irsde_bench_naf_chain", "irsde_debug_force_subbatches", "irsde_debug_force_chain_groups", "irsde_debug_force_wino_poly", "irsde_debug_force_split3", "irsde_debug_force_split3_attn", "irsde_debug_force_split3_blocks", "irsde_debug_force_split3_mfma", "irsde_debug_split3_m16_read_offset", "irsde_debug_force_split3_1x1", "irsde_debug_split3_1x1", "irsde_debug_split3_1x1_choice", "irsde_debug_scam", "irsde_debug_scam_full",
     "irsde_debug_scam_stream", "irsde_debug_scam_full_stream", "irsde_debug_force_scam_stream",
     "irsde_debug_naf_gate_sca", "irsde_debug_tlsc", "irsde_debug_ln_film", "irsde_debug_naf_lnconv", "irsde_debug_naf_chain", "irsde_debug_naf_chain_split_order",
     "irsde_debug_full_attention16",
@@ -138,6 +138,8 @@
     lib.irsde_debug_split3_1x1.argtypes = [P, c.c_int, c.c_int, P, c.c_int, c.c_int, P, P, P, c.c_int, c.c_int, c.c_int, c.c_int, P]
     lib.irsde_debug_split3_1x1_choice.argtypes = [c.c_int] * 13 + [c.c_uint] + [c.c_int] * 6 + [c.c_char_p, c.c_int]
     lib.irsde_debug_force_split3_blocks.argtypes = [c.c_int]
+    lib.irsde_debug_force_split3_mfma.argtypes = [c.c_int]
+    lib.irsde_debug_split3_m16_read_offset.argtypes = [c.c_int, c.c_int, c.c_int]
     lib.irsde_debug_scam.argtypes = [P, c.c_int, c.c_int, c.c_int, c.c_int] + [P] * 12 + [P, P]
     lib.irsde_debug_scam_full.argtypes = [P, c.c_int, c.c_int, c.c_int, c.c_int] + [P] * 12 + [P, P]
     lib.irsde_debug_scam_stream.argtypes = [P, c.c_int, c.c_int, c.c_int, c.c_int] + [P] * 12 + [c.c_int, P, P]
diff --git a/image_restoration_sde_amd/csrc/common.h b/image_restoration_sde_amd/csrc/common.h
--- a/image_restoration_sde_amd/csrc/common.h
+++ b/image_restoration_sde_amd/csrc/common.h
@@ -137,7 +137,11 @@
     Abl abl = FULL;
     Tri walk = RULE;
     Tri drain = RULE;
-};
+    Tri mfma16 = RULE;
+};
+constexpr int kSplit3MfmaDefault = 1;
+void set_force_split3_mfma(int shape);
+int split3_m16_read_offset(int kind, int lane, int sel);
 void launch_gemm_split_triples(const SplitGemmArgs& a, int ncomp, hipStream_t s, const Split3Launch& o = {});
 void set_force_split3_blocks(int n);
 bool gemm_split_triples_fits(long long M, long long N, long long K, long long ldc);
diff --git a/image_restoration_sde_amd/csrc/engine_debug.hip b/image_restoration_sde_amd/csrc/engine_debug.hip
--- a/image_restoration_sde_amd/csrc/engine_debug.hip
+++ b/image_restoration_sde_amd/csrc/engine_debug.hip
@@ -88,6 +88,10 @@
 
 Split3Launch split3_launch_twin(int twin, int abl = 0) {
     Split3Launch o;
+    if (twin >= 3) {
+        o.mfma16 = Split3Launch::ON;
+        twin -= 3;
+    }
     o.abl = static_cast<Split3Launch::Abl>(abl);
     o.walk = twin == 0 ? Split3Launch::RULE : twin == 1 ? Split3Launch::OFF : Split3Launch::ON;
     o.drain = twin == 0 ? Split3Launch::RULE : twin == 1 ? Split3Launch::OFF : Split3Launch::ON;
@@ -201,6 +205,8 @@
     bench(472, 476, BenchKind::PairGemm, 0),
     bench(490, 504, BenchKind::TripleGemm, 0),
     bench(510, 524, BenchKind::Split3aGemm, 0),
+    bench(530, 544, BenchKind::TripleGemm, 15),
+    bench(550, 564, BenchKind::Split3aGemm, 15),
 };
 
 template <class Row, size_t N, class Lo, class Hi>
@@ -930,8 +936,8 @@
 
 int irsde_debug_split_gemm(const float* A, const float* Bm, float* C, int M, int N, int K, int ncomp, int nplanes, void* stream) {
     return guard([&] {
-        const int twin3 = nplanes == 43 ? 0 : nplanes == 45 ? 1 : nplanes == 47 ? 2 : -1;
-        if (twin3 < 0 && nplanes != 42 && nplanes != 44) throw HipError("debug_split_gemm: nplanes must be 42, 43, 44, 45 or 47");
+        const int twin3 = nplanes == 43 ? 0 : nplanes == 45 ? 1 : nplanes == 47 ? 2 : nplanes == 53 ? 3 : nplanes == 55 ? 4 : nplanes == 57 ? 5 : -1;
+        if (twin3 < 0 && nplanes != 42 && nplanes != 44) throw HipError("debug_split_gemm: nplanes must be 42, 43, 44, 45, 47, 53, 55 or 57");
         hipStream_t s = reinterpret_cast<hipStream_t>(stream);
         conv_global_init();
         Scratch mem(s);
@@ -968,7 +974,7 @@
 int irsde_debug_split3_1x1(const float* in0, int C0, int pix0, const float* in1, int C1, int pix1, const float* w, const float* bias, float* out, int M, int N,
                            int out_stride, int mode, void* stream) {
     return guard([&] {
-        if (!in0 || !w || !out || (C1 && !in1) || mode < 0 || mode > 2) throw HipError("debug_split3_1x1: bad argument");
+        if (!in0 || !w || !out || (C1 && !in1) || mode < 0 || mode > 5) throw HipError("debug_split3_1x1: bad argument");
         hipStream_t s = reinterpret_cast<hipStream_t>(stream);
         conv_global_init();
         Split3aArgs a;
@@ -1000,6 +1006,16 @@
     if (n >= 0 && n < 8) return guard([&] { throw HipError("debug_force_split3_blocks: n must be at least 8 (one block per XCD), or negative for the default"); });
     set_force_split3_blocks(n);
     return IRSDE_OK;
+}
+
+int irsde_debug_force_split3_mfma(int shape) {
+    set_force_split3_mfma(shape);
+    return IRSDE_OK;
+}
+
+int irsde_debug_split3_m16_read_offset(int kind, int lane, int sel) {
+    if (kind < 0 || kind > 1 || lane < 0 || lane > 63 || sel < 0 || sel > (kind ? 1 : 2)) return -1;
+    return split3_m16_read_offset(kind, lane, sel);
 }
 
 int irsde_debug_force_wino_poly(int mode) {
@@ -1164,7 +1180,7 @@
         }
         if (kind == BenchKind::Split3aGemm) {
             const Split3x1Choice c = split3_1x1_choose(p, true, 2, 2, device_cu_count());
-            if (!c.adopt || up || epi) throw HipError(std::string("bench_conv: variants 510 - 524 run a plain 1x1 layer: ") + (c.adopt ? "no epilogue" : c.why_not));
+            if (!c.adopt || up || epi) throw HipError(std::string("bench_conv: variants 510 - 524 and 550 - 564 run a plain 1x1 layer: ") + (c.adopt ? "no epilogue" : c.why_not));
             unsigned short* dwt = mem.alloc<unsigned short>(split3_comp_elems((size_t)Cout, (size_t)Cin));
             launch_split_triples(dw, dwt, 1, (size_t)Cout, Cin, s);
             const Split3aArgs a = split3_1x1_args(p, dwt);
diff --git a/image_restoration_sde_amd/csrc/gemm_split.hip b/image_restoration_sde_amd/csrc/gemm_split.hip
--- a/image_restoration_sde_amd/csrc/gemm_split.hip
+++ b/image_restoration_sde_amd/csrc/gemm_split.hip
@@ -1,6 +1,7 @@
 #include "common.h"
 #include <algorithm>
 #include <atomic>
+#include <initializer_list>
 #include <type_traits>
 
 namespace irsde {
@@ -10,6 +11,15 @@
 typedef _Float16 f16x8 __attribute__((ext_vector_type(8)));
 typedef unsigned uintx4 __attribute__((ext_vector_type(4)));
 typedef float floatx4 __attribute__((ext_vector_type(4)));
+
+__host__ __device__ constexpr int split3_rot(int row, bool m16) { return m16 ? 2 * ((row >> 2) & 3) : (row >> 2) & 3; }
+__host__ __device__ constexpr int split3a_swz(int row, bool m16) { return m16 ? ((row >> 1) & 1) | (row & 4) : (row >> 1) & 7; }
+__host__ __device__ constexpr int split3_m16_frag_off(int lane, int plane) {
+    return (lane & 15) * 192 + ((plane * 4 + (lane >> 4) + split3_rot(lane & 15, true)) % 12) * 16;
+}
+__host__ __device__ constexpr int split3a_m16_frag_off(int lane, int e) {
+    return (lane & 15) * 128 + ((2 * (lane >> 4) + e) ^ split3a_swz(lane & 15, true)) * 16;
+}
 
 namespace {
 
@@ -174,7 +184,7 @@
         asm volatile("s_waitcnt lgkmcnt(0)" ::: "memory"); \
         __builtin_amdgcn_s_barrier();                      \
     } while (0)
-template <int ABL = 0, bool WALK = true, bool DRAIN = false>
+template <int ABL = 0, bool WALK = true, bool DRAIN = false, bool M16 = false>
 __global__ __launch_bounds__(512, 1) void gemm_split3i_kernel(const SplitGemmArgs g) {
     constexpr int TM = 2, TN = 2, WN = 2, BM = 256, BN = 128;
     constexpr int ROWB = 192, GROUP = 16 * ROWB;
@@ -211,7 +221,7 @@
             const int gi = q / 3, wl = q - gi * 3;
             const int sl = wl * 64 + lane;
             const int r = sl / 12, pos = sl - r * 12;
-            int j = pos - ((r >> 2) & 3);
+            int j = pos - split3_rot(r, M16);
             j = j < 0 ? j + 12 : j;
             if (gi < 2) {
                 int m = m0 + (ga0 + 2 * gi) * 16 + r;
@@ -247,13 +257,26 @@
         }
     };
 
-    floatx16 acc[TM][TN];
-#pragma unroll
-    for (int i = 0; i < TM; ++i)
-#pragma unroll
-        for (int j = 0; j < TN; ++j)
-#pragma unroll
-            for (int r = 0; r < 16; ++r) acc[i][j][r] = 0.f;
+    floatx16 acc[M16 ? 1 : TM][M16 ? 1 : TN];
+    floatx4 acc16[M16 ? 2 : 1][2][4];
+    auto zero_acc = [&]() {
+        if constexpr (M16) {
+#pragma unroll
+            for (int i = 0; i < 2; ++i)
+#pragma unroll
+                for (int t = 0; t < 2; ++t)
+#pragma unroll
+                    for (int j = 0; j < 4; ++j) acc16[i][t][j] = floatx4{0.f, 0.f, 0.f, 0.f};
+        } else {
+#pragma unroll
+            for (int i = 0; i < TM; ++i)
+#pragma unroll
+                for (int j = 0; j < TN; ++j)
+#pragma unroll
+                    for (int r = 0; r < 16; ++r) acc[i][j][r] = 0.f;
+        }
+    };
+    zero_acc();
 
     set_item(it);
     issue_first();
@@ -262,17 +285,21 @@
 #pragma unroll
     for (int p = 0; p < 3; ++p)
 #pragma unroll
-        for (int sb = 0; sb < 2; ++sb) fr_off[p][sb] = l31 * ROWB + ((p * 4 + sb * 2 + h + ((l31 >> 2) & 3)) % 12) * 16;
+        for (int sb = 0; sb < 2; ++sb)
+            fr_off[p][sb] = l31 * ROWB + ((p * 4 + sb * 2 + h + split3_rot(l31, false)) % 12) * 16;
+    int fr16[3];
+#pragma unroll
+    for (int p = 0; p < 3; ++p) fr16[p] = split3_m16_frag_off(lane, p);
     bf16x8 fa[2][3], fb[2][3][TN];
-    auto read_a = [&](int sb, const char* a) {
-#pragma unroll
-        for (int p = 0; p < 3; ++p) fa[sb][p] = *reinterpret_cast<const bf16x8*>(a + fr_off[p][sb]);
-    };
-    auto read_b = [&](int sb, const char* b) {
+    auto read_a = [&](int set, const char* a) {
+#pragma unroll
+        for (int p = 0; p < 3; ++p) fa[set][p] = *reinterpret_cast<const bf16x8*>(a + (M16 ? fr16[p] : fr_off[p][set]));
+    };
+    auto read_b = [&](int set, const char* b) {
 #pragma unroll
         for (int p = 0; p < 3; ++p)
 #pragma unroll
-            for (int j = 0; j < TN; ++j) fb[sb][p][j] = *reinterpret_cast<const bf16x8*>(b + j * 32 * ROWB + fr_off[p][sb]);
+            for (int j = 0; j < TN; ++j) fb[set][p][j] = *reinterpret_cast<const bf16x8*>(b + j * (M16 ? 16 : 32) * ROWB + (M16 ? fr16[p] : fr_off[p][set]));
     };
     const bool late = wave >= 4;
     const int a_base = wm * TM * 32 * ROWB, b_base = A_STAGE + wn * TN * 32 * ROWB;
@@ -294,6 +321,33 @@
                     read_a(0, a + 32 * ROWB);
                     __builtin_amdgcn_sched_barrier(0);
                 }
+                if constexpr (M16) {
+#pragma unroll
+                    for (int sg = 0; sg < 4; ++sg)
+#pragma unroll
+                        for (int pr = 0; pr < 6; ++pr) {
+                            const int s = sg >> 1, t16 = sg & 1;
+#pragma unroll
+                            for (int j = 0; j < TN; ++j) {
+                                if (ABL != 3)
+                                    acc16[i][t16][2 * s + j] = __builtin_amdgcn_mfma_f32_16x16x32_bf16(fa[t16][PA[pr]], fb[s][PB[pr]][j], acc16[i][t16][2 * s + j], 0, 0, 0);
+                                else acc16[i][t16][2 * s + j][0] += (float)fa[t16][PA[pr]][0] * (float)fb[s][PB[pr]][j][0];
+                            }
+                            __builtin_amdgcn_sched_barrier(0);
+                            if (sg == 0 && pr == 0) read_a(1, a + (32 * i + 16) * ROWB);
+                            if (i == 0 && sg == 1 && pr == 0) read_b(1, b + 32 * ROWB);
+                            if (i == 1 && more1 && pr == 0) {
+                                if (sg == 2) read_b(0, bn);
+                                if (sg == 3) read_a(0, an);
+                            }
+                            if (ABL != 1 && (s == 1) == late && !(pr & 1)) {
+                                const int lq = t16 * 3 + (pr >> 1);
+                                if (i == 0 && lq >= 1 && lq <= 3 && more1) issue_one(st + 1, 1, lq - 1);
+                                if (i == 1 && more2) issue_one(st + 2, lq < 3 ? 0 : 2, lq % 3);
+                            }
+                            __builtin_amdgcn_sched_barrier(0);
+                        }
+                } else
 #pragma unroll
                 for (int sb = 0; sb < 2; ++sb)
 #pragma unroll
@@ -340,6 +394,28 @@
             issue_first();
             __builtin_amdgcn_sched_barrier(0);
         }
+        if constexpr (M16) {
+            const int l15 = lane & 15, r4 = 4 * (lane >> 4);
+            int ldc = g.ldc;
+            asm volatile("" : "+s"(ldc));
+#pragma unroll
+            for (int i = 0; i < 2; ++i)
+#pragma unroll
+                for (int t = 0; t < 2; ++t)
+#pragma unroll
+                    for (int j = 0; j < 4; ++j) {
+                        const int col = colb + j * 16 + l15;
+                        if (col < g.N && (ABL != 4 || acc16[i][t][j][0] == 1.2345e30f)) {
+#pragma unroll
+                            for (int r = 0; r < 4; ++r) {
+                                const float v = acc16[i][t][j][r];
+                                const unsigned voff = (unsigned)((i * 32 + t * 16 + r4 + r) * ldc + col) * 4u;
+                                __builtin_amdgcn_raw_buffer_store_b32(__builtin_bit_cast(unsigned, v), ro, (int)voff, 0, 0);
+                            }
+                        }
+                        __builtin_amdgcn_sched_barrier(0);
+                    }
+        } else {
 #pragma unroll
         for (int i = 0; i < TM; ++i)
 #pragma unroll
@@ -354,16 +430,12 @@
                     }
                 }
             }
+        }
         if (!next) break;
-#pragma unroll
-        for (int i = 0; i < TM; ++i)
-#pragma unroll
-            for (int j = 0; j < TN; ++j)
-#pragma unroll
-                for (int r = 0; r < 16; ++r) acc[i][j][r] = 0.f;
-    }
-}
-template <int ABL = 0, bool WALK = true, bool DRAIN = false>
+        zero_acc();
+    }
+}
+template <int ABL = 0, bool WALK = true, bool DRAIN = false, bool M16 = false>
 __global__ __launch_bounds__(512, 1) void gemm_split3a_kernel(const Split3aArgs g) {
     constexpr int TN = 4, BM = 256, BN = 128;
     constexpr int AROW = 128, BROW = 192;
@@ -394,7 +466,7 @@
 #pragma unroll
         for (int ps = 0; ps < 4; ++ps) {
             const int row = (ps * 8 + wave) * 8 + (lane >> 3);
-            const unsigned pc = (unsigned)((lane & 7) ^ ((row >> 1) & 7)) * 16u;
+            const unsigned pc = (unsigned)((lane & 7) ^ split3a_swz(row & 15, M16)) * 16u;
             int m = m0 + row;
             m = m < g.M ? m : g.M - 1;
             a_voff0[ps] = (unsigned)m * (unsigned)g.pix0 * 4u + pc;
@@ -407,7 +479,7 @@
                 const int sl = wl * 32 + lane;
                 const int r = sl / 12, pos = sl - r * 12;
                 const int rowt = wave * 8 + r;
-                int j = pos - ((rowt >> 2) & 3);
+                int j = pos - split3_rot(rowt, M16);
                 j = j < 0 ? j + 12 : j;
                 int n = n0 + hb * 64 + rowt;
                 n = n < g.N ? n : g.N - 1;
@@ -415,8 +487,8 @@
             }
         if (g.bias) {
 #pragma unroll
-            for (int j = 0; j < TN; ++j) {
-                int n = n0 + j * 32 + l31;
+            for (int j = 0; j < (M16 ? 2 : TN); ++j) {
+                int n = n0 + (M16 ? j * 64 + lane : j * 32 + l31);
                 n = n < g.N ? n : g.N - 1;
                 bias_r[j] = g.bias[n];
             }
@@ -443,11 +515,22 @@
         }
     };
 
-    floatx16 acc[TN];
-#pragma unroll
-    for (int j = 0; j < TN; ++j)
-#pragma unroll
-        for (int r = 0; r < 16; ++r) acc[j][r] = 0.f;
+    floatx16 acc[M16 ? 1 : TN];
+    floatx4 acc16[M16 ? 2 : 1][8];
+    auto zero_acc = [&]() {
+        if constexpr (M16) {
+#pragma unroll
+            for (int t = 0; t < 2; ++t)
+#pragma unroll
+                for (int j = 0; j < 8; ++j) acc16[t][j] = floatx4{0.f, 0.f, 0.f, 0.f};
+        } else {
+#pragma unroll
+            for (int j = 0; j < TN; ++j)
+#pragma unroll
+                for (int r = 0; r < 16; ++r) acc[j][r] = 0.f;
+        }
+    };
+    zero_acc();
 
     set_item(it);
     issue_first();
@@ -461,12 +544,18 @@
 #pragma unroll
     for (int p = 0; p < 3; ++p)
 #pragma unroll
-        for (int sb = 0; sb < 2; ++sb) fr_off[p][sb] = l31 * BROW + ((p * 4 + sb * 2 + h + ((l31 >> 2) & 3)) % 12) * 16;
+        for (int sb = 0; sb < 2; ++sb)
+            fr_off[p][sb] = l31 * BROW + ((p * 4 + sb * 2 + h + split3_rot(l31, false)) % 12) * 16;
+    int fa16[2], fr16[3];
+#pragma unroll
+    for (int e = 0; e < 2; ++e) fa16[e] = split3a_m16_frag_off(lane, e);
+#pragma unroll
+    for (int p = 0; p < 3; ++p) fr16[p] = split3_m16_frag_off(lane, p);
     bf16x8 fa[2][3], fb[2][3][2];
     floatx4 ra[2];
-    auto read_a = [&](int sb, const char* a) {
-#pragma unroll
-        for (int e = 0; e < 2; ++e) ra[e] = *reinterpret_cast<const floatx4*>(a + fa_off[sb][e]);
+    auto read_a = [&](int set, const char* a) {
+#pragma unroll
+        for (int e = 0; e < 2; ++e) ra[e] = *reinterpret_cast<const floatx4*>(a + (M16 ? set * 16 * AROW + fa16[e] : fa_off[set][e]));
     };
     auto split_a = [&](int sb) {
 #pragma unroll
@@ -480,11 +569,11 @@
             }
         }
     };
-    auto read_b = [&](int sb, const char* b) {
+    auto read_b = [&](int set, const char* b) {
 #pragma unroll
         for (int p = 0; p < 3; ++p)
 #pragma unroll
-            for (int j = 0; j < 2; ++j) fb[sb][p][j] = *reinterpret_cast<const bf16x8*>(b + j * 32 * BROW + fr_off[p][sb]);
+            for (int j = 0; j < 2; ++j) fb[set][p][j] = *reinterpret_cast<const bf16x8*>(b + j * (M16 ? 16 : 32) * BROW + (M16 ? fr16[p] : fr_off[p][set]));
     };
     const bool late = wave >= 4;
     const int a_base = wave * 32 * AROW;
@@ -507,6 +596,41 @@
                     read_b(0, b + B_HALF);
                     __builtin_amdgcn_sched_barrier(0);
                 }
+                if constexpr (M16) {
+#pragma unroll
+                    for (int sg = 0; sg < 4; ++sg)
+#pragma unroll
+                        for (int pr = 0; pr < 6; ++pr) {
+                            const int s = sg >> 1, t16 = sg & 1;
+#pragma unroll
+                            for (int j = 0; j < 2; ++j) {
+                                floatx4& c = acc16[t16][4 * i + 2 * s + j];
+                                if (ABL != 3) c = __builtin_amdgcn_mfma_f32_16x16x32_bf16(fa[t16][PA[pr]], fb[s][PB[pr]][j], c, 0, 0, 0);
+                                else c[0] += (float)fa[t16][PA[pr]][0] * (float)fb[s][PB[pr]][j][0];
+                            }
+                            __builtin_amdgcn_sched_barrier(0);
+                            if (sg == 0 && pr == 0) {
+                                if (i == 0) read_a(1, a);
+                                else read_b(1, b + B_HALF + 32 * BROW);
+                            }
+                            if (i == 0 && sg == 0 && pr == 4) split_a(1);
+                            if (i == 0 && sg == 1 && pr == 0) read_b(1, b + 32 * BROW);
+                            if (i == 1 && more1) {
+                                if (sg == 2 && pr == 0) read_b(0, bn);
+                                if (sg == 3 && pr == 0) read_a(0, an);
+                                if (sg == 3 && pr == 4) split_a(0);
+                            }
+                            if (ABL != 1 && (s == 1) == late && !(pr & 1)) {
+                                const int lq = t16 * 3 + (pr >> 1);
+                                if (i == 0 && lq >= 1 && lq <= 2 && more1) issue_b(st + 1, 1, lq - 1);
+                                if (i == 1 && more2) {
+                                    if (lq < 4) issue_a(st + 2, lq);
+                                    else issue_b(st + 2, 0, lq - 4);
+                                }
+                            }
+                            __builtin_amdgcn_sched_barrier(0);
+                        }
+                } else
 #pragma unroll
                 for (int sb = 0; sb < 2; ++sb)
 #pragma unroll
@@ -549,10 +673,22 @@
         }
 
         if (g.bias) {
+            if constexpr (M16) {
+#pragma unroll
+                for (int j = 0; j < 8; ++j) {
+                    const int src = (16 * (j & 3) + (lane & 15)) * 4;
+                    const float bv = __builtin_bit_cast(float, __builtin_amdgcn_ds_bpermute(src, __builtin_bit_cast(int, bias_r[j >> 2])));
+#pragma unroll
+                    for (int t = 0; t < 2; ++t)
+#pragma unroll
+                        for (int r = 0; r < 4; ++r) acc16[t][j][r] += bv;
+                }
+            } else {
 #pragma unroll
             for (int j = 0; j < TN; ++j)
 #pragma unroll
                 for (int r = 0; r < 16; ++r) acc[j][r] += bias_r[j];
+            }
         }
         const int rowb_ = m0 + wave * 32, colb = n0;
         float* ob = g.out + (long long)rowb_ * g.out_stride;
@@ -567,6 +703,26 @@
             issue_first();
             __builtin_amdgcn_sched_barrier(0);
         }
+        if constexpr (M16) {
+            const int l15 = lane & 15, r4 = 4 * (lane >> 4);
+            int ostr = g.out_stride;
+            asm volatile("" : "+s"(ostr));
+#pragma unroll
+            for (int t = 0; t < 2; ++t)
+#pragma unroll
+                for (int j = 0; j < 8; ++j) {
+                    const int col = colb + j * 16 + l15;
+                    if (col < g.N && (ABL != 4 || acc16[t][j][0] == 1.2345e30f)) {
+#pragma unroll
+                        for (int r = 0; r < 4; ++r) {
+                            const float v = acc16[t][j][r];
+                            const unsigned voff = (unsigned)((t * 16 + r4 + r) * ostr + col) * 4u;
+                            __builtin_amdgcn_raw_buffer_store_b32(__builtin_bit_cast(unsigned, v), ro, (int)voff, 0, 0);
+                        }
+                    }
+                    __builtin_amdgcn_sched_barrier(0);
+                }
+        } else
 #pragma unroll
         for (int j = 0; j < TN; ++j) {
             const int colu = colb + j * 32;
@@ -580,10 +736,7 @@
             }
         }
         if (!next) break;
-#pragma unroll
-        for (int j = 0; j < TN; ++j)
-#pragma unroll
-            for (int r = 0; r < 16; ++r) acc[j][r] = 0.f;
+        zero_acc();
     }
 }
 #undef IRSDE_PHASE_BARRIER
@@ -684,29 +837,19 @@
     IRSDE_HIP_CHECK(hipFuncSetAttribute(reinterpret_cast<const void*>(gemm_split2i_kernel<1>), hipFuncAttributeMaxDynamicSharedMemorySize, 160 * 1024));
     IRSDE_HIP_CHECK(hipFuncSetAttribute(reinterpret_cast<const void*>(gemm_split2i_kernel<3>), hipFuncAttributeMaxDynamicSharedMemorySize, 160 * 1024));
     IRSDE_HIP_CHECK(hipFuncSetAttribute(reinterpret_cast<const void*>(gemm_split2i_kernel<4>), hipFuncAttributeMaxDynamicSharedMemorySize, 160 * 1024));
-    IRSDE_HIP_CHECK(hipFuncSetAttribute(reinterpret_cast<const void*>(gemm_split3i_kernel<0, true>), hipFuncAttributeMaxDynamicSharedMemorySize, 160 * 1024));
-    IRSDE_HIP_CHECK(hipFuncSetAttribute(reinterpret_cast<const void*>(gemm_split3i_kernel<0, false>), hipFuncAttributeMaxDynamicSharedMemorySize, 160 * 1024));
-    IRSDE_HIP_CHECK(hipFuncSetAttribute(reinterpret_cast<const void*>(gemm_split3i_kernel<0, true, true>), hipFuncAttributeMaxDynamicSharedMemorySize, 160 * 1024));
-    IRSDE_HIP_CHECK(hipFuncSetAttribute(reinterpret_cast<const void*>(gemm_split3a_kernel<0, true>), hipFuncAttributeMaxDynamicSharedMemorySize, 160 * 1024));
-    IRSDE_HIP_CHECK(hipFuncSetAttribute(reinterpret_cast<const void*>(gemm_split3a_kernel<0, false>), hipFuncAttributeMaxDynamicSharedMemorySize, 160 * 1024));
-    IRSDE_HIP_CHECK(hipFuncSetAttribute(reinterpret_cast<const void*>(gemm_split3a_kernel<0, true, true>), hipFuncAttributeMaxDynamicSharedMemorySize, 160 * 1024));
+    auto lds160 = [](std::initializer_list<const void*> fs) {
+        for (const void* f : fs) IRSDE_HIP_CHECK(hipFuncSetAttribute(f, hipFuncAttributeMaxDynamicSharedMemorySize, 160 * 1024));
+    };
+#define IRSDE_SPLIT3_TWINS(KERNEL, ABL)                                                                                                               \
+    reinterpret_cast<const void*>(KERNEL<ABL, true, false, false>), reinterpret_cast<const void*>(KERNEL<ABL, false, false, false>),                  \
+        reinterpret_cast<const void*>(KERNEL<ABL, true, true, false>), reinterpret_cast<const void*>(KERNEL<ABL, true, false, true>),                 \
+        reinterpret_cast<const void*>(KERNEL<ABL, false, false, true>), reinterpret_cast<const void*>(KERNEL<ABL, true, true, true>)
+    lds160({IRSDE_SPLIT3_TWINS(gemm_split3i_kernel, 0), IRSDE_SPLIT3_TWINS(gemm_split3a_kernel, 0)});
 #ifdef IRSDE_PROBES
-    for (const void* f : {reinterpret_cast<const void*>(gemm_split3a_kernel<1, true>), reinterpret_cast<const void*>(gemm_split3a_kernel<3, true>),
-                          reinterpret_cast<const void*>(gemm_split3a_kernel<4, true>), reinterpret_cast<const void*>(gemm_split3a_kernel<1, false>),
-                          reinterpret_cast<const void*>(gemm_split3a_kernel<3, false>), reinterpret_cast<const void*>(gemm_split3a_kernel<4, false>),
-                          reinterpret_cast<const void*>(gemm_split3a_kernel<1, true, true>), reinterpret_cast<const void*>(gemm_split3a_kernel<3, true, true>),
-                          reinterpret_cast<const void*>(gemm_split3a_kernel<4, true, true>)})
-        IRSDE_HIP_CHECK(hipFuncSetAttribute(f, hipFuncAttributeMaxDynamicSharedMemorySize, 160 * 1024));
-    IRSDE_HIP_CHECK(hipFuncSetAttribute(reinterpret_cast<const void*>(gemm_split3i_kernel<1, true>), hipFuncAttributeMaxDynamicSharedMemorySize, 160 * 1024));
-    IRSDE_HIP_CHECK(hipFuncSetAttribute(reinterpret_cast<const void*>(gemm_split3i_kernel<3, true>), hipFuncAttributeMaxDynamicSharedMemorySize, 160 * 1024));
-    IRSDE_HIP_CHECK(hipFuncSetAttribute(reinterpret_cast<const void*>(gemm_split3i_kernel<4, true>), hipFuncAttributeMaxDynamicSharedMemorySize, 160 * 1024));
-    IRSDE_HIP_CHECK(hipFuncSetAttribute(reinterpret_cast<const void*>(gemm_split3i_kernel<1, false>), hipFuncAttributeMaxDynamicSharedMemorySize, 160 * 1024));
-    IRSDE_HIP_CHECK(hipFuncSetAttribute(reinterpret_cast<const void*>(gemm_split3i_kernel<3, false>), hipFuncAttributeMaxDynamicSharedMemorySize, 160 * 1024));
-    IRSDE_HIP_CHECK(hipFuncSetAttribute(reinterpret_cast<const void*>(gemm_split3i_kernel<4, false>), hipFuncAttributeMaxDynamicSharedMemorySize, 160 * 1024));
-    IRSDE_HIP_CHECK(hipFuncSetAttribute(reinterpret_cast<const void*>(gemm_split3i_kernel<1, true, true>), hipFuncAttributeMaxDynamicSharedMemorySize, 160 * 1024));
-    IRSDE_HIP_CHECK(hipFuncSetAttribute(reinterpret_cast<const void*>(gemm_split3i_kernel<3, true, true>), hipFuncAttributeMaxDynamicSharedMemorySize, 160 * 1024));
-    IRSDE_HIP_CHECK(hipFuncSetAttribute(reinterpret_cast<const void*>(gemm_split3i_kernel<4, true, true>), hipFuncAttributeMaxDynamicSharedMemorySize, 160 * 1024));
+    lds160({IRSDE_SPLIT3_TWINS(gemm_split3i_kernel, 1), IRSDE_SPLIT3_TWINS(gemm_split3i_kernel, 3), IRSDE_SPLIT3_TWINS(gemm_split3i_kernel, 4),
+            IRSDE_SPLIT3_TWINS(gemm_split3a_kernel, 1), IRSDE_SPLIT3_TWINS(gemm_split3a_kernel, 3), IRSDE_SPLIT3_TWINS(gemm_split3a_kernel, 4)});
 #endif
+#undef IRSDE_SPLIT3_TWINS
 }
 
 void launch_gemm_split_pairs(const SplitGemmArgs& a, int ncomp, hipStream_t s, int abl, bool f16) {
@@ -746,14 +889,29 @@
            (unsigned long long)M * ldc * 4ull < 0xffffffffull;
 }
 
+int split3_m16_read_offset(int kind, int lane, int sel) { return kind ? split3a_m16_frag_off(lane, sel) : split3_m16_frag_off(lane, sel); }
+
+static std::atomic<int> g_force_split3_mfma{-1};
+void set_force_split3_mfma(int shape) { g_force_split3_mfma.store(shape == 0 || shape == 1 ? shape : -1, std::memory_order_relaxed); }
+static bool split3_mfma16(Split3Launch::Tri t) {
+    if (t != Split3Launch::RULE) return t == Split3Launch::ON;
+    static const int knob = tuning_env_int("IRSDE_SPLIT3_MFMA", kSplit3MfmaDefault);
+    const int forced = g_force_split3_mfma.load(std::memory_order_relaxed);
+    return (forced >= 0 ? forced : knob) == 1;
+}
 static std::atomic<int> g_force_split3_blocks{-1};
 void set_force_split3_blocks(int n) { g_force_split3_blocks.store(n >= 8 ? n : -1, std::memory_order_relaxed); }
 
+template <int ABL, bool M16>
+static void launch_split3_twin(bool walk, bool drain, dim3 grid, size_t lds, hipStream_t s, const SplitGemmArgs& g) {
+    if (drain) hipLaunchKernelGGL((gemm_split3i_kernel<ABL, true, true, M16>), grid, dim3(512), lds, s, g);
+    else if (walk) hipLaunchKernelGGL((gemm_split3i_kernel<ABL, true, false, M16>), grid, dim3(512), lds, s, g);
+    else hipLaunchKernelGGL((gemm_split3i_kernel<ABL, false, false, M16>), grid, dim3(512), lds, s, g);
+}
 template <int ABL>
-static void launch_split3_abl(bool walk, bool drain, dim3 grid, size_t lds, hipStream_t s, const SplitGemmArgs& g) {
-    if (drain) hipLaunchKernelGGL((gemm_split3i_kernel<ABL, true, true>), grid, dim3(512), lds, s, g);
-    else if (walk) hipLaunchKernelGGL((gemm_split3i_kernel<ABL, true>), grid, dim3(512), lds, s, g);
-    else hipLaunchKernelGGL((gemm_split3i_kernel<ABL, false>), grid, dim3(512), lds, s, g);
+static void launch_split3_abl(bool m16, bool walk, bool drain, dim3 grid, size_t lds, hipStream_t s, const SplitGemmArgs& g) {
+    if (m16) launch_split3_twin<ABL, true>(walk, drain, grid, lds, s, g);
+    else launch_split3_twin<ABL, false>(walk, drain, grid, lds, s, g);
 }
 void launch_gemm_split_triples(const SplitGemmArgs& a, int ncomp, hipStream_t s, const Split3Launch& o) {
     if (a.K % SG_BK) throw HipError("gemm_split_triples: K must be a multiple of 32");
@@ -763,6 +921,7 @@
     const bool walk = o.walk == Split3Launch::RULE ? walk_knob : o.walk == Split3Launch::ON;
     const bool drain = o.drain == Split3Launch::RULE ? drain_knob : o.drain == Split3Launch::ON;
     if (drain && !walk) throw HipError("gemm_split_triples: the drain twin exists on the walk only");
+    const bool m16 = split3_mfma16(o.mfma16);
     SplitGemmArgs g = a;
     g.nblk_n = (a.N + 127) / 128;
     g.n_inner = ncomp;
@@ -778,11 +937,11 @@
     const dim3 grid((unsigned)blocks);
     const size_t lds = (size_t)2 * (256 + 128) * 192;
     switch (o.abl) {
-        case Split3Launch::FULL: launch_split3_abl<0>(walk, drain, grid, lds, s, g); break;
+        case Split3Launch::FULL: launch_split3_abl<0>(m16, walk, drain, grid, lds, s, g); break;
 #ifdef IRSDE_PROBES
-        case Split3Launch::NO_LOADS: launch_split3_abl<1>(walk, drain, grid, lds, s, g); break;
-        case Split3Launch::NO_MFMA: launch_split3_abl<3>(walk, drain, grid, lds, s, g); break;
-        case Split3Launch::NO_STORES: launch_split3_abl<4>(walk, drain, grid, lds, s, g); break;
+        case Split3Launch::NO_LOADS: launch_split3_abl<1>(m16, walk, drain, grid, lds, s, g); break;
+        case Split3Launch::NO_MFMA: launch_split3_abl<3>(m16, walk, drain, grid, lds, s, g); break;
+        case Split3Launch::NO_STORES: launch_split3_abl<4>(m16, walk, drain, grid, lds, s, g); break;
 #endif
         default: throw HipError("gemm_split_triples: the ablation twins are part of the PROBES build");
     }
@@ -867,11 +1026,16 @@
     return c;
 }
 
+template <int ABL, bool M16>
+static void launch_split3a_twin(bool walk, bool drain, dim3 grid, hipStream_t s, const Split3aArgs& g) {
+    if (drain) hipLaunchKernelGGL((gemm_split3a_kernel<ABL, true, true, M16>), grid, dim3(512), kSplit3aLds, s, g);
+    else if (walk) hipLaunchKernelGGL((gemm_split3a_kernel<ABL, true, false, M16>), grid, dim3(512), kSplit3aLds, s, g);
+    else hipLaunchKernelGGL((gemm_split3a_kernel<ABL, false, false, M16>), grid, dim3(512), kSplit3aLds, s, g);
+}
 template <int ABL>
-static void launch_split3a_abl(bool walk, bool drain, dim3 grid, hipStream_t s, const Split3aArgs& g) {
-    if (drain) hipLaunchKernelGGL((gemm_split3a_kernel<ABL, true, true>), grid, dim3(512), kSplit3aLds, s, g);
-    else if (walk) hipLaunchKernelGGL((gemm_split3a_kernel<ABL, true>), grid, dim3(512), kSplit3aLds, s, g);
-    else hipLaunchKernelGGL((gemm_split3a_kernel<ABL, false>), grid, dim3(512), kSplit3aLds, s, g);
+static void launch_split3a_abl(bool m16, bool walk, bool drain, dim3 grid, hipStream_t s, const Split3aArgs& g) {
+    if (m16) launch_split3a_twin<ABL, true>(walk, drain, grid, s, g);
+    else launch_split3a_twin<ABL, false>(walk, drain, grid, s, g);
 }
 void launch_gemm_split3a(const Split3aArgs& a, hipStream_t s, const Split3Launch& o) {
     const char* why = nullptr;
@@ -879,6 +1043,7 @@
     if (!a.in0 || (a.C1 && !a.in1) || !a.w3 || !a.out) throw HipError("gemm_split3a: null operand");
     const bool walk = o.walk != Split3Launch::OFF, drain = o.drain == Split3Launch::ON;
     if (drain && !walk) throw HipError("gemm_split3a: the drain twin exists on the walk only");
+    const bool m16 = split3_mfma16(o.mfma16);
     Split3aArgs g = a;
     g.nblk_n = (a.N + 127) / 128;
     const int forced = g_force_split3_blocks.load(std::memory_order_relaxed);
@@ -886,11 +1051,11 @@
     if (blocks < 1) throw HipError("gemm_split3a: grid too large");
     const dim3 grid((unsigned)blocks);
     switch (o.abl) {
-        case Split3Launch::FULL: launch_split3a_abl<0>(walk, drain, grid, s, g); break;
+        case Split3Launch::FULL: launch_split3a_abl<0>(m16, walk, drain, grid, s, g); break;
 #ifdef IRSDE_PROBES
-        case Split3Launch::NO_LOADS: launch_split3a_abl<1>(walk, drain, grid, s, g); break;
-        case Split3Launch::NO_MFMA: launch_split3a_abl<3>(walk, drain, grid, s, g); break;
-        case Split3Launch::NO_STORES: launch_split3a_abl<4>(walk, drain, grid, s, g); break;
+        case Split3Launch::NO_LOADS: launch_split3a_abl<1>(m16, walk, drain, grid, s, g); break;
+        case Split3Launch::NO_MFMA: launch_split3a_abl<3>(m16, walk, drain, grid, s, g); break;
+        case Split3Launch::NO_STORES: launch_split3a_abl<4>(m16, walk, drain, grid, s, g); break;
 #endif
         default: throw HipError("gemm_split3a: the ablation twins are part of the PROBES build");
     }
diff --git a/include/irsde_hip_debug.h b/include/irsde_hip_debug.h
--- a/include/irsde_hip_debug.h
+++ b/include/irsde_hip_debug.h
@@ -35,6 +35,8 @@
 int irsde_debug_force_split3(int mode);
 int irsde_debug_force_split3_attn(int mode);
 int irsde_debug_force_split3_blocks(int n);
+int irsde_debug_force_split3_mfma(int shape);
+int irsde_debug_split3_m16_read_offset(int kind, int lane, int sel);
 int irsde_debug_force_split3_1x1(int mode);
 int irsde_debug_split3_1x1(const float* in0, int C0, int pix0, const float* in1, int C1, int pix1, const float* w, const float* bias, float* out, int M, int N,
                            int out_stride, int mode, void* stream);
```

Result: no change. 5.126 images/s, median of 6 (+0.9%).
